# eloialonso/diamond

Measured on NVIDIA H100. Metric: imagined frames/sec (64x64, 3 denoise steps), higher is better.
Workload: dtype fp16 tensor-core operands (split-fp16 on the residual-stream 1x1/conv_in layers), fp32 accumulate, fp32 activations

## Files before the change

### diamond_b200/_lib.py

```python
import ctypes as C
import os
from typing import Optional

_HERE = os.path.dirname(os.path.abspath(__file__))
LIB_PATH = os.path.join(_HERE, "libdiamond_b200.so")
DMD_MAX_LEVELS = 8

_vp, _i, _f, _sz = C.c_void_p, C.c_int, C.c_float, C.c_size_t


class PrepDesc(C.Structure):
    _fields_ = [
        ("src0", _vp), ("src1", _vp), ("C0", _i), ("C1", _i), ("B", _i), ("Hs", _i), ("Ws", _i), ("upsample", _i),
        ("mode", _i), ("silu", _i), ("stats0", _vp), ("stats1", _vp), ("gs0", _i), ("gs1", _i),
        ("film", _vp), ("film_stride", _i), ("film_off", _i), ("gamma", _vp), ("beta", _vp), ("eps", _f),
        ("dst0", _vp), ("dst1", _vp), ("dst_raw0", _vp), ("dst_raw1", _vp),
        ("dst_lo0", _vp), ("dst_lo1", _vp), ("dst_raw_lo0", _vp), ("dst_raw_lo1", _vp),
    ]


class ConvDesc(C.Structure):
    _fields_ = [
        ("src0", _vp), ("src1", _vp), ("C0", _i), ("C1", _i), ("B", _i), ("H", _i), ("W", _i), ("taps", _i), ("stride", _i),
        ("wpk", _vp), ("bias", _vp), ("Cout", _i), ("CoutPad", _i),
        ("residual", _vp), ("out", _vp), ("out_stats", _vp), ("out_gs", _i), ("debug", _i), ("debug_buf", _vp),
        ("precise", _i), ("wpk_layout", _i), ("src0_lo", _vp), ("src1_lo", _vp),
        ("xsrc0", _vp), ("xsrc1", _vp), ("xsrc0_lo", _vp), ("xsrc1_lo", _vp), ("xC0", _i), ("xC1", _i), ("wpk_x", _vp), ("bias_x", _vp),
    ]


class DenoiserConfigC(C.Structure):
    _fields_ = [
        ("img_channels", _i), ("num_steps_conditioning", _i), ("cond_channels", _i), ("num_levels", _i),
        ("depths", _i * DMD_MAX_LEVELS), ("channels", _i * DMD_MAX_LEVELS), ("attn_depths", _i * DMD_MAX_LEVELS),
        ("num_actions", _i), ("sigma_data", _f), ("sigma_offset_noise", _f),
    ]


class ActorCriticConfigC(C.Structure):
    _fields_ = [
        ("lstm_dim", _i), ("img_channels", _i), ("img_size", _i), ("num_levels", _i),
        ("channels", _i * DMD_MAX_LEVELS), ("down", _i * DMD_MAX_LEVELS), ("num_actions", _i),
    ]


class RewEndConfigC(C.Structure):
    _fields_ = [
        ("lstm_dim", _i), ("img_channels", _i), ("img_size", _i), ("cond_channels", _i), ("num_levels", _i),
        ("depths", _i * DMD_MAX_LEVELS), ("channels", _i * DMD_MAX_LEVELS), ("attn_depths", _i * DMD_MAX_LEVELS), ("num_actions", _i),
    ]


class SamplerConfigC(C.Structure):
    _fields_ = [
        ("num_sigmas", _i), ("sigmas_host", C.POINTER(_f)), ("order", _i),
        ("s_churn", _f), ("s_tmin", _f), ("s_tmax", _f), ("s_noise", _f),
    ]


class WgradDesc(C.Structure):
    _fields_ = [("grad", _vp), ("act", _vp), ("Cg", _i), ("Ca", _i), ("B", _i), ("H", _i), ("W", _i), ("taps", _i),
                ("dW", _vp), ("Cout", _i), ("Cin", _i), ("CinTot", _i), ("ci_off", _i), ("inv_scale", _vp),
                ("accumulate", _i), ("partial", _vp), ("partial_bytes", _sz), ("debug", _i)]


class ConvPlanInfo(C.Structure):
    _fields_ = [("tiles", _i), ("kslabs", _i), ("stages", _i), ("acc_cols", _i),
                ("smem_bytes", C.c_ulonglong), ("weight_bytes", C.c_ulonglong)]


class NormBwdDesc(C.Structure):
    _fields_ = [("x", _vp), ("gy", _vp), ("stats", _vp), ("B", _i), ("HW", _i), ("C", _i), ("gs", _i), ("mode", _i), ("act", _i),
                ("film", _vp), ("film_stride", _i), ("film_off", _i), ("film_ctot", _i), ("c_off", _i),
                ("gamma", _vp), ("beta", _vp), ("eps", _f), ("sumA", _vp), ("sumB", _vp), ("sum_stride", _i),
                ("gx", _vp), ("addend", _vp), ("accumulate", _i)]


_ll = C.c_longlong


class U8Frames(C.Structure):
    _fields_ = [("levels", _vp), ("batch_stride", _ll), ("frame_stride", _ll),
                ("kinds", _vp), ("kind_batch_stride", _ll), ("kind_frame_stride", _ll), ("table", _vp)]


class OptimTensor(C.Structure):
    _fields_ = [("param", _vp), ("grad", _vp), ("exp_avg", _vp), ("exp_avg_sq", _vp), ("numel", _ll), ("weight_decay", C.c_double)]


SIGNATURES = {
    "dmd_version": (_i, []),
    "dmd_last_error": (C.c_char_p, []),
    "dmd_launch_count": (C.c_longlong, [_i]),
    "dmd_ktrace_begin": (_i, [_i]),
    "dmd_ktrace_end": (_i, [_vp, _i]),
    "dmd_ktrace_name": (C.c_char_p, [_i]),
    "dmd_pack_conv_weight": (_i, [_vp, _vp, _i, _i, _i, _i, _i, _i, _i, _i, _vp]),
    "dmd_plc16_bytes": (_sz, [_i, _i, _i, _i]),
    "dmd_prep_act": (_i, [C.POINTER(PrepDesc), _vp]),
    "dmd_prep_plan": (_i, [C.POINTER(PrepDesc), C.POINTER(C.c_int), C.POINTER(C.c_int), C.POINTER(C.c_int)]),
    "dmd_conv_plan": (_i, [C.POINTER(ConvDesc), C.POINTER(ConvPlanInfo)]),
    "dmd_conv2d_fprop": (_i, [C.POINTER(ConvDesc), _vp]),
    "dmd_pack_conv_weight_dgrad": (_i, [_vp, _vp, _i, _i, _i, _i, _i, _vp]),
    "dmd_wgrad_partial_bytes": (_sz, []),
    "dmd_conv2d_wgrad": (_i, [C.POINTER(WgradDesc), _vp]),
    "dmd_gn_stats": (_i, [_vp, _vp, _i, _i, _i, _i, _vp]),
    "dmd_attn_fwd": (_i, [_vp] * 10 + [_i, _i, _i, _i, _f, _vp]),
    "dmd_attn_scratch_bytes": (_sz, [_i, _i, _i]),
    "dmd_attn_fwd_scratch": (_i, [_vp] * 10 + [_i, _i, _i, _i, _f, _vp, _sz, _vp]),
    "dmd_nchw_to_nhwc": (_i, [_vp, _vp, _i, _i, _i, _i, _vp]),
    "dmd_nhwc_to_nchw": (_i, [_vp, _vp, _i, _i, _i, _i, _vp]),
    "dmd_linear": (_i, [_vp, _vp, _vp, _vp, _i, _i, _i, _i, _i, _i, _vp]),
    "dmd_maxpool2_stats": (_i, [_vp, _vp, _vp, _i, _i, _i, _i, _i, _vp]),
    "dmd_lstm_gates": (_i, [_vp, _vp, _vp, _vp, _i, _i, _vp]),
    "dmd_resize_nhwc": (_i, [_vp, _vp, _i, _i, _i, _i, _i, _i, _vp, _i, _vp]),
    "dmd_norm_bwd": (_i, [C.POINTER(NormBwdDesc), _i, _vp]),
    "dmd_norm_affine_grad": (_i, [C.POINTER(NormBwdDesc), _vp, _vp, _vp, _vp]),
    "dmd_attn_bwd": (_i, [_vp] * 16 + [_i, _i, _i, _i, _f, _vp]),
    "dmd_sgemm_partial_floats": (_ll, [_i, _i, _i, _i]),
    "dmd_sgemm": (_i, [_vp, _ll, _ll, _vp, _ll, _ll, _vp, _ll, _i, _i, _i, _vp, _i, _i, _vp, _vp]),
    "dmd_film_wgrad": (_i, [_vp, _vp, _vp, _vp, _vp, _i, _i, _i, _vp, _vp]),
    "dmd_embedding_bwd": (_i, [_vp, _vp, _vp, _i, _i, _i, _i, _vp, _vp]),
    "dmd_colsum": (_i, [_vp, _vp, _vp, _vp, _ll, _i, _i, _vp]),
    "dmd_sumpool2": (_i, [_vp, _vp, _i, _i, _i, _i, _i, _vp]),
    "dmd_dsilu_mul": (_i, [_vp, _vp, _vp, _ll, _vp]),
    "dmd_maxpool2_bwd": (_i, [_vp, _vp, _vp, _i, _i, _i, _i, _vp]),
    "dmd_lstm_cell_bwd": (_i, [_vp] * 6 + [_i, _i, _vp]),
    "dmd_heads_bwd": (_i, [_vp] * 10 + [_i, _i, _i, _vp]),
    "dmd_loss_scale": (_i, [_vp, _ll, _vp, _vp, _vp]),
    "dmd_denoiser_create": (_vp, [C.POINTER(DenoiserConfigC)]),
    "dmd_denoiser_destroy": (None, [_vp]),
    "dmd_denoiser_num_tensors": (_i, [_vp]),
    "dmd_denoiser_packed_bytes": (_sz, [_vp]),
    "dmd_denoiser_set_weights": (_i, [_vp, C.POINTER(_vp), _i, _vp, _vp]),
    "dmd_denoiser_workspace_bytes": (_sz, [_vp, _i, _i, _i]),
    "dmd_denoiser_forward": (_i, [_vp, _i, _i, _i, _vp, _vp, _i, _vp, _vp, _vp, _vp, _vp, _sz, _vp]),
    "dmd_inner_model_forward": (_i, [_vp, _i, _i, _i, _vp, _vp, _i, _vp, _vp, _vp, _vp, _sz, _vp]),
    "dmd_denoiser_train_workspace_bytes": (_sz, [_vp, _i, _i, _i]),
    "dmd_denoiser_grad_layout": (C.c_longlong, [_vp, C.POINTER(C.c_longlong), C.POINTER(C.c_longlong), _i]),
    "dmd_inner_model_forward_train": (_i, [_vp, _i, _i, _i, _vp, _vp, _i, _vp, _vp, _vp, _vp, _sz, _vp]),
    "dmd_denoiser_backward": (_i, [_vp, _i, _i, _i, _vp, _vp, C.c_longlong, _vp, _vp]),
    "dmd_inner_model_forward_u8": (_i, [_vp, _i, _i, _i, _vp, _vp, _i, C.POINTER(U8Frames), _vp, _vp, _vp, _sz, _vp]),
    "dmd_inner_model_forward_train_u8": (_i, [_vp, _i, _i, _i, _vp, _vp, _i, C.POINTER(U8Frames), _vp, _vp, _vp, _sz, _vp]),
    "dmd_sampler_sample": (_i, [_vp, C.POINTER(SamplerConfigC), _i, _i, _i, _vp, _vp, _i, _vp, _vp, _vp, _vp, _sz, _i, _vp]),
    "dmd_actor_critic_create": (_vp, [C.POINTER(ActorCriticConfigC)]),
    "dmd_actor_critic_destroy": (None, [_vp]),
    "dmd_actor_critic_num_tensors": (_i, [_vp]),
    "dmd_actor_critic_packed_bytes": (_sz, [_vp]),
    "dmd_actor_critic_set_weights": (_i, [_vp, C.POINTER(_vp), _i, _vp, _vp]),
    "dmd_actor_critic_workspace_bytes": (_sz, [_vp, _i]),
    "dmd_actor_critic_forward": (_i, [_vp, _i, _vp, _vp, _vp, _vp, _vp, _vp, _vp, _vp, _sz, _vp]),
    "dmd_actor_critic_backward_scratch_bytes": (_sz, [_vp, _i]),
    "dmd_actor_critic_grad_layout": (C.c_longlong, [_vp, C.POINTER(C.c_longlong), C.POINTER(C.c_longlong), _i]),
    "dmd_actor_critic_backward": (_i, [_vp, _i] + [_vp] * 8 + [C.c_longlong, _vp, _vp, _vp, _vp, _sz, _vp]),
    "dmd_actor_critic_backward_accumulate": (_i, [_vp, _i] + [_vp] * 8 + [C.c_longlong, _vp, _vp, _vp, _vp, _sz, _vp]),
    "dmd_rew_end_create": (_vp, [C.POINTER(RewEndConfigC)]),
    "dmd_rew_end_destroy": (None, [_vp]),
    "dmd_rew_end_num_tensors": (_i, [_vp]),
    "dmd_rew_end_packed_bytes": (_sz, [_vp]),
    "dmd_rew_end_set_weights": (_i, [_vp, C.POINTER(_vp), _i, _vp, _vp]),
    "dmd_rew_end_workspace_bytes": (_sz, [_vp, _i]),
    "dmd_rew_end_predict": (_i, [_vp, _i, _i] + [_vp] * 9 + [_vp, _sz, _vp]),
    "dmd_rew_end_train_workspace_bytes": (_sz, [_vp, _i, _i]),
    "dmd_rew_end_grad_layout": (C.c_longlong, [_vp, C.POINTER(C.c_longlong), C.POINTER(C.c_longlong), _i]),
    "dmd_rew_end_forward_train": (_i, [_vp, _i, _i] + [_vp] * 9 + [_vp, _sz, _vp]),
    "dmd_rew_end_backward": (_i, [_vp, _i, _i] + [_vp] * 5 + [C.c_longlong, _vp, _vp, _vp, _vp]),
    "dmd_rew_end_predict_u8": (_i, [_vp, _i, _i, C.POINTER(U8Frames), C.POINTER(U8Frames)] + [_vp] * 7 + [_vp, _sz, _vp]),
    "dmd_rew_end_forward_train_u8": (_i, [_vp, _i, _i, C.POINTER(U8Frames), C.POINTER(U8Frames)] + [_vp] * 7 + [_vp, _sz, _vp]),
    "dmd_lambda_returns": (_i, [_vp, _vp, _vp, _vp, _vp, _i, _i, C.c_double, C.c_double, _vp]),
    "dmd_grad_norm_partial_bytes": (_sz, [C.POINTER(OptimTensor), _i]),
    "dmd_grad_norm_clip": (_i, [C.POINTER(OptimTensor), _i, C.c_double, _i, _vp, _vp, _sz, _vp]),
    "dmd_adamw_step": (_i, [C.POINTER(OptimTensor), _i, C.c_double, C.c_double, C.c_double, C.c_double, C.c_double, _vp]),
}

_lib: Optional[C.CDLL] = None


class LibraryMissing(RuntimeError):
    pass


def lib() -> C.CDLL:
    global _lib
    if _lib is None:
        if not os.path.exists(LIB_PATH):
            raise LibraryMissing(
                f"{LIB_PATH} not found: build it with `python -c 'import __graft_entry__ as g; g.build()'` "
                "(diamond_b200 has no CPU / eager fallback)"
            )
        handle = C.CDLL(LIB_PATH)
        for name, (res, args) in SIGNATURES.items():
            fn = getattr(handle, name)
            fn.restype, fn.argtypes = res, args
        _lib = handle
    return _lib


def check(rc: int) -> None:
    if rc != 0:
        raise RuntimeError("diamond_b200: " + lib().dmd_last_error().decode("utf-8", "replace"))


def ptr(t) -> Optional[int]:
    return None if t is None else t.data_ptr()


def current_stream() -> int:
    import torch

    return torch.cuda.current_stream().cuda_stream
```

### diamond_b200/csrc/api.cu

```cuda
#include <cstdlib>
#include <memory>
#include <mutex>
#include <map>
#include <cuda_runtime.h>

#include <cmath>
#include <cstdarg>
#include <cstdio>
#include <cstring>
#include <functional>
#include <string>
#include <vector>

#include "../../include/diamond_b200.h"
#include "aux_kernels.cuh"
#include "conv_tc.cuh"
#include "wgrad_tc.cuh"
#include "bwd_kernels.cuh"
#include "optim_kernels.cuh"

using namespace dmd;

static thread_local std::string g_err;
static thread_local long long g_launches = 0;

static int fail(const char* fmt, ...) {
  char buf[1024];
  va_list ap;
  va_start(ap, fmt);
  vsnprintf(buf, sizeof(buf), fmt, ap);
  va_end(ap);
  g_err = buf;
  return 1;
}
#define DMD_CHECK(cond, ...) \
  do {                       \
    if (!(cond)) return fail(__VA_ARGS__); \
  } while (0)
#define DMD_CUDA(expr)                                                                   \
  do {                                                                                   \
    cudaError_t e__ = (expr);                                                            \
    if (e__ != cudaSuccess) { (void)cudaGetLastError(); return fail("%s failed: %s", #expr, cudaGetErrorString(e__)); } \
  } while (0)
#define DMD_LAUNCH_OK()                                                                 \
  do {                                                                                  \
    ++g_launches;                                                                       \
    cudaError_t e__ = cudaGetLastError();                                               \
    if (e__ != cudaSuccess) return fail("kernel launch failed: %s (%s:%d)", cudaGetErrorString(e__), __FILE__, __LINE__); \
  } while (0)

static int u8_frames_arg(const char* who, const char* name, const dmd_u8_frames* f, U8Frames* out) {
  DMD_CHECK(f, "%s: %s is NULL", who, name);
  DMD_CHECK(f->levels, "%s: %s->levels is NULL", who, name);
  DMD_CHECK(f->kinds, "%s: %s->kinds is NULL", who, name);
  DMD_CHECK(f->table, "%s: %s->table is NULL", who, name);
  DMD_CHECK(((uintptr_t)f->table & 3) == 0, "%s: %s->table is not 4-byte aligned", who, name);
  DMD_CHECK(f->batch_stride >= 0 && f->frame_stride >= 0, "%s: %s->batch_stride / frame_stride must be >= 0 (got %lld, %lld)", who,
            name, f->batch_stride, f->frame_stride);
  DMD_CHECK(f->kind_batch_stride >= 0 && f->kind_frame_stride >= 0,
            "%s: %s->kind_batch_stride / kind_frame_stride must be >= 0 (got %lld, %lld)", who, name, f->kind_batch_stride,
            f->kind_frame_stride);
  *out = U8Frames{f->levels, f->batch_stride, f->frame_stride, f->kinds, f->kind_batch_stride, f->kind_frame_stride, f->table};
  return 0;
}

extern "C" int dmd_version(void) { return DMD_VERSION; }
extern "C" const char* dmd_last_error(void) { return g_err.c_str(); }
extern "C" long long dmd_launch_count(int reset) {
  long long v = g_launches;
  if (reset) g_launches = 0;
  return v;
}

static long long* g_kt_buf = nullptr;
static int g_kt_cap = 0, g_kt_n = 0;
static bool g_kt_on = false;
static std::vector<std::string> g_kt_names;
static long long* kt_slot(const char* kind, int grid, int aux) {
  if (!g_kt_on || g_kt_n >= g_kt_cap) return nullptr;
  char buf[96];
  snprintf(buf, sizeof(buf), "%s grid=%d aux=%d", kind, grid, aux);
  g_kt_names.push_back(buf);
  return g_kt_buf + g_kt_n++;
}
extern "C" int dmd_ktrace_begin(int capacity) {
  if (g_kt_cap < capacity) {
    if (g_kt_buf) cudaFree(g_kt_buf);
    if (cudaMalloc(&g_kt_buf, (size_t)capacity * 8) != cudaSuccess) { g_kt_buf = nullptr; g_kt_cap = 0; g_err = "ktrace: cudaMalloc failed"; return 1; }
    g_kt_cap = capacity;
  }
  cudaMemset(g_kt_buf, 0, (size_t)g_kt_cap * 8);
  g_kt_n = 0; g_kt_names.clear(); g_kt_on = true;
  return 0;
}
extern "C" int dmd_ktrace_end(long long* stamps, int capacity) {
  g_kt_on = false;
  const int n = g_kt_n < capacity ? g_kt_n : capacity;
  if (n > 0 && stamps) cudaMemcpy(stamps, g_kt_buf, (size_t)n * 8, cudaMemcpyDeviceToHost);
  return n;
}
extern "C" const char* dmd_ktrace_name(int i) { return (i >= 0 && i < (int)g_kt_names.size()) ? g_kt_names[i].c_str() : ""; }

static inline int round_up(int x, int m) { return (x + m - 1) / m * m; }
constexpr int kPlanSms = 132;
static inline int gn_group_size(int C) {
  int G = C / 32 > 1 ? C / 32 : 1;
  return C / G;
}

static size_t plc16_bytes(int B, int H, int W, int C) {
  const Plc g = plc_geometry(B, H, W);
  return (size_t)(round_up(C, 16) / 8) * g.Qalloc * 16;
}
extern "C" size_t dmd_plc16_bytes(int B, int H, int W, int C) { return plc16_bytes(B, H, W, C); }

static int tune_int(const char* name, int dflt) {
  static std::mutex mu;
  static std::map<std::string, int> cache;
  std::lock_guard<std::mutex> lk(mu);
  auto it = cache.find(name);
  if (it != cache.end()) return it->second;
  const char* v = getenv(name);
  const int r = (v && *v) ? atoi(v) : dflt;
  cache[name] = r;
  return r;
}

static int conv_fill(const dmd_conv_desc* d, ConvParams* p, size_t* smem, int* acc_cols) {
  DMD_CHECK(d->src0 && d->out && d->wpk, "conv: null src0/out/wpk");
  DMD_CHECK(d->taps == 9 || d->taps == 1, "conv: taps must be 1 or 9 (got %d)", d->taps);
  DMD_CHECK(d->debug == 0 && d->debug_buf == nullptr, "conv: debug / debug_buf must be 0 / NULL (the kernel has no bring-up switches)");
  DMD_CHECK(d->stride == 1 || d->stride == 2, "conv: stride must be 1 or 2");
  DMD_CHECK(d->C0 > 0 && d->C0 % 16 == 0 && d->C1 % 16 == 0 && d->C0 + d->C1 <= kMaxCin, "conv: operand channels must be multiples of 16, total <= %d (C0=%d C1=%d)", kMaxCin, d->C0, d->C1);
  DMD_CHECK((d->C1 == 0) == (d->src1 == nullptr), "conv: src1/C1 mismatch");
  if (d->precise) DMD_CHECK(d->src0_lo && ((d->C1 == 0) == (d->src1_lo == nullptr)), "conv: precise mode needs the low operand parts");
  DMD_CHECK(d->CoutPad % 16 == 0 && d->CoutPad >= 16 && d->CoutPad <= 128 && d->Cout <= d->CoutPad && d->Cout > 0, "conv: bad Cout=%d CoutPad=%d", d->Cout, d->CoutPad);
  memset(p, 0, sizeof(*p));
  {
    const uint8_t* hi[2] = {(const uint8_t*)d->src0, (const uint8_t*)d->src1};
    const uint8_t* lo[2] = {(const uint8_t*)d->src0_lo, (const uint8_t*)d->src1_lo};
    const int cs[2] = {d->C0, d->C1};
    const int nsrc = d->C1 ? 2 : 1;
    int n = 0;
    for (int rep = 0; rep < (d->precise ? 3 : 1); ++rep)
      for (int k = 0; k < nsrc; ++k) { p->seg_base[n] = (rep == 1) ? lo[k] : hi[k]; p->seg_slabs[n] = cs[k] / 16; ++n; }
    p->Cin = (d->C0 + d->C1) * (d->precise ? 3 : 1);
    p->Cextra = 0;
    if (d->wpk_x) {
      DMD_CHECK(d->xsrc0 && d->xsrc0_lo && d->xC0 > 0 && d->xC0 % 16 == 0 && d->xC1 % 16 == 0 && d->xC0 + d->xC1 <= kMaxCin, "conv: bad fused projection operands");
      DMD_CHECK((d->xC1 == 0) == (d->xsrc1 == nullptr) && (d->xC1 == 0) == (d->xsrc1_lo == nullptr), "conv: fused projection src1 mismatch");
      const uint8_t* xh[2] = {(const uint8_t*)d->xsrc0, (const uint8_t*)d->xsrc1};
      const uint8_t* xl[2] = {(const uint8_t*)d->xsrc0_lo, (const uint8_t*)d->xsrc1_lo};
      const int xc[2] = {d->xC0, d->xC1};
      for (int rep = 0; rep < 2; ++rep)
        for (int k = 0; k < (d->xC1 ? 2 : 1); ++k) {
          DMD_CHECK(n < kMaxSegs, "conv: too many operand segments");
          p->seg_base[n] = (rep == 1) ? xl[k] : xh[k]; p->seg_slabs[n] = xc[k] / 16; ++n;
        }
      p->Cextra = 3 * (d->xC0 + d->xC1);
      p->xslabs = 2 * (d->xC0 + d->xC1) / 16;
      p->wpk_extra = reinterpret_cast<const __half*>(d->wpk_x);
      p->bias_extra = d->bias_x;
    }
    p->nseg = n;
  }
  p->B = d->B; p->H = d->H; p->W = d->W; p->taps = d->taps; p->stride = d->stride;
  if (d->stride == 2) DMD_CHECK(p->H % 2 == 0 && p->W % 2 == 0, "conv: stride 2 needs even H,W");
  p->wpk = reinterpret_cast<const __half*>(d->wpk); p->bias = d->bias; p->Cout = d->Cout; p->CoutPad = d->CoutPad;
  p->resid = d->residual; p->out = d->out; p->ostats = d->out_stats; p->ogs = d->out_gs > 0 ? d->out_gs : d->Cout;
  const Plc g = plc_geometry(d->B, d->H, d->W);
  p->PW = g.PW; p->PH = g.PH; p->Q = g.Q; p->G = g.G; p->plane_bytes = (unsigned long long)g.Qalloc * 16;
  DMD_CHECK((long long)g.Q * (g.PW > g.PH ? g.PW : g.PH) < (1ll << 32), "conv: problem too large for 32-bit position math");
  p->trs = d->wpk_layout == 1 ? 1 : 0;
  if (p->trs) DMD_CHECK(d->taps == 9 && !d->precise && 3 * d->CoutPad <= 256, "conv: row-stacked weights need a 3x3, non-split conv with CoutPad <= 80");
  const int halo = d->taps == 9 ? g.PW + 1 : 0;
  p->P = kTileM + 2 * halo; p->Palloc = p->P | 1;
  if (d->out_stats) {
    const int L4 = d->Cout / 4;
    DMD_CHECK(g.PH * g.PW >= 64, "conv: image too small for the statistics epilogue (a tile may touch at most %d images)", kStatSlots);
    DMD_CHECK(d->Cout % 4 == 0 && (L4 == 4 || L4 == 8 || L4 == 16 || L4 == 32), "conv: out_stats needs Cout in {16,32,64,128} (got %d)", d->Cout);
    DMD_CHECK(d->out_gs == 16 || d->out_gs == 32 || d->out_gs == 64 || d->out_gs == 128, "conv: out_gs must be 16/32/64/128");
    DMD_CHECK(d->Cout % d->out_gs == 0 && d->Cout / d->out_gs <= kMaxOutGroups, "conv: bad output groups");
  }
  p->dPW.init(g.PW); p->dPH.init(g.PH);
  p->num_tiles = (g.Q + kTileM - 1) / kTileM;
  const int kslabs = p->Cin / 16 + p->xslabs;
  const uint32_t w_bytes = conv_weight_bytes(p->taps, p->Cin, p->Cextra, p->CoutPad);
  const ConvSmemLayout L0 = conv_smem_layout(w_bytes, p->Palloc, 0);
  const long long budget = 227ll * 1024 - (long long)L0.total;
  int stages = budget > 0 ? (int)(budget / (long long)L0.slab_bytes) : 0;
  if (stages > 4 * kslabs) stages = 4 * kslabs;
  if (stages > kMaxStages) stages = kMaxStages;
  DMD_CHECK(stages >= 2, "conv: shared memory too small for W=%d Cin=%d CoutPad=%d", p->W, p->Cin, p->CoutPad);
  p->stages = stages;
  *smem = conv_smem_layout(w_bytes, p->Palloc, stages).total;
  *acc_cols = d->CoutPad <= 16 ? 16 : (d->CoutPad <= 32 ? 32 : (d->CoutPad <= 64 ? 64 : 128));
  return 0;
}

struct DevState { int num_sms = 0; void* zeros = nullptr; };
static thread_local int g_num_sms = 0;
static thread_local const uint8_t* g_zeros = nullptr;
static int init_kernels() {
  static std::mutex mu;
  static std::map<int, DevState> states;
  int dev = 0;
  DMD_CUDA(cudaGetDevice(&dev));
  std::lock_guard<std::mutex> lk(mu);
  auto it = states.find(dev);
  if (it == states.end()) {
    DevState st;
    DMD_CUDA(cudaDeviceGetAttribute(&st.num_sms, cudaDevAttrMultiProcessorCount, dev));
    DMD_CUDA(cudaFuncSetAttribute(conv_tc_kernel<16, 9>, cudaFuncAttributeMaxDynamicSharedMemorySize, 227 * 1024));
    DMD_CUDA(cudaFuncSetAttribute(conv_tc_kernel<32, 9>, cudaFuncAttributeMaxDynamicSharedMemorySize, 227 * 1024));
    DMD_CUDA(cudaFuncSetAttribute(conv_tc_kernel<64, 9>, cudaFuncAttributeMaxDynamicSharedMemorySize, 227 * 1024));
    DMD_CUDA(cudaFuncSetAttribute(conv_tc_kernel<128, 9>, cudaFuncAttributeMaxDynamicSharedMemorySize, 227 * 1024));
    DMD_CUDA(cudaFuncSetAttribute(conv_tc_kernel<16, 1>, cudaFuncAttributeMaxDynamicSharedMemorySize, 227 * 1024));
    DMD_CUDA(cudaFuncSetAttribute(conv_tc_kernel<32, 1>, cudaFuncAttributeMaxDynamicSharedMemorySize, 227 * 1024));
    DMD_CUDA(cudaFuncSetAttribute(conv_tc_kernel<64, 1>, cudaFuncAttributeMaxDynamicSharedMemorySize, 227 * 1024));
    DMD_CUDA(cudaFuncSetAttribute(conv_tc_kernel<128, 1>, cudaFuncAttributeMaxDynamicSharedMemorySize, 227 * 1024));
    DMD_CUDA(cudaFuncSetAttribute(wgrad_tc_kernel<16>, cudaFuncAttributeMaxDynamicSharedMemorySize, 227 * 1024));
    DMD_CUDA(cudaFuncSetAttribute(wgrad_tc_kernel<32>, cudaFuncAttributeMaxDynamicSharedMemorySize, 227 * 1024));
    DMD_CUDA(cudaFuncSetAttribute(wgrad_tc_kernel<64>, cudaFuncAttributeMaxDynamicSharedMemorySize, 227 * 1024));
    DMD_CUDA(cudaFuncSetAttribute(attn_cluster_kernel<64>, cudaFuncAttributeMaxDynamicSharedMemorySize, 128 * 1024));
    DMD_CUDA(cudaFuncSetAttribute(attn_cluster_kernel<32>, cudaFuncAttributeMaxDynamicSharedMemorySize, 128 * 1024));
    DMD_CUDA(cudaFuncSetAttribute(attn_kernel<64>, cudaFuncAttributeMaxDynamicSharedMemorySize, 128 * 1024));
    DMD_CUDA(cudaFuncSetAttribute(attn_kernel<32>, cudaFuncAttributeMaxDynamicSharedMemorySize, 128 * 1024));
    DMD_CUDA(cudaFuncSetAttribute(attn_bwd_kernel<64>, cudaFuncAttributeMaxDynamicSharedMemorySize, 200 * 1024));
    DMD_CUDA(cudaFuncSetAttribute(attn_bwd_kernel<32>, cudaFuncAttributeMaxDynamicSharedMemorySize, 200 * 1024));
    DMD_CUDA(cudaFuncSetAttribute(linear_kernel<4>, cudaFuncAttributeMaxDynamicSharedMemorySize, 64 * 1024));
    DMD_CUDA(cudaFuncSetAttribute(linear_kernel<2>, cudaFuncAttributeMaxDynamicSharedMemorySize, 64 * 1024));
    DMD_CUDA(cudaFuncSetAttribute(linear_kernel<1>, cudaFuncAttributeMaxDynamicSharedMemorySize, 64 * 1024));
    DMD_CUDA(cudaMalloc(&st.zeros, 4096));
    DMD_CUDA(cudaMemset(st.zeros, 0, 4096));
    it = states.emplace(dev, st).first;
  }
  g_num_sms = it->second.num_sms;
  g_zeros = (const uint8_t*)it->second.zeros;
  return 0;
}

template <typename Kernel, typename Params>
static int launch_pdl(Kernel kernel, dim3 grid, dim3 block, size_t smem, cudaStream_t st, const Params& p) {
  cudaLaunchConfig_t cfg;
  memset(&cfg, 0, sizeof(cfg));
  cfg.gridDim = grid; cfg.blockDim = block; cfg.dynamicSmemBytes = smem; cfg.stream = st;
  cudaLaunchAttribute attr[1];
  attr[0].id = cudaLaunchAttributeProgrammaticStreamSerialization;
  attr[0].val.programmaticStreamSerializationAllowed = 1;
  cfg.attrs = attr; cfg.numAttrs = tune_int("DMD_NO_PDL", 0) ? 0 : 1;
  DMD_CUDA(cudaLaunchKernelEx(&cfg, kernel, p));
  DMD_LAUNCH_OK();
  return 0;
}

template <int kCols>
static int conv_launch_t(const ConvParams& p0, size_t smem, cudaStream_t st) {
  if (init_kernels()) return 1;
  const int grid = p0.num_tiles < g_num_sms ? p0.num_tiles : g_num_sms;
  ConvParams p = p0;
  p.ktrace = kt_slot(p.taps == 9 ? "conv3x3" : "conv1x1", p.num_tiles, (p.Cin + p.Cextra) * 1000 + p.W);
  if (p.taps == 9) return launch_pdl(conv_tc_kernel<kCols, 9>, dim3(grid), dim3(kConvThreads), smem, st, p);
  return launch_pdl(conv_tc_kernel<kCols, 1>, dim3(grid), dim3(kConvThreads), smem, st, p);
}

static int prep_fill(const dmd_prep_desc* d, PrepParams* p, int* nsrc) {
  DMD_CHECK(d->src0 && d->dst0, "prep: null src0/dst0");
  DMD_CHECK(d->C0 % 8 == 0 && d->C1 % 8 == 0 && d->C0 > 0 && d->C0 <= kMaxCin && d->C1 <= kMaxCin, "prep: channels must be multiples of 8 (C0=%d C1=%d)", d->C0, d->C1);
  DMD_CHECK((d->C1 == 0) == (d->src1 == nullptr) && (d->C1 == 0) == (d->dst1 == nullptr), "prep: src1/dst1/C1 mismatch");
  DMD_CHECK(d->mode >= 0 && d->mode <= 2, "prep: bad mode");
  for (int c : {d->C0, d->C1 ? d->C1 : 16}) {
    const int cp = round_up(c, 16);
    DMD_CHECK(cp == 16 || cp == 32 || cp == 64 || cp == 128, "prep: a source must have <= 16/32/64/128 channels after padding (got %d)", c);
  }
  memset(p, 0, sizeof(*p));
  p->s[0].src = d->src0; p->s[0].C = d->C0; p->s[0].Cpad = round_up(d->C0, 16); p->s[0].stats = d->stats0; p->s[0].gs = d->gs0 > 0 ? d->gs0 : 8;
  p->s[0].c_offset = 0; p->s[0].dst = (uint8_t*)d->dst0; p->s[0].dst_raw = (uint8_t*)d->dst_raw0;
  p->s[0].dst_lo = (uint8_t*)d->dst_lo0; p->s[0].dst_raw_lo = (uint8_t*)d->dst_raw_lo0;
  p->s[1].dst_lo = (uint8_t*)d->dst_lo1; p->s[1].dst_raw_lo = (uint8_t*)d->dst_raw_lo1;
  DMD_CHECK(!(d->dst_raw_lo0 && !d->dst_raw0) && !(d->dst_raw_lo1 && !d->dst_raw1), "prep: raw low part needs the raw operand too");
  p->s[1].src = d->src1; p->s[1].C = d->C1; p->s[1].Cpad = round_up(d->C1 > 0 ? d->C1 : 16, 16); p->s[1].stats = d->stats1; p->s[1].gs = d->gs1 > 0 ? d->gs1 : 8;
  p->s[1].c_offset = d->C0; p->s[1].dst = (uint8_t*)d->dst1; p->s[1].dst_raw = (uint8_t*)d->dst_raw1;
  if (d->mode) {
    DMD_CHECK(d->stats0 && d->gs0 > 0 && d->C0 % d->gs0 == 0, "prep: norm mode needs stats0/gs0");
    if (d->C1) DMD_CHECK(d->stats1 && d->gs1 > 0 && d->C1 % d->gs1 == 0, "prep: norm mode needs stats1/gs1");
    if (d->mode == 1) DMD_CHECK(d->film != nullptr, "prep: AdaGroupNorm needs film");
    if (d->mode == 2) DMD_CHECK(d->gamma && d->beta, "prep: GroupNorm needs gamma/beta");
    DMD_CHECK(d->upsample == 0, "prep: norm + upsample unsupported");
  }
  p->B = d->B; p->Hs = d->Hs; p->Ws = d->Ws; p->ups = d->upsample;
  DMD_CHECK(d->upsample >= 0 && d->upsample <= 2, "prep: upsample must be 0, 1 (nearest 2x) or 2 (zero insertion)");
  DMD_CHECK(d->upsample != 2 || (d->mode == 0 && !d->silu && d->C1 == 0 && !d->dst_raw0 && !d->dst_lo0), "prep: zero insertion is a raw single-source operand");
  p->H = d->upsample ? 2 * d->Hs : d->Hs; p->W = d->upsample ? 2 * d->Ws : d->Ws;
  p->mode = d->mode; p->act = d->silu ? 1 : 0;
  p->film = d->film; p->film_stride = d->film_stride; p->film_off = d->film_off; p->film_ctot = d->C0 + d->C1;
  p->gamma = d->gamma; p->beta = d->beta; p->eps = d->eps;
  const Plc g = plc_geometry(d->B, p->H, p->W);
  DMD_CHECK(g.PH * g.PW >= 32, "prep: image too small");
  int ppb = g.PH * g.PW >= 256 ? 256 : (g.PH * g.PW / 32) * 32;
  while (ppb > 64 && (g.Qalloc + ppb - 1) / ppb < tune_int("DMD_PREP_MIN_BLOCKS", 2 * kPlanSms)) ppb >>= 1;
  ppb = (ppb / 32) * 32;
  p->pos_per_block = ppb;
  DMD_CHECK(d->mode == 0 || (d->C0 / (d->gs0 > 0 ? d->gs0 : 8) <= 4 && d->C1 / (d->gs1 > 0 ? d->gs1 : 8) <= 4),
            "prep: at most 4 groups per source (C0=%d gs0=%d, C1=%d gs1=%d)", d->C0, d->gs0, d->C1, d->gs1);
  DMD_CHECK((long long)g.Q * (g.PW > g.PH ? g.PW : g.PH) < (1ll << 32), "prep: problem too large for 32-bit position math");
  p->PW = g.PW; p->PH = g.PH; p->Q = g.Q; p->G = g.G; p->Qalloc = g.Qalloc; p->plane_bytes = (unsigned long long)g.Qalloc * 16;
  p->dPW.init(g.PW); p->dPH.init(g.PH);
  *nsrc = d->C1 ? 2 : 1;
  return 0;
}
static int prep_launch(const PrepParams& p0, int nsrc, cudaStream_t st) {
  PrepParams p = p0;
  p.ktrace = kt_slot("prep", (p.Qalloc + p.pos_per_block - 1) / p.pos_per_block * nsrc, p.mode * 1000 + p.W);
  if (p.ups == 2) {
    const long long total = (long long)p.Qalloc * (p.s[0].Cpad >> 3);
    return launch_pdl(zero_insert_prep_kernel, dim3((unsigned)((total + 255) / 256)), dim3(256), 0, st, p);
  }
  const dim3 grid((p.Qalloc + p.pos_per_block - 1) / p.pos_per_block, 1, nsrc);
  bool fast = tune_int("DMD_PREP_FAST", 1) != 0 && p.mode != 0 && p.act && p.ups == 0;
  const bool raw = p.s[0].dst_raw != nullptr;
  for (int k = 0; k < nsrc && fast; ++k) {
    const PrepSrc& S = p.s[k];
    if (S.dst_lo != nullptr || (S.dst_raw != nullptr) != raw || (S.dst_raw_lo != nullptr) != raw || S.Cpad != p.s[0].Cpad || S.C % 8 != 0) fast = false;
  }
  if (fast && (long long)p.B * p.Hs * p.Ws * (p.s[0].C > p.s[nsrc - 1].C ? p.s[0].C : p.s[nsrc - 1].C) >= (1ll << 31)) fast = false;
  if (fast) {
    const int nch = p.s[0].Cpad >> 3;
    if (nch == 8) return raw ? launch_pdl(prep_fast_kernel<8, true>, grid, dim3(kPrepThreads), 0, st, p) : launch_pdl(prep_fast_kernel<8, false>, grid, dim3(kPrepThreads), 0, st, p);
    if (nch == 4) return raw ? launch_pdl(prep_fast_kernel<4, true>, grid, dim3(kPrepThreads), 0, st, p) : launch_pdl(prep_fast_kernel<4, false>, grid, dim3(kPrepThreads), 0, st, p);
  }
  return launch_pdl(prep_act_kernel, grid, dim3(kPrepThreads), 0, st, p);
}
extern "C" int dmd_prep_plan(const dmd_prep_desc* d, int* blocks, int* pos_per_block, int* sources) {
  DMD_CHECK(d && blocks && pos_per_block && sources, "prep_plan: null argument");
  PrepParams p; int nsrc;
  if (prep_fill(d, &p, &nsrc)) return 1;
  *blocks = (p.Qalloc + p.pos_per_block - 1) / p.pos_per_block; *pos_per_block = p.pos_per_block; *sources = nsrc;
  return 0;
}
extern "C" int dmd_conv_plan(const dmd_conv_desc* d, dmd_conv_plan_info* out) {
  DMD_CHECK(d && out, "conv_plan: null argument");
  ConvParams p; size_t smem; int cols;
  if (conv_fill(d, &p, &smem, &cols)) return 1;
  out->tiles = p.num_tiles; out->kslabs = p.Cin / 16 + p.xslabs; out->stages = p.stages; out->acc_cols = cols;
  out->smem_bytes = smem; out->weight_bytes = conv_weight_bytes(p.taps, p.Cin, p.Cextra, p.CoutPad);
  return 0;
}
extern "C" int dmd_prep_act(const dmd_prep_desc* d, void* stream) {
  PrepParams p; int nsrc;
  if (prep_fill(d, &p, &nsrc)) return 1;
  return prep_launch(p, nsrc, (cudaStream_t)stream);
}

static int conv_launch(const ConvParams& p, size_t smem, int acc_cols, cudaStream_t st) {
  switch (acc_cols) {
    case 16: return conv_launch_t<16>(p, smem, st);
    case 32: return conv_launch_t<32>(p, smem, st);
    case 64: return conv_launch_t<64>(p, smem, st);
    default: return conv_launch_t<128>(p, smem, st);
  }
}

extern "C" int dmd_conv2d_fprop(const dmd_conv_desc* d, void* stream) {
  ConvParams p; size_t smem; int cols;
  if (conv_fill(d, &p, &smem, &cols)) return 1;
  return conv_launch(p, smem, cols, (cudaStream_t)stream);
}

struct WgradLaunch { WgradParams wp; WgradReduceParams rp; size_t smem; int grid; };
static size_t wgrad_partial_bytes(int num_sms) { return (size_t)num_sms * kWgTaps * 64 * 64 * sizeof(float); }

static int wgrad_fill(const void* grad, int Cg, const void* act, int Ca, int B, int H, int W, int taps, float* partial,
                      int Cout, int Cin, int CinTot, int ci_off, const float* inv_scale, int accumulate, int debug, WgradLaunch* L) {
  DMD_CHECK(grad && act && partial, "wgrad: null operand / partial buffer");
  DMD_CHECK(taps == 9 || taps == 1, "wgrad: taps must be 1 or 9");
  DMD_CHECK(Cg % 8 == 0 && Cg > 0 && Cg <= 64, "wgrad: gradient operand channels must be a multiple of 8, <= 64 (got %d)", Cg);
  DMD_CHECK(Ca == 16 || Ca == 32 || Ca == 64, "wgrad: activation operand channels must be 16, 32 or 64 (got %d)", Ca);
  DMD_CHECK(Cout > 0 && Cout <= Cg && Cin > 0 && Cin <= Ca && ci_off >= 0 && ci_off + Cin <= CinTot, "wgrad: bad channel counts");
  if (init_kernels()) return 1;
  memset(L, 0, sizeof(*L));
  const Plc g = plc_geometry(B, H, W);
  const size_t plane = (size_t)g.Qalloc * 16;
  WgradParams& wp = L->wp;
  const int ng = Cg / 8;
  for (int j = 0; j < 8; ++j) wp.a_plane[j] = j < ng ? (const uint8_t*)grad + (size_t)j * plane : nullptr;
  wp.zeros = g_zeros;
  wp.nB = Ca / 8;
  for (int j = 0; j < wp.nB; ++j) wp.b_plane[j] = (const uint8_t*)act + (size_t)j * plane;
  wp.taps = taps; wp.PW = g.PW; wp.halo = taps == 9 ? g.PW + 1 : 0;
  wp.G = g.G; wp.num_tiles = (g.Q + kTileM - 1) / kTileM; wp.Pb = kTileM + 2 * wp.halo;
  const WgradSmem one = wgrad_smem(wp.nB, wp.halo, 1);
  int stages = (int)((227ll * 1024 - 256) / (long long)(one.a_bytes + one.b_bytes));
  if (stages > kWgStagesMax) stages = kWgStagesMax;
  DMD_CHECK(stages >= 2, "wgrad: image too wide for the shared-memory stage (W=%d)", W);
  wp.stages = stages;
  wp.partial = partial; wp.dbg = debug;
  L->smem = wgrad_smem(wp.nB, wp.halo, stages).total;
  L->grid = wp.num_tiles < g_num_sms ? wp.num_tiles : g_num_sms;
  WgradReduceParams& rp = L->rp;
  rp.partial = partial; rp.nparts = L->grid; rp.N = Ca;
  rp.Cout = Cout; rp.Cin = Cin; rp.CinTot = CinTot; rp.ci_off = ci_off; rp.taps = taps;
  rp.inv_scale = inv_scale; rp.accumulate = accumulate;
  return 0;
}
static int wgrad_launch(const WgradLaunch& L, float* dW, cudaStream_t st) {
  const int N = L.wp.nB * 8;
  if (N == 16) { if (launch_pdl(wgrad_tc_kernel<16>, dim3(L.grid), dim3(kWgThreads), L.smem, st, L.wp)) return 1; }
  else if (N == 32) { if (launch_pdl(wgrad_tc_kernel<32>, dim3(L.grid), dim3(kWgThreads), L.smem, st, L.wp)) return 1; }
  else if (launch_pdl(wgrad_tc_kernel<64>, dim3(L.grid), dim3(kWgThreads), L.smem, st, L.wp)) return 1;
  WgradReduceParams rp = L.rp;
  rp.dW = dW;
  const int total = rp.taps * 64 * rp.N;
  wgrad_reduce_kernel<<<(total + 63) / 64, 256, 0, st>>>(rp);
  DMD_LAUNCH_OK();
  return 0;
}

extern "C" size_t dmd_wgrad_partial_bytes(void) {
  if (init_kernels()) return 0;
  return wgrad_partial_bytes(g_num_sms);
}
extern "C" int dmd_conv2d_wgrad(const dmd_wgrad_desc* d, void* stream) {
  DMD_CHECK(d && d->dW, "wgrad: null descriptor / dW");
  if (init_kernels()) return 1;
  DMD_CHECK(d->partial_bytes >= wgrad_partial_bytes(g_num_sms), "wgrad: partial buffer too small (%zu < %zu)", d->partial_bytes, wgrad_partial_bytes(g_num_sms));
  WgradLaunch L;
  if (wgrad_fill(d->grad, d->Cg, d->act, d->Ca, d->B, d->H, d->W, d->taps, (float*)d->partial, d->Cout, d->Cin, d->CinTot, d->ci_off,
                 d->inv_scale, d->accumulate, d->debug, &L)) return 1;
  return wgrad_launch(L, d->dW, (cudaStream_t)stream);
}
extern "C" int dmd_pack_conv_weight_dgrad(const float* w, void* wpk, int CoutF, int CinTotF, int ci_off, int CinK, int taps, void* stream) {
  DMD_CHECK(w && wpk, "pack_T: null pointer");
  const int CinP = round_up(CoutF, 16), CoutP = round_up(CinK, 16);
  const int total = taps * CinP * CoutP;
  pack_conv_weight_T_kernel<<<(total + 255) / 256, 256, 0, (cudaStream_t)stream>>>(w, (__half*)wpk, CoutF, CinTotF, ci_off, CinK, CinP, CoutP, taps);
  DMD_LAUNCH_OK();
  return 0;
}

extern "C" int dmd_pack_conv_weight(const float* w, void* wpk, int Cout, int CoutPad, int CinReal, int Cin, int taps,
                                    int c0_real, int c0_store, int precise, void* stream) {
  DMD_CHECK(w && wpk, "pack: null pointer");
  if (precise == 3) {
    DMD_CHECK(taps == 9, "pack: the row-stacked layout is for 3x3 kernels");
    const int total3 = 9 * Cin * CoutPad;
    pack_conv_weight_trs_kernel<<<(total3 + 255) / 256, 256, 0, (cudaStream_t)stream>>>(w, (__half*)wpk, Cout, CoutPad, CinReal, Cin, c0_real, c0_store);
    DMD_LAUNCH_OK();
    return 0;
  }
  DMD_CHECK(precise >= 0 && precise <= 2, "pack: precise must be 0, 1 (split [W_hi | W_hi | W_lo]), 2 (low parts only) or 3 (row-stacked)");
  const int total = taps * Cin * CoutPad * (precise == 1 ? 3 : 1);
  pack_conv_weight_kernel<<<(total + 255) / 256, 256, 0, (cudaStream_t)stream>>>(w, (__half*)wpk, Cout, CoutPad, CinReal, Cin, taps, c0_real, c0_store, precise);
  DMD_LAUNCH_OK();
  return 0;
}

extern "C" int dmd_gn_stats(const float* x, double* stats, int B, int HW, int C, int gs, void* stream) {
  DMD_CHECK(x && stats && gs > 0 && C % gs == 0, "gn_stats: bad arguments");
  long long per = (long long)HW * C;
  int chunks = (int)((per + 256 * 64 - 1) / (256 * 64));
  if (chunks < 1) chunks = 1;
  if (chunks > 64) chunks = 64;
  gn_stats_kernel<<<dim3(chunks, B), 256, 0, (cudaStream_t)stream>>>(x, stats, HW, C, gs);
  DMD_LAUNCH_OK();
  return 0;
}

static size_t attn_scratch_bytes(int B, int L, int C) { return L == kAttnL ? 0 : (size_t)B * L * 3 * C * sizeof(float); }

static int attn_launch(const AttnParams& p, int B, cudaStream_t st) {
  DMD_CHECK((p.C == 64 || p.C == 32) && p.L >= 1 && p.C % p.gs == 0 && p.gs % 8 == 0,
            "attn: unsupported shape L=%d C=%d gs=%d (C in {32, 64}, groups of a multiple of 8 channels)", p.L, p.C, p.gs);
  if (init_kernels()) return 1;
  if (p.L != kAttnL) {
    DMD_CHECK(p.scratch && ((uintptr_t)p.scratch & 15) == 0, "attn: L=%d needs 16-byte aligned scratch of dmd_attn_scratch_bytes", p.L);
    DMD_CHECK(B >= 1 && B <= 65535, "attn: B=%d out of range", B);
    const dim3 grid((p.L + kAttnTile - 1) / kAttnTile, B);
    AttnParams pa = p;
    pa.ktrace = kt_slot("attn qkv", (int)(grid.x * grid.y), p.L);
    if (p.C == 64) attn_qkv_kernel<64><<<grid, kAttnQkvThreads, 0, st>>>(pa);
    else attn_qkv_kernel<32><<<grid, kAttnQkvThreads, 0, st>>>(pa);
    DMD_LAUNCH_OK();
    pa.ktrace = kt_slot("attn softmax", (int)(grid.x * grid.y), p.L);
    if (p.C == 64) attn_stream_kernel<64><<<grid, kAttnSThreads, 0, st>>>(pa);
    else attn_stream_kernel<32><<<grid, kAttnSThreads, 0, st>>>(pa);
    DMD_LAUNCH_OK();
    return 0;
  }
  const size_t smem = sizeof(float) * ((size_t)p.L * (p.C + 1) * 2 + (size_t)p.L * (3 * p.C + 4));
  AttnParams pt = p;
  pt.ktrace = kt_slot("attn", B, p.C);
  if (tune_int("DMD_ATTN_CLUSTER", 1) != 0 && p.gs % (p.C / 4) == 0) {
    const int CH = p.C / 4;
    const size_t csmem = sizeof(float) * ((size_t)p.L * (p.C + 1) * 2 + (size_t)p.L * (3 * CH + 4) + (size_t)p.L * CH + (size_t)4 * CH * p.C);
    if (p.C == 64) attn_cluster_kernel<64><<<4 * B, kAttnCThreads, csmem, st>>>(pt);
    else attn_cluster_kernel<32><<<4 * B, kAttnCThreads, csmem, st>>>(pt);
    DMD_LAUNCH_OK();
    return 0;
  }
  if (p.C == 64) attn_kernel<64><<<B, kAttnThreads, smem, st>>>(pt);
  else attn_kernel<32><<<B, kAttnThreads, smem, st>>>(pt);
  DMD_LAUNCH_OK();
  return 0;
}

static int linear_launch(const float* in, const float* W, const float* bias, float* out, int B, int K, int F, int silu, cudaStream_t st,
                         int accumulate = 0, int hw_perm = 0) {
  DMD_CHECK(K % 4 == 0, "linear: K=%d must be a multiple of 4", K);
  DMD_CHECK(hw_perm == 0 || K % hw_perm == 0, "linear: bad hw_perm");
  if (init_kernels()) return 1;
  const int by = (B + 31) / 32;
  const int forceJ = tune_int("DMD_LINEAR_J", 0);
  if (forceJ == 4 || (forceJ == 0 && (long long)((F + 31) / 32) * by >= 2 * kPlanSms))
    linear_kernel<4><<<dim3((F + 31) / 32, by), 256, (size_t)(32 + 32) * kLinChunk * sizeof(float), st>>>(in, W, bias, out, B, K, F, silu, accumulate, hw_perm);
  else if (forceJ == 2 || (forceJ == 0 && (long long)((F + 15) / 16) * by >= kPlanSms))
    linear_kernel<2><<<dim3((F + 15) / 16, by), 256, (size_t)(16 + 32) * kLinChunk * sizeof(float), st>>>(in, W, bias, out, B, K, F, silu, accumulate, hw_perm);
  else
    linear_kernel<1><<<dim3((F + 7) / 8, by), 256, (size_t)(8 + 32) * kLinChunk * sizeof(float), st>>>(in, W, bias, out, B, K, F, silu, accumulate, hw_perm);
  DMD_LAUNCH_OK();
  return 0;
}

static int maxpool2_stats_launch(const float* x, float* y, double* stats, int B, int H, int W, int C, int gs, cudaStream_t st) {
  DMD_CHECK(H % 2 == 0 && W % 2 == 0, "maxpool2_stats: H=%d, W=%d must be even", H, W);
  DMD_CHECK((long long)(H / 2) * (W / 2) * C < (1ll << 31), "maxpool2_stats: image too large for 32-bit indices");
  if (stats) DMD_CHECK(gs > 0 && C % gs == 0 && (gs % 32 == 0 || (gs <= 32 && (gs & (gs - 1)) == 0)) && (C % 32 == 0 || 256 % C == 0),
                       "maxpool2_stats: statistics need gs a power of two <= 32 or a multiple of 32, and C %% 32 == 0 or 256 %% C == 0 (C=%d gs=%d)", C, gs);
  const int total = (H / 2) * (W / 2) * C;
  maxpool2_stats_kernel<<<dim3((total + 255) / 256, B), 256, 0, st>>>(x, y, stats, H, W, C, gs);
  DMD_LAUNCH_OK();
  return 0;
}

static int lstm_gates_launch(const float* gates, const float* c_in, float* h_out, float* c_out, int B, int Hd, cudaStream_t st) {
  lstm_gates_kernel<<<(B * Hd + 255) / 256, 256, 0, st>>>(gates, c_in, h_out, c_out, B, Hd);
  DMD_LAUNCH_OK();
  return 0;
}

extern "C" int dmd_linear(const float* in, const float* W, const float* bias, float* out, int B, int K, int F, int silu, int accumulate,
                          int hw_perm, void* stream) {
  DMD_CHECK(in && W && out && B > 0 && K > 0 && F > 0 && hw_perm >= 0, "linear: bad arguments");
  return linear_launch(in, W, bias, out, B, K, F, silu, (cudaStream_t)stream, accumulate, hw_perm);
}
extern "C" int dmd_maxpool2_stats(const float* x, float* y, double* stats, int B, int H, int W, int C, int gs, void* stream) {
  DMD_CHECK(x && y && B > 0 && H > 0 && W > 0 && C > 0, "maxpool2_stats: bad arguments");
  return maxpool2_stats_launch(x, y, stats, B, H, W, C, gs, (cudaStream_t)stream);
}
extern "C" int dmd_lstm_gates(const float* gates, const float* c_in, float* h_out, float* c_out, int B, int Hd, void* stream) {
  DMD_CHECK(gates && c_in && h_out && c_out && B > 0 && Hd > 0, "lstm_gates: bad arguments");
  DMD_CHECK((long long)B * Hd <= (1ll << 30), "lstm_gates: too many cells for 32-bit indices");
  return lstm_gates_launch(gates, c_in, h_out, c_out, B, Hd, (cudaStream_t)stream);
}

extern "C" int dmd_attn_fwd(const float* x, const double* stats_in, const float* gamma, const float* beta,
                            const float* wqkv, const float* bqkv, const float* wout, const float* bout, float* out,
                            double* out_stats, int B, int L, int C, int gs, float eps, void* stream) {
  AttnParams p{x, stats_in, gamma, beta, wqkv, bqkv, wout, bout, out, out_stats, L, C, gs, eps};
  return attn_launch(p, B, (cudaStream_t)stream);
}
extern "C" size_t dmd_attn_scratch_bytes(int B, int L, int C) { return B > 0 && L > 0 && C > 0 ? attn_scratch_bytes(B, L, C) : 0; }
extern "C" int dmd_attn_fwd_scratch(const float* x, const double* stats_in, const float* gamma, const float* beta,
                                    const float* wqkv, const float* bqkv, const float* wout, const float* bout, float* out,
                                    double* out_stats, int B, int L, int C, int gs, float eps, void* scratch, size_t scratch_bytes,
                                    void* stream) {
  DMD_CHECK(x && stats_in && gamma && beta && wqkv && bqkv && wout && bout && out && B > 0 && L > 0 && C > 0 && gs > 0,
            "attn_fwd_scratch: bad arguments");
  DMD_CHECK(scratch_bytes >= attn_scratch_bytes(B, L, C), "attn_fwd_scratch: scratch too small (%zu < %zu)", scratch_bytes,
            attn_scratch_bytes(B, L, C));
  AttnParams p{x, stats_in, gamma, beta, wqkv, bqkv, wout, bout, out, out_stats, L, C, gs, eps};
  p.scratch = (float*)scratch;
  return attn_launch(p, B, (cudaStream_t)stream);
}

extern "C" int dmd_nchw_to_nhwc(const float* in, float* out, int B, int C, int CP, int HW, void* stream) {
  nchw_to_nhwc_kernel<<<dim3((HW + 255) / 256, B), 256, 0, (cudaStream_t)stream>>>(in, out, C, CP, HW);
  DMD_LAUNCH_OK();
  return 0;
}
extern "C" int dmd_nhwc_to_nchw(const float* in, float* out, int B, int C, int CP, int HW, void* stream) {
  nhwc_to_nchw_kernel<<<dim3((HW + 255) / 256, B), 256, 0, (cudaStream_t)stream>>>(in, out, C, CP, HW);
  DMD_LAUNCH_OK();
  return 0;
}


static int loss_scale_launch(const float* g, long long n, unsigned int* amax_bits, float* scale, cudaStream_t st) {
  absmax_kernel<<<(int)std::min<long long>(std::max<long long>((n + 255) / 256, 1), 1184), 256, 0, st>>>(g, amax_bits, n);
  DMD_LAUNCH_OK();
  loss_scale_kernel<<<1, 1, 0, st>>>(amax_bits, scale);
  DMD_LAUNCH_OK();
  return 0;
}

static int colsum_launch(const float* x, float* out, float* out2, const float* inv, long long rows, int C, int Creal, cudaStream_t st) {
  const int L4 = (C < 256 ? C : 256) >> 2, lanes = 256 / L4;
  long long blocks = (rows + (long long)lanes * 8 - 1) / ((long long)lanes * 8);
  blocks = blocks > 592 ? 592 : (blocks < 1 ? 1 : blocks);
  colsum_kernel<<<dim3((unsigned)blocks, (C + 255) / 256), 256, 0, st>>>(x, out, out2, inv, rows, C, Creal);
  DMD_LAUNCH_OK();
  return 0;
}

static int norm_bwd_ppb(int B, int HW) {
  int ppb = HW;
  while (ppb > 32 && (long long)B * ((HW + ppb - 1) / ppb) < 2 * kPlanSms) ppb >>= 1;
  return ppb;
}
static int norm_bwd_launch(const NormBwdParams& nb, int pass, cudaStream_t st) {
  const int ppb = norm_bwd_ppb(nb.B, nb.HW);
  const dim3 grid((nb.HW + ppb - 1) / ppb, nb.B);
  if (pass == 1) norm_bwd_pass1_kernel<<<grid, kNormThreads, 0, st>>>(nb, ppb);
  else norm_bwd_pass2_kernel<<<grid, kNormThreads, 0, st>>>(nb, ppb);
  DMD_LAUNCH_OK();
  return 0;
}
// ... 217 lines not shown
  FilmW n1, n2; ConvW c1, c2;
  int has_attn; int an_w, an_b, qkv_w, qkv_b, op_w, op_b;
};

struct Tens { float* data; double* stats; int C, H, W, gs; float* grad = nullptr; int gid = -1; };

enum OpKind { OP_CONV = 0, OP_ATTN = 1, OP_PREP = 2, OP_RESIZE = 4 };
struct Op { int kind; ConvParams conv; size_t smem; int cols; AttnParams attn; PrepParams prep; int prep_nsrc; ResizeParams rs; };
constexpr int kScratchSlots = 10;

struct Operand {
  uint8_t *n0 = nullptr, *n1 = nullptr, *r0 = nullptr, *r1 = nullptr, *nl0 = nullptr, *rl0 = nullptr, *rl1 = nullptr; int C0 = 0, C1 = 0, H = 0, W = 0, op = -1;
  Tens a{}, b{}; bool has_b = false;
  int upsample = 0, mode = 0; const FilmW* film = nullptr; int gamma_idx = 0, beta_idx = 0; bool silu = false, also_raw = false, split = false;
};

enum BKind { B_PREP = 0, B_CONV, B_WGRAD, B_COLSUM, B_NORM1, B_NORM2, B_AFFINE, B_POOL, B_ATTN, B_MEMSET, B_SGEMM, B_FILMW,
             B_LINEAR, B_DSILU, B_EMB };
struct BOp {
  int kind = 0;
  PrepParams prep; int prep_nsrc = 1;
  ConvParams conv; size_t smem = 0; int cols = 0;
  WgradLaunch wg;
  long long goff = -1, goff2 = -1;
  NormBwdParams nb;
  int chunks = 0;
  const float* src = nullptr; float* dst = nullptr; long long rows = 0; int C = 0, Creal = 0, H = 0, W = 0, acc = 0;
  AttnBwdParams ab; long long goffs[6] = {-1, -1, -1, -1, -1, -1};
  void* ms_ptr = nullptr; size_t ms_bytes = 0;
  const float *ga = nullptr, *gb = nullptr; float* gc = nullptr; long long sam = 0, sak = 0, sbk = 0, sbn = 0, ldc = 0, c_goff = -1;
  int M = 0, N = 0, K = 0, use_inv = 0;
  const float *lin_in = nullptr, *lin_w = nullptr, *lin_b = nullptr; float* lin_out = nullptr; int lin_K = 0, lin_F = 0;
  int emb_T = 0, emb_actions = 0;
};

enum RecKind { R_CONVIN = 0, R_DOWN, R_UP, R_RES, R_OUT };
struct Rec {
  int kind = 0;
  const ConvW* cw = nullptr; const ResBlockW* rb = nullptr;
  Tens x, skip, t, o, a; bool has_skip = false;
  Operand in1, in2;
};

struct Plan {
  int B = 0, H = 0, W = 0;
  int T = 1;
  long long tmp_floats = 0;
  uint8_t* base = nullptr;
  size_t bytes = 0;
  float *xin = nullptr, *cs = nullptr, *cemb = nullptr, *chid = nullptr, *cond = nullptr, *film = nullptr, *fout = nullptr;
  double* stats = nullptr; size_t stats_bytes = 0;
  int CP_in = 0, CF = 0;
  std::vector<Op> ops;
  uint8_t* scratch[kScratchSlots] = {nullptr};
  int scratch_next = 0;
  bool train = false;
  int n_grad_tensors = 0;
  std::vector<BOp> bops;
  std::vector<Rec> tape;
  const int64_t* t_act = nullptr;
  float *tA = nullptr, *tB = nullptr, *tC = nullptr;
  uint8_t *gyA = nullptr, *gyB = nullptr;
  float *gF = nullptr;
  float *dfilm = nullptr, *nsum = nullptr, *partial = nullptr, *scale = nullptr;
  float *dcond = nullptr, *dh = nullptr, *cpre = nullptr, *dpre = nullptr, *de = nullptr;
  unsigned int* amax = nullptr;
  long long *film_woff = nullptr, *film_boff = nullptr;
  std::vector<long long> film_woff_h, film_boff_h;
  uint8_t* zero_begin = nullptr; size_t zero_bytes = 0;
  Tens feat{};
  float *gates = nullptr;
  float *cseq = nullptr, *hseq = nullptr;
  float *hid = nullptr, *logits_tm = nullptr;
  int64_t* act_tm = nullptr;
  float *g_tm = nullptr, *g_hid = nullptr, *hpre = nullptr, *g_pre = nullptr, *g_y = nullptr, *dgates = nullptr, *gcs = nullptr;
  float *s_xc = nullptr, *s_x2 = nullptr, *s_d = nullptr;
  float *sig_all = nullptr, *cemb_all = nullptr, *chid_all = nullptr, *cond_all = nullptr, *film_all = nullptr;
};

constexpr int kMaxSamplerEvals = 24;
struct SamplerGraph {
  bool valid = false;
  int B = 0, H = 0, W = 0; void* ws = nullptr; int order = 0; bool has_eps = false;
  const void *obs = nullptr, *act = nullptr, *traj = nullptr, *eps = nullptr, *out = nullptr; StackView sv{};
  unsigned long long stamp = 0;
  std::vector<float> sigmas; float churn[4] = {0, 0, 0, 0};
  long long kernels = 0;
  cudaGraphExec_t exec = nullptr;
};

struct ModelCore {
  int n_tensors = 0;
  std::vector<long long> numel, goff;
  long long grad_total = 0;
  std::vector<const float*> ptrs;
  uint8_t* packed = nullptr;
  size_t packed_bytes = 0;
  int cond_channels = 0, film_rows = 0;
  size_t film_w_off = 0, film_b_off = 0;
  std::vector<std::unique_ptr<Plan>> tplans;

  const float* P(int idx) const { return ptrs.empty() ? nullptr : ptrs[idx]; }
  void finish(size_t pk) {
    n_tensors = (int)numel.size();
    goff.assign(n_tensors, 0);
    grad_total = 0;
    for (int i = 0; i < n_tensors; ++i) { goff[i] = grad_total; grad_total += (numel[i] + 3) & ~3ll; }
    film_w_off = pk; pk += (size_t)film_rows * cond_channels * 4; pk = (pk + 255) & ~(size_t)255;
    film_b_off = pk; pk += (size_t)film_rows * 4; pk = (pk + 255) & ~(size_t)255;
    packed_bytes = pk;
  }
  int set_weights(const char* module, const float* const* ptrs_host, int n_ptrs, void* packed_buf, bool* moved) {
    DMD_CHECK(ptrs_host && packed_buf, "set_weights: null argument");
    DMD_CHECK(n_ptrs == n_tensors, "set_weights: expected %d tensors (%s.state_dict order), got %d", n_tensors, module, n_ptrs);
    *moved = packed != (uint8_t*)packed_buf || ptrs.empty() || memcmp(ptrs.data(), ptrs_host, sizeof(float*) * n_ptrs) != 0;
    ptrs.assign(ptrs_host, ptrs_host + n_ptrs);
    packed = (uint8_t*)packed_buf;
    return 0;
  }
  bool ready() const { return !ptrs.empty() && packed; }
};

long long grad_layout(const ModelCore* m, long long* offsets, long long* numels, int n) {
  if (!m || n != m->n_tensors) { fail("grad_layout: expected %d entries", m ? m->n_tensors : 0); return -1; }
  for (int i = 0; i < n; ++i) { if (offsets) offsets[i] = m->goff[i]; if (numels) numels[i] = m->numel[i]; }
  return m->grad_total;
}

struct RewEndLayout {
  Plan plan;
  Tens feat{};
  float *x_gates = nullptr, *y = nullptr, *hid = nullptr, *logits_tm = nullptr, *hc[2] = {nullptr, nullptr};
};

}

struct dmd_denoiser {
  dmd_denoiser_config cfg;
  ModelCore core;
  int i_fourier = 0, i_actemb = 0, i_cp0w = 0, i_cp0b = 0, i_cp2w = 0, i_cp2b = 0, i_normout_w = 0, i_normout_b = 0;
  ConvW conv_in, conv_out;
  std::vector<std::vector<ResBlockW>> d_blocks, u_blocks;
  std::vector<ResBlockW> mid;
  std::vector<ConvW> downs, ups;
  Plan plan;
  std::vector<SamplerGraph> graphs;
  unsigned long long graph_clock = 0;
  cudaStream_t cap_stream = nullptr;
  int need_B = 0, need_H = 0, need_W = 0; size_t need_bytes = 0;
};

struct dmd_rew_end {
  dmd_rew_end_config cfg;
  ModelCore core;
  ConvW conv_in;
  std::vector<std::vector<ResBlockW>> blocks;
  std::vector<ConvW> downs;
  int i_actemb = 0, i_wih = 0, i_whh = 0, i_bih = 0, i_bhh = 0, i_h0w = 0, i_h0b = 0, i_h2w = 0;
  int feat_c = 0, feat_hw = 0;
  RewEndLayout lay;
};

namespace {

struct Walker {
  ModelCore* m; size_t pk = 0;
  int next(long long n) { m->numel.push_back(n); return (int)m->numel.size() - 1; }
  size_t take(size_t bytes) { const size_t off = pk; pk = (pk + bytes + 255) & ~(size_t)255; return off; }
  ConvW conv(int cout, int cin_real, int taps, int c0_real, int c0_store, int c1, bool split = false, bool dgrad = true) {
    ConvW c; c.w_idx = next((long long)cout * cin_real * taps); c.b_idx = next(cout);
    c.Cout = cout; c.CoutPad = round_up(cout, 16); c.CinReal = cin_real; c.taps = taps;
    c.c0_real = c0_real; c.c0_store = c0_store; c.Cin = round_up(c0_store + c1, 16);
    const size_t w1 = (size_t)taps * c.Cin * c.CoutPad * 2;
    c.precise = split && 3 * w1 <= 120 * 1024;
    c.three_pass = split && !c.precise;
    c.trs = (taps == 9 && !split && 3 * c.CoutPad <= 256 && tune_int("DMD_CONV_TRS", 0) != 0) ? 1 : 0;
    c.pk_off = take(w1 * (c.precise ? 3 : 1));
    if (c.three_pass) c.pk_lo_off = take(w1);
    if (dgrad) {
      c.nsrcT = c1 ? 2 : 1;
      c.srcC[0] = c0_real; c.srcC[1] = c1; c.srcOff[0] = 0; c.srcOff[1] = c0_real;
      for (int k = 0; k < c.nsrcT; ++k) c.pkT_off[k] = take((size_t)taps * round_up(cout, 16) * round_up(c.srcC[k], 16) * 2);
    }
    return c;
  }
  FilmW film(int C) {
    FilmW f; f.w_idx = next((long long)2 * C * m->cond_channels); f.b_idx = next(2 * C);
    f.C = C; f.off = m->film_rows; m->film_rows += 2 * C; return f;
  }
  ResBlockW resblock(int c0, int c1, int cout, bool attn) {
    ResBlockW r; r.cin = c0 + c1; r.cout = cout;
    r.has_proj = (r.cin != cout);
    if (r.has_proj) r.proj = conv(cout, r.cin, 1, c0, c0, c1, true);
    r.n1 = film(r.cin);
    r.c1 = conv(cout, r.cin, 9, c0, c0, c1);
    r.n2 = film(cout);
    r.c2 = conv(cout, cout, 9, cout, cout, 0);
    r.has_attn = attn;
    if (attn) {
      r.an_w = next(cout); r.an_b = next(cout); r.qkv_w = next((long long)3 * cout * cout); r.qkv_b = next(3 * cout);
      r.op_w = next((long long)cout * cout); r.op_b = next(cout);
    }
    return r;
  }
};

int build_structure(dmd_denoiser* h) {
  const dmd_denoiser_config& c = h->cfg;
  const int L = c.num_levels;
  h->core.cond_channels = c.cond_channels;
  Walker w{&h->core};
  const long long CC = c.cond_channels;
  h->i_fourier = w.next(CC / 2); h->i_actemb = w.next((long long)c.num_actions * (CC / c.num_steps_conditioning));
  h->i_cp0w = w.next(CC * CC); h->i_cp0b = w.next(CC); h->i_cp2w = w.next(CC * CC); h->i_cp2b = w.next(CC);
  const int cin_real = (c.num_steps_conditioning + 1) * c.img_channels;
  const int cin_store = round_up(cin_real, 16);
  h->conv_in = w.conv(c.channels[0], cin_real, 9, cin_real, cin_store, 0, true, false);
  h->d_blocks.resize(L);
  for (int i = 0; i < L; ++i) {
    const int c1 = c.channels[i > 0 ? i - 1 : 0], c2 = c.channels[i];
    for (int k = 0; k < c.depths[i]; ++k) h->d_blocks[i].push_back(w.resblock(k == 0 ? c1 : c2, 0, c2, c.attn_depths[i] != 0));
  }
  h->u_blocks.resize(L);
  for (int m = 0; m < L; ++m) {
    const int i = L - 1 - m;
    const int c1 = c.channels[i > 0 ? i - 1 : 0], c2 = c.channels[i];
    const int n = c.depths[i];
    for (int k = 0; k <= n; ++k) h->u_blocks[m].push_back(w.resblock(c2, k < n ? c2 : c1, k < n ? c2 : c1, c.attn_depths[i] != 0));
  }
  for (int k = 0; k < 2; ++k) h->mid.push_back(w.resblock(c.channels[L - 1], 0, c.channels[L - 1], true));
  h->downs.resize(L); h->ups.resize(L);
  for (int i = 1; i < L; ++i) h->downs[i] = w.conv(c.channels[i - 1], c.channels[i - 1], 9, c.channels[i - 1], c.channels[i - 1], 0);
  for (int m = 1; m < L; ++m) { const int ch = c.channels[L - 1 - m]; h->ups[m] = w.conv(ch, ch, 9, ch, ch, 0); }
  h->i_normout_w = w.next(c.channels[0]); h->i_normout_b = w.next(c.channels[0]);
  h->conv_out = w.conv(c.img_channels, c.channels[0], 9, c.channels[0], c.channels[0], 0);
  h->core.finish(w.pk);
  return 0;
}

dmd_prep_desc prep_desc(const float* src, int C, int B, int Hs, int Ws, int ups, int mode, const double* stats, const float* gamma,
                        const float* beta, void* dst, void* dst_lo = nullptr) {
  dmd_prep_desc d; memset(&d, 0, sizeof(d));
  d.src0 = src; d.C0 = C; d.B = B; d.Hs = Hs; d.Ws = Ws; d.upsample = ups; d.mode = mode; d.silu = mode ? 1 : 0;
  if (mode) { d.stats0 = stats; d.gs0 = gn_group_size(C); d.gamma = gamma; d.beta = beta; }
  d.eps = kGnEps; d.dst0 = dst; d.dst_lo0 = dst_lo;
  return d;
}
dmd_conv_desc dgrad_desc(const ConvW& cw, int k, const void* wpk, const void* gy, int B, int H, int W, float* out, bool accumulate) {
  dmd_conv_desc d; memset(&d, 0, sizeof(d));
  d.src0 = gy; d.C0 = round_up(cw.Cout, 16); d.B = B; d.H = H; d.W = W; d.taps = cw.taps; d.stride = 1;
  d.wpk = wpk; d.Cout = cw.srcC[k]; d.CoutPad = round_up(cw.srcC[k], 16);
  d.out = out; d.residual = accumulate ? out : nullptr;
  return d;
}
dmd_conv_desc conv_pass(dmd_conv_desc d, int pass, const void* wpk_lo) {
  const void *lo0 = d.src0_lo, *lo1 = d.src1_lo;
  d.precise = 0; d.src0_lo = d.src1_lo = nullptr;
  if (pass == 1) { d.src0 = lo0; d.src1 = lo1; }
  if (pass == 2) d.wpk = wpk_lo;
  if (pass > 0) { d.bias = nullptr; d.residual = d.out; }
  if (pass < 2) d.out_stats = nullptr;
  return d;
}
NormBwdParams gn_bwd_params(const float* x, const float* gy, const double* stats, int B, int HW, int C, int gs, const float* gamma,
                            const float* beta, float* nsum, float* gx, const float* addend, bool accumulate) {
  NormBwdParams nb; memset(&nb, 0, sizeof(nb));
  nb.x = x; nb.gy = gy; nb.stats = stats; nb.B = B; nb.HW = HW; nb.C = C; nb.gs = gs; nb.mode = 2; nb.act = 1; nb.eps = kGnEps;
  nb.gamma = gamma; nb.beta = beta;
  nb.sumA = nsum; nb.sumB = nsum ? nsum + (size_t)B * kMaxCin : nullptr; nb.sum_stride = kMaxCin;
  nb.gx = gx; nb.addend = addend; nb.accumulate = accumulate ? 1 : 0;
  return nb;
}

struct Bump {
  uint8_t* base; size_t off = 0;
  void* take(size_t bytes) { off = (off + 255) & ~(size_t)255; void* p = base ? base + off : nullptr; off += bytes; return p; }
};

struct PlanBuilder {
  const ModelCore* core; Plan* pl; Bump* bump; Bump* sbump; int err = 0;

  Tens tensor(int C, int H, int W, bool with_stats, bool with_grad = true) {
    Tens t; t.C = C; t.H = H; t.W = W; t.gs = gn_group_size(C);
    t.data = (float*)bump->take((size_t)pl->B * H * W * C * 4);
    t.stats = with_stats ? (double*)sbump->take((size_t)pl->B * (C / t.gs) * 2 * 8) : nullptr;
    if (pl->train && with_grad) { t.grad = (float*)bump->take((size_t)pl->B * H * W * C * 4); t.gid = pl->n_grad_tensors++; }
    return t;
  }
  void record(const Rec& r) { if (pl->train) pl->tape.push_back(r); }
  const float* P(int idx) const { return core->P(idx); }
  const void* pk(size_t off) const { return core->packed ? core->packed + off : (const void*)1; }

  uint8_t* scratch() {
    uint8_t* p = pl->scratch[pl->scratch_next];
    pl->scratch_next = (pl->scratch_next + 1) % kScratchSlots;
    return p ? p : (uint8_t*)1;
  }

  Operand prep(const Tens& a, const Tens* b, int upsample, int mode, const FilmW* film, int gamma_idx, int beta_idx, bool silu, bool also_raw, bool split = false) {
    Operand o;
    o.a = a; o.has_b = b != nullptr; if (b) o.b = *b;
    o.upsample = upsample; o.mode = mode; o.film = film; o.gamma_idx = gamma_idx; o.beta_idx = beta_idx; o.silu = silu; o.also_raw = also_raw; o.split = split;
    o.C0 = round_up(a.C, 16); o.C1 = b ? round_up(b->C, 16) : 0;
    o.H = upsample ? 2 * a.H : a.H; o.W = upsample ? 2 * a.W : a.W;
    materialize(o);
    return o;
  }
  void materialize(Operand& o) {
    if (o.n0) return;
    const Tens& a = o.a; const Tens* b = o.has_b ? &o.b : nullptr;
    dmd_prep_desc d; memset(&d, 0, sizeof(d));
    d.src0 = a.data ? a.data : (const float*)1; d.C0 = a.C; d.src1 = b ? (b->data ? b->data : (const float*)1) : nullptr; d.C1 = b ? b->C : 0;
    d.B = pl->B; d.Hs = a.H; d.Ws = a.W; d.upsample = o.upsample; d.mode = o.mode; d.silu = o.silu;
    if (o.mode) {
      d.stats0 = a.stats ? a.stats : (const double*)1; d.gs0 = a.gs;
      if (b) { d.stats1 = b->stats ? b->stats : (const double*)1; d.gs1 = b->gs; }
    }
    if (o.mode == 1) { d.film = pl->film ? pl->film : (const float*)1; d.film_stride = core->film_rows; d.film_off = o.film->off; }
    if (o.mode == 2) { d.gamma = P(o.gamma_idx) ? P(o.gamma_idx) : (const float*)1; d.beta = P(o.beta_idx) ? P(o.beta_idx) : (const float*)1; }
    d.eps = kGnEps;
    o.n0 = scratch(); d.dst0 = o.n0;
    if (b) { o.n1 = scratch(); d.dst1 = o.n1; }
    if (o.also_raw) { o.r0 = scratch(); d.dst_raw0 = o.r0; if (b) { o.r1 = scratch(); d.dst_raw1 = o.r1; } }
    if (o.split && o.also_raw) { o.rl0 = scratch(); d.dst_raw_lo0 = o.rl0; if (b) { o.rl1 = scratch(); d.dst_raw_lo1 = o.rl1; } }
    if (o.split && !o.also_raw) { o.nl0 = scratch(); d.dst_lo0 = o.nl0; }
    Op op; op.kind = OP_PREP;
    if (prep_fill(&d, &op.prep, &op.prep_nsrc)) { err = 1; return; }
    o.op = (int)pl->ops.size();
    pl->ops.push_back(op);
  }

  void conv(const ConvW& cw, Operand& in, bool raw, int stride, const Tens* resid, Tens& out, bool out_stats,
            const ConvW* xproj = nullptr, Operand* xin = nullptr) {
    materialize(in);
    if (xin) materialize(*xin);
    if (err) return;
    dmd_conv_desc d; memset(&d, 0, sizeof(d));
    if (xproj) {
      d.xsrc0 = xin->r0; d.xsrc0_lo = xin->rl0; d.xC0 = xin->C0;
      if (xin->C1) { d.xsrc1 = xin->r1; d.xsrc1_lo = xin->rl1; d.xC1 = xin->C1; }
      d.wpk_x = pk(xproj->pk_off); d.bias_x = P(xproj->b_idx);
      if (!xproj->precise) { fail("plan: a fused projection needs its split-fp16 weights in one pack"); err = 1; return; }
    }
    const bool split = cw.precise || cw.three_pass;
    d.src0 = raw ? in.r0 : in.n0; d.src1 = in.C1 ? (raw ? in.r1 : in.n1) : nullptr;
    d.precise = cw.precise; d.wpk_layout = cw.trs;
    if (split) { d.src0_lo = raw ? in.rl0 : in.nl0; d.src1_lo = in.C1 ? in.rl1 : nullptr; }
    d.C0 = in.C0; d.C1 = in.C1; d.B = pl->B; d.H = in.H; d.W = in.W; d.taps = cw.taps; d.stride = stride;
    d.wpk = pk(cw.pk_off); d.bias = P(cw.b_idx);
    d.Cout = cw.Cout; d.CoutPad = cw.CoutPad;
    d.residual = resid ? (resid->data ? resid->data : (const float*)1) : nullptr; d.out = out.data ? out.data : (float*)1;
    d.out_stats = out_stats ? (out.stats ? out.stats : (double*)1) : nullptr; d.out_gs = out.gs;
    if (split && (!d.src0_lo || (in.C1 && !d.src1_lo))) { fail("plan: precise conv without low operand parts"); err = 1; return; }
    if (in.C0 + in.C1 != cw.Cin) { fail("plan: operand channels %d+%d do not match the packed weights (%d)", in.C0, in.C1, cw.Cin); err = 1; return; }
    for (int pass = 0; pass < (cw.three_pass ? 3 : 1); ++pass) {
      const dmd_conv_desc dp = cw.three_pass ? conv_pass(d, pass, pk(cw.pk_lo_off)) : d;
      Op op; op.kind = OP_CONV;
      if (conv_fill(&dp, &op.conv, &op.smem, &op.cols)) { err = 1; return; }
      pl->ops.push_back(op);
    }
  }

  Tens resblock(const ResBlockW& rb, const Tens& x, const Tens* skip) {
    const int H = x.H, W = x.W;
    Operand in1 = prep(x, skip, 0, 1, &rb.n1, 0, 0, true, rb.has_proj != 0, rb.has_proj != 0);
    Tens t = tensor(rb.cout, H, W, true, false);
    conv(rb.c1, in1, false, 1, nullptr, t, true);
    Operand in2 = prep(t, nullptr, 0, 1, &rb.n2, 0, 0, true, false);
    Tens o = tensor(rb.cout, H, W, true);
    if (rb.has_proj) conv(rb.c2, in2, false, 1, nullptr, o, true, &rb.proj, &in1);
    else conv(rb.c2, in2, false, 1, &x, o, true);
    Rec rec; rec.kind = R_RES; rec.rb = &rb; rec.x = x; rec.has_skip = skip != nullptr; if (skip) rec.skip = *skip;
    rec.t = t; rec.o = o; rec.in1 = in1; rec.in2 = in2;
    if (!rb.has_attn) { record(rec); return o; }
    if (pl->train && H * W != kAttnL) {
      fail("training: the attention backward (attn_bwd_kernel) is built for 8x8 = 64 tokens only; this plan has an attention block "
           "over %dx%d = %d tokens (inference runs at any token count)", H, W, H * W);
      err = 1;
      return o;
    }
    Tens a = tensor(rb.cout, H, W, true);
    Op op; op.kind = OP_ATTN;
    op.attn = AttnParams{o.data, o.stats, P(rb.an_w), P(rb.an_b), P(rb.qkv_w), P(rb.qkv_b), P(rb.op_w), P(rb.op_b), a.data, a.stats, H * W, rb.cout, o.gs, kGnEps};
    if (H * W != kAttnL) op.attn.scratch = (float*)bump->take(attn_scratch_bytes(pl->B, H * W, rb.cout));
    pl->ops.push_back(op);
    rec.a = a;
    record(rec);
    return a;
  }

  int build_rew_end(const dmd_rew_end* h, Tens* feat) {
    const dmd_rew_end_config& c = h->cfg;
    const int L = c.num_levels, B = pl->B, H = pl->H, W = pl->W;
    if (H % (1 << (L - 1)) || W % (1 << (L - 1))) return fail("rew_end: H=%d W=%d must be multiples of %d", H, W, 1 << (L - 1));
    int cmax = 16;
    for (int i = 0; i < L; ++i) cmax = c.channels[i] > cmax ? c.channels[i] : cmax;
    const size_t slot_bytes = (plc16_bytes(B, H, W, cmax) + 255) & ~(size_t)255;
    for (int i = 0; i < kScratchSlots; ++i) pl->scratch[i] = (uint8_t*)bump->take(slot_bytes);
    pl->scratch_next = 0;
    pl->CP_in = h->conv_in.c0_store;
    pl->xin = (float*)bump->take((size_t)B * H * W * pl->CP_in * 4);
    pl->cond = (float*)bump->take((size_t)B * c.cond_channels * 4);
    pl->film = (float*)bump->take((size_t)B * core->film_rows * 4);
    Tens xin{pl->xin, nullptr, pl->CP_in, H, W, 8};
    Tens x = tensor(c.channels[0], H, W, true);
    {
      Operand in0 = prep(xin, nullptr, 0, 0, nullptr, 0, 0, false, false, true);
      conv(h->conv_in, in0, false, 1, nullptr, x, true);
      Rec rec; rec.kind = R_CONVIN; rec.cw = &h->conv_in; rec.x = xin; rec.o = x; rec.in1 = in0; record(rec);
    }
    for (int i = 0; i <= L; ++i) {
      if (i > 0 && i < L) {
        Tens xd = tensor(c.channels[i - 1], x.H / 2, x.W / 2, true);
        Operand ind = prep(x, nullptr, 0, 0, nullptr, 0, 0, false, false);
        conv(h->downs[i], ind, false, 2, nullptr, xd, true);
        Rec rec; rec.kind = R_DOWN; rec.cw = &h->downs[i]; rec.x = x; rec.o = xd; rec.in1 = ind; record(rec);
        x = xd;
      }
      for (auto& rb : h->blocks[i]) x = resblock(rb, x, nullptr);
    }
    *feat = x;
    return err;
  }

  void resize(const Tens& src, const Tens& dst) {
    Op op; op.kind = OP_RESIZE;
    op.rs = ResizeParams{src.data ? src.data : (const float*)1, dst.data ? dst.data : (float*)1, pl->B, src.H, src.W, dst.H, dst.W, src.C,
                         dst.stats ? dst.stats : (double*)1, dst.gs};
    pl->ops.push_back(op);
  }

  int build(const dmd_denoiser* h) {
    const dmd_denoiser_config& c = h->cfg;
    const int L = c.num_levels, B = pl->B, H = pl->H, W = pl->W;
    const int div = 1 << (L - 1);
    const int Hp = (H + div - 1) / div * div, Wp = (W + div - 1) / div * div;
    const bool padded = Hp != H || Wp != W;
    if (padded && pl->train) return fail("denoiser: training at H=%d W=%d (not multiples of %d) needs the pad / crop adjoints, which are not built", H, W, div);
    int cmax = 16;
    for (int i = 0; i < L; ++i) cmax = c.channels[i] > cmax ? c.channels[i] : cmax;
    const size_t slot_bytes = (plc16_bytes(B, Hp, Wp, cmax) + 255) & ~(size_t)255;
    for (int i = 0; i < kScratchSlots; ++i) pl->scratch[i] = (uint8_t*)bump->take(slot_bytes);
    pl->scratch_next = 0;
    pl->CP_in = h->conv_in.c0_store;
    pl->xin = (float*)bump->take((size_t)B * H * W * pl->CP_in * 4);
    pl->cs = (float*)bump->take((size_t)(B + 1) * 4 * 4);
    pl->cemb = (float*)bump->take((size_t)B * c.cond_channels * 4);
    pl->chid = (float*)bump->take((size_t)B * c.cond_channels * 4);
    pl->cond = (float*)bump->take((size_t)B * c.cond_channels * 4);
    pl->film = (float*)bump->take((size_t)B * core->film_rows * 4);
    Tens xin{pl->xin, nullptr, pl->CP_in, H, W, 8};
    Tens x = tensor(c.channels[0], H, W, !padded);
    {
      Operand in = prep(xin, nullptr, 0, 0, nullptr, 0, 0, false, false, true);
      conv(h->conv_in, in, false, 1, nullptr, x, !padded);
      Rec rec; rec.kind = R_CONVIN; rec.cw = &h->conv_in; rec.x = xin; rec.o = x; rec.in1 = in; record(rec);
    }
    if (padded) {
      Tens xp = tensor(c.channels[0], Hp, Wp, true);
      resize(x, xp);
      x = xp;
    }
    std::vector<std::vector<Tens>> d_outputs;
    for (int i = 0; i < L; ++i) {
      Tens xd = x;
      if (i > 0) {
        xd = tensor(c.channels[i - 1], x.H / 2, x.W / 2, true);
        Operand in = prep(x, nullptr, 0, 0, nullptr, 0, 0, false, false);
        conv(h->downs[i], in, false, 2, nullptr, xd, true);
        Rec rec; rec.kind = R_DOWN; rec.cw = &h->downs[i]; rec.x = x; rec.o = xd; rec.in1 = in; record(rec);
      }
      std::vector<Tens> outs{xd};
      x = xd;
      for (auto& rb : h->d_blocks[i]) { x = resblock(rb, x, nullptr); outs.push_back(x); }
      d_outputs.push_back(outs);
    }
    for (auto& rb : h->mid) x = resblock(rb, x, nullptr);
    for (int m = 0; m < L; ++m) {
      Tens xu = x;
      if (m > 0) {
        xu = tensor(x.C, x.H * 2, x.W * 2, true);
        Operand in = prep(x, nullptr, 1, 0, nullptr, 0, 0, false, false);
        conv(h->ups[m], in, false, 1, nullptr, xu, true);
        Rec rec; rec.kind = R_UP; rec.cw = &h->ups[m]; rec.x = x; rec.o = xu; rec.in1 = in; record(rec);
      }
      x = xu;
      const std::vector<Tens>& skip = d_outputs[L - 1 - m];
      const int ns = (int)skip.size();
      for (size_t k = 0; k < h->u_blocks[m].size(); ++k) x = resblock(h->u_blocks[m][k], x, &skip[ns - 1 - (int)k]);
    }
    if (padded) {
      Tens xc = tensor(x.C, H, W, true);
      resize(x, xc);
      x = xc;
    }
    pl->CF = c.img_channels;
    pl->fout = (float*)bump->take((size_t)B * H * W * pl->CF * 4);
    Tens f{pl->fout, nullptr, pl->CF, H, W, pl->CF};
    {
      Operand in = prep(x, nullptr, 0, 2, nullptr, h->i_normout_w, h->i_normout_b, true, false, false);
      conv(h->conv_out, in, false, 1, nullptr, f, false);
      Rec rec; rec.kind = R_OUT; rec.cw = &h->conv_out; rec.x = x; rec.in1 = in; record(rec);
    }
    const size_t img = (size_t)B * c.img_channels * H * W * 4;
    pl->s_xc = (float*)bump->take(img); pl->s_x2 = (float*)bump->take(img); pl->s_d = (float*)bump->take(img);
    if (!pl->train) {
      const size_t K = kMaxSamplerEvals;
      pl->sig_all = (float*)bump->take(K * 4);
      pl->cemb_all = (float*)bump->take(K * B * c.cond_channels * 4); pl->chid_all = (float*)bump->take(K * B * c.cond_channels * 4);
      pl->cond_all = (float*)bump->take(K * B * c.cond_channels * 4); pl->film_all = (float*)bump->take(K * B * core->film_rows * 4);
    }
    return err;
  }
};

int make_plan(const dmd_denoiser* h, Plan* pl, int B, int H, int W, uint8_t* base, size_t* total) {
  pl->B = B; pl->H = H; pl->W = W; pl->ops.clear();
  Bump b0{nullptr}, s0{nullptr};
  { Plan tmp; tmp.B = B; tmp.H = H; tmp.W = W; PlanBuilder pb{&h->core, &tmp, &b0, &s0}; if (pb.build(h)) return 1; }
  const size_t stats_bytes = (s0.off + 255) & ~(size_t)255;
  if (total) *total = stats_bytes + b0.off + 256;
  if (!base) return 0;
  Bump sb{base}, bb{base + stats_bytes};
  pl->base = base; pl->stats = (double*)base; pl->stats_bytes = stats_bytes;
  PlanBuilder pb{&h->core, pl, &bb, &sb};
  if (pb.build(h)) return 1;
  pl->bytes = stats_bytes + bb.off;
  return 0;
}

struct BwdBuilder {
  const ModelCore* core; Plan* pl; int err = 0;
  std::vector<char> ginit;

  const float* P(int idx) const { return core->P(idx); }
  long long G(int idx) const { return core->goff[idx]; }
  bool was_init(const Tens& t) { const bool w = ginit[t.gid] != 0; ginit[t.gid] = 1; return w; }
  void push(const BOp& b) { pl->bops.push_back(b); }
  void begin() { ginit.assign(pl->n_grad_tensors, 0); pl->bops.clear(); }

  void replay(const Operand& o) { BOp b; b.kind = B_PREP; b.prep = pl->ops[o.op].prep; b.prep_nsrc = pl->ops[o.op].prep_nsrc; push(b); }
  void gprep(const float* g, int C, int Hs, int Ws, int ups, uint8_t* dst) {
    const dmd_prep_desc d = prep_desc(g, C, pl->B, Hs, Ws, ups, 0, nullptr, nullptr, nullptr, dst);
    BOp b; b.kind = B_PREP;
    if (prep_fill(&d, &b.prep, &b.prep_nsrc)) { err = 1; return; }
    push(b);
  }
  void colsum(const float* g, long long rows, int C, int Creal, int idx, int idx2 = -1) {
    BOp b; b.kind = B_COLSUM; b.src = g; b.rows = rows; b.C = C; b.Creal = Creal; b.goff = G(idx); b.goff2 = idx2 >= 0 ? G(idx2) : -1;
    push(b);
  }
  void dgrad(const ConvW& cw, int k, const uint8_t* gy, int H, int W, float* out, bool accumulate) {
    const dmd_conv_desc d = dgrad_desc(cw, k, core->packed + cw.pkT_off[k], gy, pl->B, H, W, out, accumulate);
    BOp b; b.kind = B_CONV;
    if (conv_fill(&d, &b.conv, &b.smem, &b.cols)) { err = 1; return; }
    push(b);
  }
  void wgrad(const ConvW& cw, const uint8_t* gy, const uint8_t* act, int Ca, int Cin, int ci_off, int H, int W) {
    BOp b; b.kind = B_WGRAD; b.goff = G(cw.w_idx);
    if (wgrad_fill(gy ? gy : (const void*)1, round_up(cw.Cout, 16), act ? act : (const void*)1, Ca, pl->B, H, W, cw.taps,
                   pl->partial ? pl->partial : (float*)1, cw.Cout, Cin, cw.CinReal, ci_off, pl->scale ? pl->scale + 1 : (const float*)1, 1, 0, &b.wg)) { err = 1; return; }
    push(b);
  }
  void norm_bwd(const Tens& x, const float* gy, int mode, const FilmW* film, int c_off, int ctot, int gamma_idx, int beta_idx,
                float* gx, const float* addend, bool accumulate) {
    const int R = core->film_rows;
    NormBwdParams nb = gn_bwd_params(x.data, gy, x.stats, pl->B, x.H * x.W, x.C, x.gs, P(gamma_idx), P(beta_idx), pl->nsum, gx, addend, accumulate);
    if (mode == 1) {
      nb.mode = 1; nb.gamma = nb.beta = nullptr; nb.c_off = c_off;
      nb.film = pl->film; nb.film_stride = R; nb.film_off = film->off; nb.film_ctot = ctot;
      nb.sumB = pl->dfilm ? pl->dfilm + film->off + c_off : nullptr;
      nb.sumA = pl->dfilm ? pl->dfilm + film->off + ctot + c_off : nullptr;
      nb.sum_stride = R;
    } else {
      BOp m; m.kind = B_MEMSET; m.ms_ptr = pl->nsum; m.ms_bytes = (size_t)2 * pl->B * kMaxCin * 4; push(m);
    }
    BOp b1; b1.kind = B_NORM1; b1.nb = nb;
    push(b1);
    if (mode == 2) {
      BOp a; a.kind = B_AFFINE; a.nb = nb; a.goff = G(gamma_idx); a.goff2 = G(beta_idx); push(a);
    }
    BOp b2 = b1; b2.kind = B_NORM2; push(b2);
  }

  void resblock(const Rec& r) {
    const ResBlockW& rb = *r.rb;
    const int H = r.o.H, W = r.o.W, B = pl->B;
    const long long pix = (long long)B * H * W;
    Tens o = r.o;
    if (rb.has_attn) {
      BOp b; b.kind = B_ATTN;
      b.ab = AttnBwdParams{o.data, o.stats, P(rb.an_w), P(rb.an_b), P(rb.qkv_w), P(rb.qkv_b), P(rb.op_w), r.a.grad, o.grad,
                           nullptr, nullptr, nullptr, nullptr, nullptr, nullptr, pl->scale ? pl->scale + 1 : nullptr, H * W, rb.cout, o.gs, kGnEps};
      const int ids[6] = {rb.an_w, rb.an_b, rb.qkv_w, rb.qkv_b, rb.op_w, rb.op_b};
      for (int i = 0; i < 6; ++i) b.goffs[i] = G(ids[i]);
      push(b);
      ginit[o.gid] = 1;
    }
    const Tens* src[2] = {&r.x, r.has_skip ? &r.skip : nullptr};
    const int nsrc = r.has_skip ? 2 : 1;
    gprep(o.grad, rb.cout, H, W, 0, pl->gyA);
    colsum(o.grad, pix, rb.cout, rb.cout, rb.c2.b_idx, rb.has_proj ? rb.proj.b_idx : -1);
    replay(r.in2);
    wgrad(rb.c2, pl->gyA, r.in2.n0, round_up(rb.cout, 16), rb.cout, 0, H, W);
    dgrad(rb.c2, 0, pl->gyA, H, W, pl->tA, false);
    norm_bwd(r.t, pl->tA, 1, &rb.n2, 0, rb.cout, 0, 0, pl->tB, nullptr, false);
    gprep(pl->tB, rb.cout, H, W, 0, pl->gyB);
    colsum(pl->tB, pix, rb.cout, rb.cout, rb.c1.b_idx);
    replay(r.in1);
    for (int k = 0; k < nsrc; ++k) {
      const uint8_t* act = k == 0 ? r.in1.n0 : r.in1.n1;
      wgrad(rb.c1, pl->gyB, act, round_up(src[k]->C, 16), src[k]->C, rb.c1.srcOff[k], H, W);
      float* ga = k == 0 ? pl->tA : pl->tC;
      dgrad(rb.c1, k, pl->gyB, H, W, ga, false);
      const float* addend = (!rb.has_proj && k == 0) ? o.grad : nullptr;
      const bool acc = was_init(*src[k]);
      norm_bwd(*src[k], ga, 1, &rb.n1, rb.c1.srcOff[k], rb.cin, 0, 0, src[k]->grad, addend, acc);
    }
    if (rb.has_proj) {
      for (int k = 0; k < nsrc; ++k) {
        const uint8_t* raw = k == 0 ? r.in1.r0 : r.in1.r1;
        wgrad(rb.proj, pl->gyA, raw, round_up(src[k]->C, 16), src[k]->C, rb.proj.srcOff[k], H, W);
        dgrad(rb.proj, k, pl->gyA, H, W, src[k]->grad, true);
      }
    }
  }

  int walk(int end) {
    const int B = pl->B;
    for (int i = end - 1; i >= 0; --i) {
      const Rec& r = pl->tape[i];
      if (r.kind == R_RES) {
        resblock(r);
      } else if (r.kind == R_UP) {
        const ConvW& cw = *r.cw;
        const int H = r.o.H, W = r.o.W;
        gprep(r.o.grad, cw.Cout, H, W, 0, pl->gyA);
        colsum(r.o.grad, (long long)B * H * W, cw.Cout, cw.Cout, cw.b_idx);
        replay(r.in1);
        wgrad(cw, pl->gyA, r.in1.n0, round_up(r.x.C, 16), r.x.C, 0, H, W);
        dgrad(cw, 0, pl->gyA, H, W, pl->tA, false);
        BOp b; b.kind = B_POOL; b.src = pl->tA; b.dst = r.x.grad; b.H = r.x.H; b.W = r.x.W; b.C = r.x.C; b.acc = was_init(r.x) ? 1 : 0;
        push(b);
      } else if (r.kind == R_DOWN) {
        const ConvW& cw = *r.cw;
        const int H = r.x.H, W = r.x.W;
        gprep(r.o.grad, cw.Cout, r.o.H, r.o.W, 2, pl->gyA);
        colsum(r.o.grad, (long long)B * r.o.H * r.o.W, cw.Cout, cw.Cout, cw.b_idx);
        replay(r.in1);
        wgrad(cw, pl->gyA, r.in1.n0, round_up(r.x.C, 16), r.x.C, 0, H, W);
        dgrad(cw, 0, pl->gyA, H, W, r.x.grad, was_init(r.x));
      } else if (r.kind == R_CONVIN) {
        const ConvW& cw = *r.cw;
        const int H = r.o.H, W = r.o.W;
        gprep(r.o.grad, cw.Cout, H, W, 0, pl->gyA);
        colsum(r.o.grad, (long long)B * H * W, cw.Cout, cw.Cout, cw.b_idx);
        replay(r.in1);
        wgrad(cw, pl->gyA, r.in1.n0, cw.c0_store, cw.c0_real, 0, H, W);
      } else {
        return fail("backward plan: record %d of kind %d belongs to a model's own head", i, r.kind);
      }
      if (err) return 1;
    }
    return 0;
  }

  void sgemm(const float* A, long long sam, long long sak, const float* Bm, long long sbk, long long sbn, float* C, long long c_goff,
             long long ldc, int M, int N, int K, int use_inv, int acc) {
    BOp b; b.kind = B_SGEMM; b.ga = A; b.sam = sam; b.sak = sak; b.gb = Bm; b.sbk = sbk; b.sbn = sbn; b.gc = C; b.c_goff = c_goff; b.ldc = ldc;
    b.M = M; b.N = N; b.K = K; b.use_inv = use_inv; b.acc = acc; push(b);
  }
  void film_tail() {
    const int B = pl->B, CC = core->cond_channels, R = core->film_rows;
    { BOp b; b.kind = B_FILMW; push(b); }
    const float* Wf = core->packed ? (const float*)(core->packed + core->film_w_off) : nullptr;
    sgemm(pl->dfilm, R, 1, Wf, CC, 1, pl->dcond, -1, CC, B, CC, R, 0, 0);
    {
      const long long fit = pl->tmp_floats / ((long long)B * CC);
      int splits = R / 256; if (splits > 32) splits = 32; if (splits > fit) splits = (int)fit;
      if (splits > 1) pl->bops.back().chunks = splits;
    }
  }
  void embedding(const float* de, int idx, int T, int num_actions) {
    BOp b; b.kind = B_EMB; b.src = de; b.goff = G(idx); b.C = core->cond_channels; b.emb_T = T; b.emb_actions = num_actions; push(b);
  }
};

int build_denoiser_bwd(const dmd_denoiser* h, BwdBuilder& bw) {
  Plan* pl = bw.pl;
  const int B = pl->B;
  bw.begin();
  {
    const Rec& r = pl->tape.back();
    if (r.kind != R_OUT) return fail("denoiser backward plan: the tape does not end with the output head");
    const ConvW& cw = *r.cw;
    const int H = r.x.H, W = r.x.W;
    bw.gprep(pl->gF, 8, H, W, 0, pl->gyA);
    bw.colsum(pl->gF, (long long)B * H * W, 8, cw.Cout, cw.b_idx);
    bw.replay(r.in1);
    bw.wgrad(cw, pl->gyA, r.in1.n0, round_up(r.x.C, 16), r.x.C, 0, H, W);
    bw.dgrad(cw, 0, pl->gyA, H, W, pl->tA, false);
    bw.norm_bwd(r.x, pl->tA, 2, nullptr, 0, r.x.C, h->i_normout_w, h->i_normout_b, r.x.grad, nullptr, bw.was_init(r.x));
    if (bw.err) return 1;
  }
  if (bw.walk((int)pl->tape.size() - 1)) return 1;
  bw.film_tail();
  const int CC = h->cfg.cond_channels;
  const long long* goff = h->core.goff.data();
  bw.sgemm(pl->dcond, 1, CC, pl->chid, CC, 1, nullptr, goff[h->i_cp2w], CC, CC, CC, B, 1, 1);
  bw.colsum(pl->dcond, B, CC, CC, h->i_cp2b);
  bw.sgemm(pl->dcond, CC, 1, bw.P(h->i_cp2w), CC, 1, pl->dh, -1, CC, B, CC, CC, 0, 0);
  { BOp b; b.kind = B_LINEAR; b.lin_in = pl->cemb; b.lin_w = bw.P(h->i_cp0w); b.lin_b = bw.P(h->i_cp0b); b.lin_out = pl->cpre; b.lin_K = CC; b.lin_F = CC; bw.push(b); }
  { BOp b; b.kind = B_DSILU; b.src = pl->cpre; b.ga = pl->dh; b.dst = pl->dpre; b.rows = (long long)B * CC; bw.push(b); }
  bw.sgemm(pl->dpre, 1, CC, pl->cemb, CC, 1, nullptr, goff[h->i_cp0w], CC, CC, CC, B, 1, 1);
  bw.colsum(pl->dpre, B, CC, CC, h->i_cp0b);
  bw.sgemm(pl->dpre, CC, 1, bw.P(h->i_cp0w), CC, 1, pl->de, -1, CC, B, CC, CC, 0, 0);
  bw.embedding(pl->de, h->i_actemb, h->cfg.num_steps_conditioning, h->cfg.num_actions);
  return bw.err;
}

using FwdPlanFn = std::function<int(PlanBuilder&)>;
using BwdPlanFn = std::function<int(BwdBuilder&)>;
int make_train_plan(const ModelCore& core, int cmax, int gF_ch, Plan* pl, int B, int H, int W, int T, uint8_t* base, size_t* total,
                    const FwdPlanFn& fwd, const BwdPlanFn& bwd) {
  pl->train = true; pl->n_grad_tensors = 0; pl->tape.clear();
  pl->B = B; pl->H = H; pl->W = W; pl->T = T; pl->ops.clear(); pl->bops.clear();
  Bump b0{nullptr}, s0{nullptr};
  { Plan tmp; tmp.train = true; tmp.B = B; tmp.H = H; tmp.W = W; tmp.T = T; PlanBuilder pb{&core, &tmp, &b0, &s0}; if (fwd(pb)) return 1; }
  const size_t stats_bytes = (s0.off + 255) & ~(size_t)255;
  Bump sb{base}, bb{base ? base + stats_bytes : nullptr};
  if (base) { pl->base = base; pl->stats = (double*)base; pl->stats_bytes = stats_bytes; }
  if (base) { PlanBuilder pb{&core, pl, &bb, &sb}; if (fwd(pb)) return 1; } else bb.off = b0.off;
  pl->tmp_floats = (long long)B * H * W * cmax;
  const size_t act_bytes = (size_t)pl->tmp_floats * 4;
  pl->tA = (float*)bb.take(act_bytes); pl->tB = (float*)bb.take(act_bytes); pl->tC = (float*)bb.take(act_bytes);
  const size_t op_bytes = plc16_bytes(B, H, W, cmax);
  pl->gyA = (uint8_t*)bb.take(op_bytes); pl->gyB = (uint8_t*)bb.take(op_bytes);
  pl->gF = (float*)bb.take((size_t)B * H * W * gF_ch * 4);
  if (init_kernels()) return 1;
  pl->partial = (float*)bb.take(wgrad_partial_bytes(g_num_sms));
  const int CC = core.cond_channels;
  pl->dcond = (float*)bb.take((size_t)B * CC * 4); pl->dh = (float*)bb.take((size_t)B * CC * 4); pl->cpre = (float*)bb.take((size_t)B * CC * 4);
  pl->dpre = (float*)bb.take((size_t)B * CC * 4); pl->de = (float*)bb.take((size_t)B * CC * 4);
  pl->film_woff = (long long*)bb.take((size_t)core.film_rows * 8); pl->film_boff = (long long*)bb.take((size_t)core.film_rows * 8);
  pl->scale = (float*)bb.take(256);
  uint8_t* z0 = (uint8_t*)bb.take(0);
  pl->dfilm = (float*)bb.take((size_t)B * core.film_rows * 4);
  pl->nsum = (float*)bb.take((size_t)2 * B * kMaxCin * 4);
  pl->amax = (unsigned int*)bb.take(256);
  pl->zero_begin = z0; pl->zero_bytes = base ? (size_t)((uint8_t*)pl->amax + 256 - z0) : 0;
  if (total) *total = stats_bytes + bb.off + 512;
  if (!base) return 0;
  pl->bytes = stats_bytes + bb.off;
  BwdBuilder bw{&core, pl};
  if (bwd(bw)) return 1;
  pl->film_woff_h.assign(core.film_rows, 0); pl->film_boff_h.assign(core.film_rows, 0);
  auto fill_film = [&](const FilmW& f) {
    for (int r = 0; r < 2 * f.C; ++r) { pl->film_woff_h[f.off + r] = core.goff[f.w_idx] + (long long)r * CC; pl->film_boff_h[f.off + r] = core.goff[f.b_idx] + r; }
  };
  for (const Rec& r : pl->tape) if (r.kind == R_RES) { fill_film(r.rb->n1); fill_film(r.rb->n2); }
  return 0;
}

template <class Cfg> int widest_channels(const Cfg& c) {
  int cmax = 16;
  for (int i = 0; i < c.num_levels; ++i) cmax = c.channels[i] > cmax ? c.channels[i] : cmax;
  return cmax;
}
int make_denoiser_train_plan(const dmd_denoiser* h, Plan* pl, int B, int H, int W, uint8_t* base, size_t* total) {
  return make_train_plan(h->core, widest_channels(h->cfg), 8, pl, B, H, W, 1, base, total,
                         [h](PlanBuilder& pb) { return pb.build(h); }, [h](BwdBuilder& bw) { return build_denoiser_bwd(h, bw); });
// ... 1241 lines not shown
```

### diamond_b200/csrc/conv_tc.cuh

```cuda
#pragma once
#include "ptx.cuh"

namespace dmd {

constexpr int kConvThreads = 384;
constexpr int kConvConsumerWarps = 8;
constexpr int kTileM = 128;
constexpr int kMaxCin = 128;
constexpr int kMaxSegs = 8;
constexpr int kMaxStages = 24;
constexpr int kStatSlots = 3;
constexpr int kMaxOutGroups = 4;

struct FastDiv {
  uint32_t d, m;
  __host__ void init(uint32_t dd) {
    d = dd;
    m = (uint32_t)((0x100000000ull / dd) + 1);
  }
  __device__ __forceinline__ uint32_t div(uint32_t n) const { return d == 1 ? n : __umulhi(n, m); }
};

struct Plc {
  int PW, PH, Q, G, Qalloc;
};
__host__ __device__ inline Plc plc_geometry(int B, int H, int W) {
  Plc g;
  g.PW = W + 1; g.PH = H + 1; g.Q = B * g.PH * g.PW; g.G = g.PW + 1;
  g.Qalloc = g.G + ((g.Q + kTileM - 1) / kTileM) * kTileM + kTileM + g.PW + 1;
  return g;
}

struct ConvParams {
  const uint8_t* seg_base[kMaxSegs];
  int seg_slabs[kMaxSegs];
  int nseg;
  int Cin;
  int Cextra;
  const __half* wpk_extra;
  const float* bias_extra;
  int xslabs;
  int B, H, W;
  int taps;
  int stride;
  const __half* wpk;
  const float* bias;
  int Cout, CoutPad;
  const float* resid;
  float* out;
  double* ostats;
  int ogs;
  int PW, PH, Q, G;
  unsigned long long plane_bytes;
  int P, Palloc;
  int num_tiles, stages;
  int trs;
  FastDiv dPW, dPH;
  long long* ktrace;
};

struct ConvSmemLayout {
  uint32_t bias_off, w_off, a_off, slab_bytes, total;
};

__host__ __device__ inline uint32_t conv_weight_bytes(int taps, int Cin, int Cextra, int CoutPad) {
  return (((uint32_t)taps * Cin * CoutPad * 2 + 127u) & ~127u) + (uint32_t)Cextra * CoutPad * 2;
}
__host__ __device__ inline ConvSmemLayout conv_smem_layout(uint32_t w_bytes, int Palloc, int stages) {
  ConvSmemLayout L;
  L.bias_off = 512;
  L.w_off = L.bias_off + 128 * 4;
  L.a_off = (L.w_off + w_bytes + 127u) & ~127u;
  L.slab_bytes = 2u * Palloc * 16;
  L.total = L.a_off + (uint32_t)stages * L.slab_bytes + 16;
  return L;
}

template <int N>
struct RegEpilogue {
  int lane, r0, G;
  float s[kStatSlots][kMaxOutGroups], ss[kStatSlots][kMaxOutGroups];
  int n_cur;

  __device__ __forceinline__ void init(const ConvParams& p, int row0, int lane_) {
    lane = lane_;
    r0 = row0;
    G = p.ostats ? p.Cout / p.ogs : 1;
#pragma unroll
    for (int k = 0; k < kStatSlots; ++k)
#pragma unroll
      for (int g = 0; g < kMaxOutGroups; ++g) s[k][g] = ss[k][g] = 0.f;
    n_cur = -1;
  }

  template <int kG = kMaxOutGroups>
  __device__ __forceinline__ void flush_stats(const ConvParams& p, int img0, int nslots) {
#pragma unroll
    for (int k = 0; k < kStatSlots; ++k) {
      if (k < nslots) {
        float a[kG], b[kG];
#pragma unroll
        for (int g = 0; g < kG; ++g) { a[g] = s[k][g]; b[g] = ss[k][g]; }
#pragma unroll
        for (int m = 16; m > 0; m >>= 1)
#pragma unroll
          for (int g = 0; g < kG; ++g) {
            a[g] += __shfl_xor_sync(0xffffffffu, a[g], m);
            b[g] += __shfl_xor_sync(0xffffffffu, b[g], m);
          }
        if (lane == 0 && img0 + k < p.B) {
#pragma unroll
          for (int g = 0; g < kG; ++g)
            if (g < G && (a[g] != 0.f || b[g] != 0.f)) {
              double* dst = p.ostats + ((size_t)(img0 + k) * G + g) * 2;
              atomicAdd(dst, (double)a[g]);
              atomicAdd(dst + 1, (double)b[g]);
            }
        }
      }
#pragma unroll
      for (int g = 0; g < kMaxOutGroups; ++g) s[k][g] = ss[k][g] = 0.f;
    }
  }

  template <int kLgs, bool kFull>
  __device__ __forceinline__ void tile(const ConvParams& p, const float* sbias, const float (&acc)[N / 2], int q0) {
    constexpr bool kStats = kLgs > 0;
    constexpr int kGroups = (N / 8) >> kLgs > 0 ? ((N / 8) >> kLgs < kMaxOutGroups ? (N / 8) >> kLgs : kMaxOutGroups) : 1;
    const int n_lo = (int)p.dPH.div(p.dPW.div((uint32_t)q0));
    const int q_last = min(q0 + kTileM, p.Q) - 1;
    const bool single_image = (int)p.dPH.div(p.dPW.div((uint32_t)q_last)) == n_lo;
    if (kStats && n_cur >= 0 && (!single_image || n_lo != n_cur)) { flush_stats<kGroups>(p, n_cur, 1); n_cur = -1; }
    const int c0 = 2 * (lane & 3);
    const bool vec = kFull || (p.Cout & 1) == 0;
    const bool resid = p.resid != nullptr;
    constexpr int kBatch = N / 8 < 8 ? N / 8 : 8;
    constexpr int kRows = N / 8 <= 8 ? 2 : 1;
#pragma unroll
    for (int h0 = 0; h0 < 2; h0 += kRows) {
      int opix[kRows], slot[kRows];
#pragma unroll
      for (int r = 0; r < kRows; ++r) {
        const int q = q0 + r0 + 8 * (h0 + r);
        opix[r] = -1; slot[r] = 0;
        if (q < p.Q) {
          const uint32_t R = p.dPW.div((uint32_t)q);
          const int x = q - (int)R * p.PW;
          const int n = (int)p.dPH.div(R);
          const int y = (int)R - n * p.PH;
          bool valid = (x < p.W) && (y < p.H);
          int yo = y, xo = x, Ho = p.H, Wo = p.W;
          if (!kFull && p.stride == 2) {
            valid = valid && ((x & 1) == 0) && ((y & 1) == 0);
            yo = y >> 1; xo = x >> 1; Ho = p.H >> 1; Wo = p.W >> 1;
          }
          if (valid) { opix[r] = (n * Ho + yo) * Wo + xo; slot[r] = n - n_lo; }
        }
      }
      if (kRows == 1 && opix[0] < 0) continue;
      float gs[kRows][kMaxOutGroups], gss[kRows][kMaxOutGroups];
#pragma unroll
      for (int r = 0; r < kRows; ++r)
#pragma unroll
        for (int g = 0; g < kMaxOutGroups; ++g) gs[r][g] = gss[r][g] = 0.f;
#pragma unroll
      for (int jb = 0; jb < N / 8; jb += kBatch) {
        float2 bv[kBatch], rv[kRows][kBatch];
#pragma unroll
        for (int u = 0; u < kBatch; ++u) {
          const int col = 8 * (jb + u) + c0;
          bv[u] = (kFull || col < p.Cout) ? *reinterpret_cast<const float2*>(sbias + col) : make_float2(0.f, 0.f);
#pragma unroll
          for (int r = 0; r < kRows; ++r) {
            const int h = h0 + r;
            rv[r][u] = make_float2(0.f, 0.f);
            if (resid && opix[r] >= 0 && (kFull || col < p.Cout)) {
              const float* rp = p.resid + (size_t)opix[r] * p.Cout;
              if (vec) rv[r][u] = __ldg(reinterpret_cast<const float2*>(rp + col));
              else {
                rv[r][u].x = __ldg(rp + col);
                if (col + 1 < p.Cout) rv[r][u].y = __ldg(rp + col + 1);
              }
            }
          }
        }
#pragma unroll
        for (int r = 0; r < kRows; ++r) {
          const int h = h0 + r;
          if (opix[r] < 0) continue;
          float* op = p.out + (size_t)opix[r] * p.Cout;
#pragma unroll
          for (int u = 0; u < kBatch; ++u) {
            const int j = jb + u;
            const int col = 8 * j + c0;
            if (kFull || col < p.Cout) {
              float2 o = make_float2(acc[4 * j + 2 * h] + bv[u].x, acc[4 * j + 2 * h + 1] + bv[u].y);
              if (vec) {
                if (resid) { o.x += rv[r][u].x; o.y += rv[r][u].y; }
                *reinterpret_cast<float2*>(op + col) = o;
              } else {
                if (resid) o.x += rv[r][u].x;
                op[col] = o.x;
                if (col + 1 < p.Cout) { if (resid) o.y += rv[r][u].y; op[col + 1] = o.y; } else o.y = 0.f;
              }
              if (kStats) {
                gs[r][j >> kLgs] += o.x + o.y;
                gss[r][j >> kLgs] += fmaf(o.x, o.x, o.y * o.y);
              }
            }
          }
        }
      }
      if (kStats) {
#pragma unroll
        for (int r = 0; r < kRows; ++r) {
          const int h = h0 + r;
          if (opix[r] < 0) continue;
          if (single_image) {
#pragma unroll
            for (int g = 0; g < kGroups; ++g) { s[0][g] += gs[r][g]; ss[0][g] += gss[r][g]; }
          } else {
#pragma unroll
            for (int k = 0; k < kStatSlots; ++k)
#pragma unroll
              for (int g = 0; g < kGroups; ++g) {
                s[k][g] += (slot[r] == k) ? gs[r][g] : 0.f;
                ss[k][g] += (slot[r] == k) ? gss[r][g] : 0.f;
              }
          }
        }
      }
    }
    if (kStats) {
      if (single_image) n_cur = n_lo;
      else { flush_stats<kGroups>(p, n_lo, kStatSlots); n_cur = -1; }
    }
  }

  template <bool kFull>
  __device__ __forceinline__ void tile_any(const ConvParams& p, int lgs, const float* sbias, const float (&acc)[N / 2], int q0) {
    if (lgs == 0) tile<0, kFull>(p, sbias, acc, q0);
    else if (lgs == 1 || N == 16) tile<1, kFull>(p, sbias, acc, q0);
    else if (lgs == 2 || N == 32) tile<2, kFull>(p, sbias, acc, q0);
    else if (lgs == 3 || N == 64) tile<3, kFull>(p, sbias, acc, q0);
    else tile<4, kFull>(p, sbias, acc, q0);
  }

  __device__ __forceinline__ void finish(const ConvParams& p) {
    if (p.ostats != nullptr && n_cur >= 0) flush_stats(p, n_cur, 1);
  }
};

template <int N, int kTaps>
__global__ void __launch_bounds__(kConvThreads, 1) conv_tc_kernel(const ConvParams p) {
  extern __shared__ __align__(128) uint8_t smem[];
  uint64_t* wbar = reinterpret_cast<uint64_t*>(smem);
  uint64_t* full = wbar + 1;
  uint64_t* empty = full + kMaxStages;
  const ConvSmemLayout L = conv_smem_layout(conv_weight_bytes(p.taps, p.Cin, p.Cextra, p.CoutPad), p.Palloc, p.stages);
  float* sbias = reinterpret_cast<float*>(smem + L.bias_off);
  uint8_t* sW = smem + L.w_off;
  uint8_t* sA = smem + L.a_off;

  const int tid = threadIdx.x;
  const int warp = tid >> 5, lane = tid & 31;
  const int halo = (kTaps == 9) ? (p.PW + 1) : 0;
  const int S = p.stages;
  const int main_slabs = p.Cin >> 4;
  const int kslabs = main_slabs + p.xslabs;
  const uint32_t w_main_bytes = ((uint32_t)p.taps * p.Cin * p.CoutPad * 2 + 127u) & ~127u;
  const int tiles_lo = p.num_tiles / (int)gridDim.x, tiles_rem = p.num_tiles % (int)gridDim.x;
  const int tile_begin = (int)blockIdx.x * tiles_lo + min((int)blockIdx.x, tiles_rem);
  const int my_tiles = tiles_lo + ((int)blockIdx.x < tiles_rem ? 1 : 0);

  pdl_launch_dependents();
  if (tid == 0) {
    mbar_init(wbar, 1);
    for (int s = 0; s < S; ++s) { mbar_init(full + s, 1); mbar_init(empty + s, kConvConsumerWarps); }
    fence_mbar_init();
    const uint32_t tap_bytes = (uint32_t)p.Cin * p.CoutPad * 2;
    const uint32_t extra_bytes = (uint32_t)p.Cextra * p.CoutPad * 2;
    mbar_expect_tx(wbar, tap_bytes * p.taps + extra_bytes);
    for (int t = 0; t < p.taps; ++t)
      bulk_g2s(sW + (size_t)t * tap_bytes, reinterpret_cast<const uint8_t*>(p.wpk) + (size_t)t * tap_bytes, tap_bytes, wbar);
    if (extra_bytes) bulk_g2s(sW + w_main_bytes, p.wpk_extra, extra_bytes, wbar);
  }
  for (int i = tid; i < 128; i += blockDim.x)
    sbias[i] = ((p.bias != nullptr && i < p.Cout) ? __ldg(p.bias + i) : 0.f) + ((p.bias_extra != nullptr && i < p.Cout) ? __ldg(p.bias_extra + i) : 0.f);
  __syncthreads();
  pdl_wait();
  if (blockIdx.x == 0 && tid == 128) ktrace_stamp(p.ktrace);

  if (warp < 2) {
    const uint32_t pid = (uint32_t)warp;
    const uint32_t chunk_bytes = (uint32_t)p.P * 16;
    uint32_t stage = 0, phase = 0, nslab = 0;
    for (int it = 0; it < my_tiles; ++it) {
      const size_t pos0 = (size_t)((tile_begin + it) * kTileM - halo + p.G) * 16;
      int seg = 0, seg_ks = 0;
      for (int ks = 0; ks < kslabs; ++ks, ++nslab) {
        if ((nslab & 1u) == pid) {
          mbar_wait(empty + stage, phase ^ 1u);
          if (elect_one_sync()) {
            uint8_t* slab = sA + (size_t)stage * L.slab_bytes;
            const bool xs = ks >= main_slabs;
            const uint32_t bytes = xs ? (uint32_t)kTileM * 16 : chunk_bytes;
            mbar_expect_tx(full + stage, 2 * bytes);
            const uint8_t* plane = p.seg_base[seg] + (size_t)(2 * seg_ks) * p.plane_bytes + pos0 + (xs ? (size_t)halo * 16 : 0);
            bulk_g2s(slab, plane, bytes, full + stage);
            bulk_g2s(slab + (size_t)p.Palloc * 16, plane + p.plane_bytes, bytes, full + stage);
          }
          __syncwarp();
        }
        if (++seg_ks == p.seg_slabs[seg]) { seg_ks = 0; ++seg; }
        if (++stage == (uint32_t)S) { stage = 0; phase ^= 1u; }
      }
    }
  } else if (warp >= 4) {
    const int m0 = ((warp >> 2) - 1) * 64;
    RegEpilogue<N> epi;
    epi.init(p, m0 + 16 * (warp & 3) + (lane >> 2), lane);
    const int lgs = p.ostats ? 31 - __clz(p.ogs >> 3) : 0;
    const bool full_cols = p.Cout == N && p.stride == 1;
    if (my_tiles > 0) mbar_wait(wbar, 0);
    const uint64_t hi = gmma_desc_hi(128);
    const uint32_t a_lbo = (uint32_t)p.Palloc * 16;
    const uint32_t b_lbo = (uint32_t)(p.trs ? 3 * p.CoutPad : p.CoutPad) * 16;
    const uint32_t x_lbo = (uint32_t)p.CoutPad * 16;
    const uint32_t a_lo0 = (((smem_u32(sA) + (uint32_t)m0 * 16) >> 4) & 0x3FFFu) | (((a_lbo >> 4) & 0x3FFFu) << 16);
    const uint32_t b_lo0 = ((smem_u32(sW) >> 4) & 0x3FFFu) | (((b_lbo >> 4) & 0x3FFFu) << 16);
    const uint32_t b_x0 = (((smem_u32(sW) + w_main_bytes) >> 4) & 0x3FFFu) | (((x_lbo >> 4) & 0x3FFFu) << 16);
    const uint32_t slab16 = L.slab_bytes >> 4;
    const uint32_t kstep16 = (2u * b_lbo) >> 4;
    const uint32_t xstep16 = (2u * x_lbo) >> 4;
    uint32_t shift[kTaps], b_tap[kTaps];
#pragma unroll
    for (int t = 0; t < kTaps; ++t) {
      shift[t] = (uint32_t)(halo + (kTaps == 9 ? (t / 3 - 1) * p.PW + (t % 3 - 1) : 0));
      b_tap[t] = p.trs ? ((uint32_t)(t / 3) * p.Cin * 3u * p.CoutPad * 2 + (uint32_t)(t % 3) * p.CoutPad * 16) >> 4
                       : ((uint32_t)t * p.Cin * p.CoutPad * 2) >> 4;
    }
    const int ng = p.xslabs >> 1;
    float acc[N / 2];
    uint32_t stage = 0, phase = 0, prev = 0;
    int done = 0;
    auto slab = [&](auto issue) {
      mbar_wait(full + stage, phase);
      wgmma_fence();
      issue(a_lo0 + stage * slab16);
      wgmma_commit();
      wgmma_wait<1>();
      if (done > 0 && lane == 0) mbar_arrive(empty + prev);
      prev = stage;
      ++done;
      if (++stage == (uint32_t)S) { stage = 0; phase ^= 1u; }
    };
    for (int it = 0; it < my_tiles; ++it) {
#pragma unroll
      for (int i = 0; i < N / 2; ++i) acc[i] = 0.f;
      done = 0;
      for (int ks = 0; ks < main_slabs; ++ks) {
        const uint32_t b_lo = b_lo0 + (uint32_t)ks * kstep16;
        slab([&](uint32_t a_lo) {
#pragma unroll
          for (int t = 0; t < kTaps; ++t) Wgmma<N>::template mma<0, 0>(acc, hi | (a_lo + shift[t]), hi | (b_lo + b_tap[t]), 1u);
        });
      }
      for (int g = 0; g < ng; ++g)
        slab([&](uint32_t a_lo) {
          Wgmma<N>::template mma<0, 0>(acc, hi | a_lo, hi | (b_x0 + (uint32_t)g * xstep16), 1u);
          Wgmma<N>::template mma<0, 0>(acc, hi | a_lo, hi | (b_x0 + (uint32_t)(2 * ng + g) * xstep16), 1u);
        });
      for (int g = 0; g < ng; ++g)
        slab([&](uint32_t a_lo) { Wgmma<N>::template mma<0, 0>(acc, hi | a_lo, hi | (b_x0 + (uint32_t)(ng + g) * xstep16), 1u); });
      wgmma_wait<0>();
      wgmma_fence_operands(acc);
      if (done > 0 && lane == 0) mbar_arrive(empty + prev);
      const int q0 = (tile_begin + it) * kTileM;
      if (full_cols) epi.template tile_any<true>(p, lgs, sbias, acc, q0);
      else epi.template tile_any<false>(p, lgs, sbias, acc, q0);
    }
    epi.finish(p);
  }
}

struct PrepSrc {
  const float* src;
  int C;
  int Cpad;
  const double* stats;
  int gs;
  int c_offset;
  uint8_t* dst;
  uint8_t* dst_lo;
  uint8_t* dst_raw;
  uint8_t* dst_raw_lo;
};
struct PrepParams {
  PrepSrc s[2];
  int B, Hs, Ws, ups, H, W;
  int mode;
  int act;
  const float* film;
  int film_stride, film_off, film_ctot;
  const float* gamma;
  const float* beta;
  float eps;
  int PW, PH, Q, G, Qalloc;
  unsigned long long plane_bytes;
  int pos_per_block;
  FastDiv dPW, dPH;
  long long* ktrace;
};

constexpr int kPrepThreads = 256;
constexpr int kPrepBatch = 2;

__device__ __forceinline__ uint4 pack_lo8(const float (&v)[8], const uint4& hi) {
  const __half2* h = reinterpret_cast<const __half2*>(&hi);
  uint4 lo;
  uint32_t* l = reinterpret_cast<uint32_t*>(&lo);
#pragma unroll
  for (int k = 0; k < 4; ++k) {
    const float2 f = __half22float2(h[k]);
    l[k] = pack_h2(v[2 * k] - f.x, v[2 * k + 1] - f.y);
  }
  return lo;
}

__global__ void __launch_bounds__(kPrepThreads, 4) prep_act_kernel(const PrepParams p) {
  __shared__ float sa[2][kMaxCin], sb[2][kMaxCin];
  __shared__ float smr[2][4][2];
  pdl_launch_dependents();
  pdl_wait();
  if (blockIdx.x == 0 && blockIdx.z == 0 && threadIdx.x == 0) ktrace_stamp(p.ktrace);
  const PrepSrc& S = p.s[blockIdx.z];
  const int nch = S.Cpad >> 3;
  const int pa0 = blockIdx.x * p.pos_per_block;
  const int q_first = pa0 - p.G;
  const int n0 = q_first > 0 ? (int)p.dPH.div(p.dPW.div((uint32_t)min(q_first, p.Q - 1))) : 0;
  const int pstep = kPrepThreads / nch;
  const int j = threadIdx.x % nch;
  int pl = threadIdx.x / nch;
  int x, y, n;
  {
    const int q = pa0 + pl - p.G;
    const int qq = q < 0 ? 0 : q;
    const uint32_t R = p.dPW.div((uint32_t)qq);
    x = qq - (int)R * p.PW; n = (int)p.dPH.div(R); y = (int)R - n * p.PH;
    if (q < 0) x += q;
  }
  const bool has_data = j * 8 < S.C;
  float4 v0[kPrepBatch], v1[kPrepBatch];
  int meta[kPrepBatch];
  size_t off[kPrepBatch];
  auto load_batch = [&]() {
#pragma unroll
    for (int u = 0; u < kPrepBatch; ++u) {
      const int pa = pa0 + pl + u * pstep;
      meta[u] = -2;
      if (pl + u * pstep < p.pos_per_block && pa < p.Qalloc) {
        meta[u] = -1;
        off[u] = (size_t)j * p.plane_bytes + (size_t)pa * 16;
        if (has_data && x >= 0 && x < p.W && y < p.H && n < p.B) {
          const int ys = p.ups ? (y >> 1) : y, xs = p.ups ? (x >> 1) : x;
          const float4* gp = reinterpret_cast<const float4*>(S.src + (((size_t)n * p.Hs + ys) * p.Ws + xs) * S.C + j * 8);
          v0[u] = __ldg(gp); v1[u] = __ldg(gp + 1);
          meta[u] = (n - n0) | (j << 8);
        }
      }
      x += pstep;
      while (x >= p.PW) { x -= p.PW; if (++y == p.PH) { y = 0; ++n; } }
    }
  };
  load_batch();
  if (p.mode != 0) {
    const int G = S.C / S.gs;
    if (threadIdx.x < 2 * G) {
      const int slot = threadIdx.x / G, g = threadIdx.x - slot * G;
      const int n = n0 + slot;
      float mean_f = 0.f, rstd_f = 0.f;
      if (n < p.B) {
        const double* st = S.stats + ((size_t)n * G + g) * 2;
        const double cnt = (double)p.Hs * p.Ws * S.gs;
        const double mean = st[0] / cnt;
        double var = st[1] / cnt - mean * mean;
        var = var > 0.0 ? var : 0.0;
        mean_f = (float)mean;
        rstd_f = (float)(1.0 / sqrt(var + (double)p.eps));
      }
      smr[slot][g][0] = mean_f;
      smr[slot][g][1] = rstd_f;
    }
    float sc[2] = {0.f, 0.f}, sh[2] = {0.f, 0.f};
#pragma unroll
    for (int k = 0; k < 2; ++k) {
      const int e = threadIdx.x + k * kPrepThreads;
      if (e < 2 * S.C) {
        const int slot = e / S.C, c = e - slot * S.C;
        const int n = n0 + slot, cg = S.c_offset + c;
        if (n < p.B) {
          if (p.mode == 1) {
            const float* f = p.film + (size_t)n * p.film_stride + p.film_off;
            sc[k] = 1.f + __ldg(f + cg);
            sh[k] = __ldg(f + p.film_ctot + cg);
          } else {
            sc[k] = __ldg(p.gamma + cg);
            sh[k] = __ldg(p.beta + cg);
          }
        }
      }
    }
    __syncthreads();
#pragma unroll
    for (int k = 0; k < 2; ++k) {
      const int e = threadIdx.x + k * kPrepThreads;
      if (e < 2 * S.C) {
        const int slot = e / S.C, c = e - slot * S.C;
        const float mean = smr[slot][c / S.gs][0], rstd = smr[slot][c / S.gs][1];
        const float a = rstd * sc[k];
        sa[slot][c] = a;
        sb[slot][c] = sh[k] - mean * a;
      }
    }
    __syncthreads();
  }
  for (;;) {
#pragma unroll
    for (int u = 0; u < kPrepBatch; ++u) {
      if (meta[u] == -2) continue;
      uint4 packed = make_uint4(0u, 0u, 0u, 0u), raw = packed, packed_lo = packed, raw_lo = packed;
      if (meta[u] >= 0) {
        const int slot = meta[u] & 0xff, j = meta[u] >> 8;
        float v[8] = {v0[u].x, v0[u].y, v0[u].z, v0[u].w, v1[u].x, v1[u].y, v1[u].z, v1[u].w};
        if (S.dst_raw != nullptr) {
          raw.x = pack_h2(v[0], v[1]); raw.y = pack_h2(v[2], v[3]); raw.z = pack_h2(v[4], v[5]); raw.w = pack_h2(v[6], v[7]);
          if (S.dst_raw_lo != nullptr) raw_lo = pack_lo8(v, raw);
        }
        if (p.mode != 0) {
          const float4* ca = reinterpret_cast<const float4*>(&sa[slot][j * 8]);
          const float4* cb = reinterpret_cast<const float4*>(&sb[slot][j * 8]);
          const float4 a0 = ca[0], a1 = ca[1], b0 = cb[0], b1 = cb[1];
          v[0] = fmaf(a0.x, v[0], b0.x); v[1] = fmaf(a0.y, v[1], b0.y); v[2] = fmaf(a0.z, v[2], b0.z); v[3] = fmaf(a0.w, v[3], b0.w);
          v[4] = fmaf(a1.x, v[4], b1.x); v[5] = fmaf(a1.y, v[5], b1.y); v[6] = fmaf(a1.z, v[6], b1.z); v[7] = fmaf(a1.w, v[7], b1.w);
        }
        if (p.act) {
#pragma unroll
          for (int k = 0; k < 8; ++k) v[k] = silu_f(v[k]);
        }
        packed.x = pack_h2(v[0], v[1]); packed.y = pack_h2(v[2], v[3]); packed.z = pack_h2(v[4], v[5]); packed.w = pack_h2(v[6], v[7]);
        if (S.dst_lo != nullptr) packed_lo = pack_lo8(v, packed);
      }
      *reinterpret_cast<uint4*>(S.dst + off[u]) = packed;
      if (S.dst_lo != nullptr) *reinterpret_cast<uint4*>(S.dst_lo + off[u]) = packed_lo;
      if (S.dst_raw != nullptr) *reinterpret_cast<uint4*>(S.dst_raw + off[u]) = raw;
      if (S.dst_raw_lo != nullptr) *reinterpret_cast<uint4*>(S.dst_raw_lo + off[u]) = raw_lo;
    }
    pl += kPrepBatch * pstep;
    if (pl >= p.pos_per_block) break;
    load_batch();
  }
}

template <int NCH, bool RAW>
__global__ void __launch_bounds__(kPrepThreads, 4) prep_fast_kernel(const PrepParams p) {
  __shared__ float sa[2][kMaxCin], sb[2][kMaxCin];
  __shared__ float smr[2][4][2];
  constexpr int PSTEP = kPrepThreads / NCH;
  constexpr int kBatch = 4;
  pdl_launch_dependents();
  pdl_wait();
  if (blockIdx.x == 0 && blockIdx.z == 0 && threadIdx.x == 0) ktrace_stamp(p.ktrace);
  const PrepSrc& S = p.s[blockIdx.z];
  const int pa0 = blockIdx.x * p.pos_per_block;
  const int q_first = pa0 - p.G;
  const int n0 = q_first > 0 ? (int)p.dPH.div(p.dPW.div((uint32_t)min(q_first, p.Q - 1))) : 0;
  const int j = threadIdx.x & (NCH - 1);
  int pl = threadIdx.x / NCH;
  int x, y, n;
  {
    const int q = pa0 + pl - p.G;
    const int qq = q < 0 ? 0 : q;
    const uint32_t R = p.dPW.div((uint32_t)qq);
    x = qq - (int)R * p.PW; n = (int)p.dPH.div(R); y = (int)R - n * p.PH;
    if (q < 0) x += q;
  }
  const bool has_data = j * 8 < S.C;
  {
    const int G = S.C / S.gs;
    if (threadIdx.x < 2 * G) {
      const int slot = threadIdx.x / G, g = threadIdx.x - slot * G;
      const int ni = n0 + slot;
      float mean_f = 0.f, rstd_f = 0.f;
      if (ni < p.B) {
        const double* st = S.stats + ((size_t)ni * G + g) * 2;
        const double cnt = (double)p.Hs * p.Ws * S.gs;
        const double mean = st[0] / cnt;
        double var = st[1] / cnt - mean * mean;
        var = var > 0.0 ? var : 0.0;
        mean_f = (float)mean;
        rstd_f = (float)(1.0 / sqrt(var + (double)p.eps));
      }
      smr[slot][g][0] = mean_f;
      smr[slot][g][1] = rstd_f;
    }
    float sc[2] = {0.f, 0.f}, sh[2] = {0.f, 0.f};
#pragma unroll
    for (int k = 0; k < 2; ++k) {
      const int e = threadIdx.x + k * kPrepThreads;
      if (e < 2 * S.C) {
        const int slot = e / S.C, c = e - slot * S.C;
        const int ni = n0 + slot, cg = S.c_offset + c;
        if (ni < p.B) {
          if (p.mode == 1) {
            const float* f = p.film + (size_t)ni * p.film_stride + p.film_off;
            sc[k] = 1.f + __ldg(f + cg);
            sh[k] = __ldg(f + p.film_ctot + cg);
          } else {
            sc[k] = __ldg(p.gamma + cg);
            sh[k] = __ldg(p.beta + cg);
          }
        }
      }
    }
    __syncthreads();
#pragma unroll
    for (int k = 0; k < 2; ++k) {
      const int e = threadIdx.x + k * kPrepThreads;
      if (e < 2 * S.C) {
        const int slot = e / S.C, c = e - slot * S.C;
        const float mean = smr[slot][c / S.gs][0], rstd = smr[slot][c / S.gs][1];
        const float a = rstd * sc[k];
        sa[slot][c] = a;
        sb[slot][c] = sh[k] - mean * a;
      }
    }
    __syncthreads();
  }
  uint8_t* const d_n = S.dst + (size_t)j * p.plane_bytes + (size_t)pa0 * 16;
  uint8_t* const d_r = RAW ? S.dst_raw + (size_t)j * p.plane_bytes + (size_t)pa0 * 16 : nullptr;
  uint8_t* const d_rl = RAW ? S.dst_raw_lo + (size_t)j * p.plane_bytes + (size_t)pa0 * 16 : nullptr;
  const int limit = min(p.pos_per_block, p.Qalloc - pa0);
  const uint4 zero4 = make_uint4(0u, 0u, 0u, 0u);
  for (; pl < limit; pl += kBatch * PSTEP) {
    float4 v0[kBatch], v1[kBatch];
    int slot[kBatch];
#pragma unroll
    for (int u = 0; u < kBatch; ++u) {
      slot[u] = -1;
      if (pl + u * PSTEP < limit && has_data && x >= 0 && x < p.W && y < p.H && n < p.B) {
        const uint32_t idx = (uint32_t)((n * p.Hs + y) * p.Ws + x) * (uint32_t)S.C + (uint32_t)(j * 8);
        const float4* gp = reinterpret_cast<const float4*>(S.src + idx);
        v0[u] = __ldg(gp); v1[u] = __ldg(gp + 1);
        slot[u] = n - n0;
      }
      x += PSTEP;
      while (x >= p.PW) { x -= p.PW; if (++y == p.PH) { y = 0; ++n; } }
    }
#pragma unroll
    for (int u = 0; u < kBatch; ++u) {
      const int pp = pl + u * PSTEP;
      if (pp >= limit) break;
      uint4 packed = zero4, raw = zero4, raw_lo = zero4;
      if (slot[u] >= 0) {
        const float4* pa4 = reinterpret_cast<const float4*>(&sa[slot[u]][j * 8]);
        const float4* pb4 = reinterpret_cast<const float4*>(&sb[slot[u]][j * 8]);
        const float4 a0 = pa4[0], a1 = pa4[1], b0 = pb4[0], b1 = pb4[1];
        const float ca[8] = {a0.x, a0.y, a0.z, a0.w, a1.x, a1.y, a1.z, a1.w};
        const float cb[8] = {b0.x, b0.y, b0.z, b0.w, b1.x, b1.y, b1.z, b1.w};
        float v[8] = {v0[u].x, v0[u].y, v0[u].z, v0[u].w, v1[u].x, v1[u].y, v1[u].z, v1[u].w};
        if (RAW) {
          raw.x = pack_h2(v[0], v[1]); raw.y = pack_h2(v[2], v[3]); raw.z = pack_h2(v[4], v[5]); raw.w = pack_h2(v[6], v[7]);
          raw_lo = pack_lo8(v, raw);
        }
#pragma unroll
        for (int k = 0; k < 8; ++k) v[k] = silu_f(fmaf(ca[k], v[k], cb[k]));
        packed.x = pack_h2(v[0], v[1]); packed.y = pack_h2(v[2], v[3]); packed.z = pack_h2(v[4], v[5]); packed.w = pack_h2(v[6], v[7]);
      }
      *reinterpret_cast<uint4*>(d_n + (size_t)pp * 16) = packed;
      if (RAW) {
        *reinterpret_cast<uint4*>(d_r + (size_t)pp * 16) = raw;
        *reinterpret_cast<uint4*>(d_rl + (size_t)pp * 16) = raw_lo;
      }
    }
  }
}

__global__ void __launch_bounds__(256) zero_insert_prep_kernel(const PrepParams p) {
  pdl_launch_dependents();
  pdl_wait();
  const PrepSrc& S = p.s[0];
  const int nch = S.Cpad >> 3;
  const long long idx = (long long)blockIdx.x * blockDim.x + threadIdx.x;
  const long long total = (long long)p.Qalloc * nch;
  if (idx >= total) return;
  const int j = (int)(idx % nch);
  const int pa = (int)(idx / nch);
  uint4 packed = make_uint4(0u, 0u, 0u, 0u);
  const int q = pa - p.G;
  if (q >= 0 && q < p.Q && j * 8 < S.C) {
    const uint32_t R = p.dPW.div((uint32_t)q);
    const int x = q - (int)R * p.PW;
    const int n = (int)p.dPH.div(R);
    const int y = (int)R - n * p.PH;
    if (x < p.W && y < p.H && ((x | y) & 1) == 0) {
      const float4* gp = reinterpret_cast<const float4*>(S.src + (((size_t)n * p.Hs + (y >> 1)) * p.Ws + (x >> 1)) * S.C + j * 8);
      const float4 a = __ldg(gp), b = __ldg(gp + 1);
      packed.x = pack_h2(a.x, a.y); packed.y = pack_h2(a.z, a.w); packed.z = pack_h2(b.x, b.y); packed.w = pack_h2(b.z, b.w);
    }
  }
  *reinterpret_cast<uint4*>(S.dst + (size_t)j * p.plane_bytes + (size_t)pa * 16) = packed;
}

}
```

### diamond_b200/ops.py

```python
import ctypes as C
from typing import Optional, Tuple

import torch
from torch import Tensor

from . import _lib


def _cuda(*ts):
    for t in ts:
        if t is not None and not (t.is_cuda and t.is_contiguous()):
            raise RuntimeError("diamond_b200 ops need contiguous CUDA tensors (no CPU fallback)")


def round_up(x: int, m: int) -> int:
    return (x + m - 1) // m * m


def nchw_to_nhwc(x: Tensor, cpad: Optional[int] = None) -> Tensor:
    _cuda(x)
    b, c, h, w = x.shape
    cp = cpad or c
    out = torch.empty(b, h, w, cp, device=x.device, dtype=torch.float32)
    _lib.check(_lib.lib().dmd_nchw_to_nhwc(x.data_ptr(), out.data_ptr(), b, c, cp, h * w, _lib.current_stream()))
    return out


def nhwc_to_nchw(x: Tensor, c: Optional[int] = None) -> Tensor:
    _cuda(x)
    b, h, w, cp = x.shape
    c = c or cp
    out = torch.empty(b, c, h, w, device=x.device, dtype=torch.float32)
    _lib.check(_lib.lib().dmd_nhwc_to_nchw(x.data_ptr(), out.data_ptr(), b, c, cp, h * w, _lib.current_stream()))
    return out


def pack_conv_weight(w: Tensor, cin_pad: int, c0_real: Optional[int] = None, c0_store: Optional[int] = None,
                     precise: bool = False, trs: bool = False) -> Tuple[Tensor, int]:
    _cuda(w)
    cout, cin, kh, kw = w.shape
    taps = kh * kw
    cout_pad = round_up(cout, 16)
    c0_real = cin if c0_real is None else c0_real
    c0_store = c0_real if c0_store is None else c0_store
    out = torch.empty(taps * cin_pad * cout_pad * (3 if precise else 1), device=w.device, dtype=torch.float16)
    _lib.check(_lib.lib().dmd_pack_conv_weight(w.data_ptr(), out.data_ptr(), cout, cout_pad, cin, cin_pad, taps,
                                              c0_real, c0_store, 3 if trs else int(precise), _lib.current_stream()))
    return out, cout_pad


def gn_stats(x: Tensor, gs: int) -> Tensor:
    _cuda(x)
    b, h, w, c = x.shape
    st = torch.zeros(b, c // gs, 2, device=x.device, dtype=torch.float64)
    _lib.check(_lib.lib().dmd_gn_stats(x.data_ptr(), st.data_ptr(), b, h * w, c, gs, _lib.current_stream()))
    return st


def prep_act(src0: Tensor, *, src1: Optional[Tensor] = None, upsample: bool = False, mode: int = 0, silu: bool = False,
             stats0: Optional[Tensor] = None, stats1: Optional[Tensor] = None, gs0: int = 0, gs1: int = 0,
             film: Optional[Tensor] = None, film_off: int = 0, gamma: Optional[Tensor] = None, beta: Optional[Tensor] = None,
             eps: float = 1e-5, also_raw: bool = False, split: bool = False, raw_split: bool = False):
    _cuda(src0, src1, stats0, stats1, film, gamma, beta)
    if raw_split and not also_raw:
        raise ValueError("raw_split needs also_raw")
    lib = _lib.lib()
    b, hs, ws, c0 = src0.shape
    h, w = (2 * hs, 2 * ws) if upsample else (hs, ws)
    c1 = src1.shape[3] if src1 is not None else 0

    def buf(c):
        return torch.empty(lib.dmd_plc16_bytes(b, h, w, c), dtype=torch.uint8, device=src0.device)

    n0, n1 = buf(c0), (buf(c1) if c1 else None)
    r0, r1 = (buf(c0) if also_raw else None), (buf(c1) if (also_raw and c1) else None)
    d = _lib.PrepDesc()
    d.src0, d.src1, d.C0, d.C1 = src0.data_ptr(), _lib.ptr(src1), c0, c1
    d.B, d.Hs, d.Ws, d.upsample, d.mode, d.silu = b, hs, ws, int(upsample), mode, int(silu)
    d.stats0, d.stats1, d.gs0, d.gs1 = _lib.ptr(stats0), _lib.ptr(stats1), gs0, gs1
    d.film, d.film_stride, d.film_off = _lib.ptr(film), (film.shape[1] if film is not None else 0), film_off
    d.gamma, d.beta, d.eps = _lib.ptr(gamma), _lib.ptr(beta), eps
    d.dst0, d.dst1, d.dst_raw0, d.dst_raw1 = n0.data_ptr(), _lib.ptr(n1), _lib.ptr(r0), _lib.ptr(r1)
    l0, l1 = (buf(c0) if split else None), (buf(c1) if (split and c1) else None)
    d.dst_lo0, d.dst_lo1 = _lib.ptr(l0), _lib.ptr(l1)
    rl0, rl1 = (buf(c0) if raw_split else None), (buf(c1) if (raw_split and c1) else None)
    d.dst_raw_lo0, d.dst_raw_lo1 = _lib.ptr(rl0), _lib.ptr(rl1)
    _lib.check(lib.dmd_prep_act(C.byref(d), _lib.current_stream()))
    if raw_split:
        return n0, n1, r0, r1, h, w, l0, l1, rl0, rl1
    if split:
        return n0, n1, r0, r1, h, w, l0, l1
    return n0, n1, r0, r1, h, w


def conv2d_operand(n0: Tensor, n1: Optional[Tensor], c0: int, c1: int, b: int, h: int, w: int, wpk: Tensor, cout: int,
                   cout_pad: int, taps: int = 9, *, bias: Optional[Tensor] = None, stride: int = 1,
                   residual: Optional[Tensor] = None, out_gs: int = 0, out: Optional[Tensor] = None,
                   ostats: Optional[Tensor] = None, debug: int = 0, debug_buf: Optional[Tensor] = None,
                   lo0: Optional[Tensor] = None, lo1: Optional[Tensor] = None, xproj=None, trs: bool = False):
    _cuda(n0, n1, wpk, bias, residual)
    ho, wo = h // stride, w // stride
    if out is None:
        out = torch.empty(b, ho, wo, cout, device=n0.device, dtype=torch.float32)
    if ostats is None and out_gs:
        ostats = torch.zeros(b, cout // out_gs, 2, device=n0.device, dtype=torch.float64)
    d = _lib.ConvDesc()
    d.src0, d.src1, d.C0, d.C1 = n0.data_ptr(), _lib.ptr(n1), c0, c1
    d.B, d.H, d.W, d.taps, d.stride = b, h, w, taps, stride
    d.wpk, d.bias, d.Cout, d.CoutPad = wpk.data_ptr(), _lib.ptr(bias), cout, cout_pad
    d.residual, d.out, d.out_stats, d.out_gs, d.debug = _lib.ptr(residual), out.data_ptr(), _lib.ptr(ostats), out_gs, debug
    d.debug_buf = _lib.ptr(debug_buf)
    d.precise, d.src0_lo, d.src1_lo = int(lo0 is not None), _lib.ptr(lo0), _lib.ptr(lo1)
    d.wpk_layout = int(trs)
    if xproj is not None:
        xh0, xh1, xl0, xl1, xc0, xc1, wpk_x, bias_x = xproj
        d.xsrc0, d.xsrc1, d.xsrc0_lo, d.xsrc1_lo = xh0.data_ptr(), _lib.ptr(xh1), xl0.data_ptr(), _lib.ptr(xl1)
        d.xC0, d.xC1, d.wpk_x, d.bias_x = xc0, xc1, wpk_x.data_ptr(), _lib.ptr(bias_x)
    _lib.check(_lib.lib().dmd_conv2d_fprop(C.byref(d), _lib.current_stream()))
    return out, ostats


def conv2d_fprop(src0: Tensor, wpk: Tensor, cout: int, cout_pad: int, cin_pad: int, taps: int = 9, *,
                 src1: Optional[Tensor] = None, bias: Optional[Tensor] = None, upsample: bool = False, stride: int = 1,
                 prologue: int = 0, silu: bool = False, stats0: Optional[Tensor] = None, stats1: Optional[Tensor] = None,
                 gs0: int = 0, gs1: int = 0, film: Optional[Tensor] = None, film_off: int = 0,
                 gamma: Optional[Tensor] = None, beta: Optional[Tensor] = None, eps: float = 1e-5,
                 residual: Optional[Tensor] = None, out_gs: int = 0, debug: int = 0, debug_buf: Optional[Tensor] = None,
                 precise: bool = False, trs: bool = False) -> Tuple[Tensor, Optional[Tensor]]:
    res = prep_act(src0, src1=src1, upsample=upsample, mode=prologue, silu=silu, stats0=stats0, stats1=stats1,
                   gs0=gs0, gs1=gs1, film=film, film_off=film_off, gamma=gamma, beta=beta, eps=eps, split=precise)
    n0, n1, _, _, h, w = res[:6]
    lo0, lo1 = (res[6], res[7]) if precise else (None, None)
    c0, c1 = round_up(src0.shape[3], 16), (round_up(src1.shape[3], 16) if src1 is not None else 0)
    if c0 + c1 != cin_pad:
        raise ValueError(f"operand channels {c0}+{c1} do not match the packed weights ({cin_pad})")
    return conv2d_operand(n0, n1, c0, c1, src0.shape[0], h, w, wpk, cout, cout_pad, taps, bias=bias, stride=stride,
                          residual=residual, out_gs=out_gs, debug=debug, debug_buf=debug_buf, lo0=lo0, lo1=lo1, trs=trs)


def attn_fwd(x: Tensor, stats_in: Tensor, gamma: Tensor, beta: Tensor, wqkv: Tensor, bqkv: Tensor, wout: Tensor,
             bout: Tensor, gs: int, eps: float = 1e-5, want_stats: bool = True) -> Tuple[Tensor, Optional[Tensor]]:
    _cuda(x, stats_in, gamma, beta, wqkv, bqkv, wout, bout)
    b, h, w, c = x.shape
    out = torch.empty_like(x)
    ostats = torch.zeros(b, c // gs, 2, device=x.device, dtype=torch.float64) if want_stats else None
    _lib.check(_lib.lib().dmd_attn_fwd(x.data_ptr(), stats_in.data_ptr(), gamma.data_ptr(), beta.data_ptr(),
                                       wqkv.data_ptr(), bqkv.data_ptr(), wout.data_ptr(), bout.data_ptr(), out.data_ptr(),
                                       _lib.ptr(ostats), b, h * w, c, gs, eps, _lib.current_stream()))
    return out, ostats



def linear(x: Tensor, w: Tensor, bias: Optional[Tensor] = None, *, out: Optional[Tensor] = None, silu: bool = False,
           accumulate: bool = False, hw_perm: int = 0) -> Tensor:
    _cuda(x, w, bias, out)
    b, k, f = x.shape[0], x[0].numel(), w.shape[0]
    if out is None:
        if accumulate:
            raise ValueError("accumulate needs out")
        out = torch.empty(b, f, device=x.device, dtype=torch.float32)
    _lib.check(_lib.lib().dmd_linear(x.data_ptr(), w.data_ptr(), _lib.ptr(bias), out.data_ptr(), b, k, f, int(silu), int(accumulate),
                                     hw_perm, _lib.current_stream()))
    return out


def maxpool2_stats(x: Tensor, y: Tensor, stats: Optional[Tensor] = None, gs: int = 0) -> Tensor:
    _cuda(x, y, stats)
    b, h, w, c = x.shape
    _lib.check(_lib.lib().dmd_maxpool2_stats(x.data_ptr(), y.data_ptr(), _lib.ptr(stats), b, h, w, c, gs, _lib.current_stream()))
    return y


def lstm_gates(gates: Tensor, c_in: Tensor, h_out: Tensor, c_out: Tensor) -> Tuple[Tensor, Tensor]:
    _cuda(gates, c_in, h_out, c_out)
    b, hd = c_in.shape
    _lib.check(_lib.lib().dmd_lstm_gates(gates.data_ptr(), c_in.data_ptr(), h_out.data_ptr(), c_out.data_ptr(), b, hd, _lib.current_stream()))
    return h_out, c_out


def resize_nhwc(x: Tensor, out: Tensor, stats: Optional[Tensor] = None, gs: int = 0) -> Tensor:
    _cuda(x, out, stats)
    b, h, w, c = x.shape
    _lib.check(_lib.lib().dmd_resize_nhwc(x.data_ptr(), out.data_ptr(), b, h, w, out.shape[1], out.shape[2], c, _lib.ptr(stats), gs,
                                          _lib.current_stream()))
    return out


def pack_conv_weight_T(w: Tensor, ci_off: int = 0, cin_k: Optional[int] = None) -> Tuple[Tensor, int, int]:
    _cuda(w)
    cout, cin, kh, kw = w.shape
    cin_k = cin - ci_off if cin_k is None else cin_k
    cin_p, cout_p = round_up(cout, 16), round_up(cin_k, 16)
    out = torch.empty(kh * kw * cin_p * cout_p, device=w.device, dtype=torch.float16)
    _lib.check(_lib.lib().dmd_pack_conv_weight_dgrad(w.data_ptr(), out.data_ptr(), cout, cin, ci_off, cin_k, kh * kw, _lib.current_stream()))
    return out, cin_p, cout_p


_partial = {}


def conv2d_wgrad(grad_op: Tensor, cg: int, act_op: Tensor, ca: int, b: int, h: int, w: int, cout: int, cin: int, taps: int = 9, *,
                 dw: Optional[Tensor] = None, cin_tot: Optional[int] = None, ci_off: int = 0, inv_scale: Optional[Tensor] = None,
                 accumulate: bool = False, debug: int = 0) -> Tensor:
    _cuda(grad_op, act_op)
    lib = _lib.lib()
    cin_tot = cin if cin_tot is None else cin_tot
    if dw is None:
        dw = torch.zeros(cout, cin_tot, taps, device=grad_op.device, dtype=torch.float32)
    key = grad_op.device.index
    if key not in _partial:
        _partial[key] = torch.empty(lib.dmd_wgrad_partial_bytes(), dtype=torch.uint8, device=grad_op.device)
    part = _partial[key]
    d = _lib.WgradDesc()
    d.grad, d.act, d.Cg, d.Ca, d.B, d.H, d.W, d.taps = grad_op.data_ptr(), act_op.data_ptr(), cg, ca, b, h, w, taps
    d.dW, d.Cout, d.Cin, d.CinTot, d.ci_off = dw.data_ptr(), cout, cin, cin_tot, ci_off
    d.inv_scale, d.accumulate, d.partial, d.partial_bytes, d.debug = _lib.ptr(inv_scale), int(accumulate), part.data_ptr(), part.numel(), debug
    _lib.check(lib.dmd_conv2d_wgrad(C.byref(d), _lib.current_stream()))
    return dw



def _inv(inv_scale):
    return _lib.ptr(inv_scale)


def norm_bwd(x: Tensor, gy: Tensor, stats: Tensor, gs: int, gx: Tensor, sum_a: Tensor, sum_b: Tensor, sum_stride: int, *, mode: int,
             act: bool = True, film: Optional[Tensor] = None, film_off: int = 0, film_ctot: int = 0, c_off: int = 0,
             gamma: Optional[Tensor] = None, beta: Optional[Tensor] = None, eps: float = 1e-5, addend: Optional[Tensor] = None,
             accumulate: bool = False, dgamma: Optional[Tensor] = None, dbeta: Optional[Tensor] = None,
             inv_scale: Optional[Tensor] = None) -> None:
    _cuda(x, gy, stats, gx, film, gamma, beta, addend)
    lib = _lib.lib()
    b, c = x.shape[0], x.shape[-1]
    d = _lib.NormBwdDesc()
    d.x, d.gy, d.stats, d.B, d.HW, d.C, d.gs = x.data_ptr(), gy.data_ptr(), stats.data_ptr(), b, x.numel() // (b * c), c, gs
    d.mode, d.act = mode, int(act)
    d.film, d.film_stride, d.film_off, d.film_ctot, d.c_off = _lib.ptr(film), (film.shape[1] if film is not None else 0), film_off, film_ctot, c_off
    d.gamma, d.beta, d.eps = _lib.ptr(gamma), _lib.ptr(beta), eps
    d.sumA, d.sumB, d.sum_stride = sum_a.data_ptr(), sum_b.data_ptr(), sum_stride
    d.gx, d.addend, d.accumulate = gx.data_ptr(), _lib.ptr(addend), int(accumulate)
    st = _lib.current_stream()
    _lib.check(lib.dmd_norm_bwd(C.byref(d), 1, st))
    if dgamma is not None:
        _lib.check(lib.dmd_norm_affine_grad(C.byref(d), dgamma.data_ptr(), dbeta.data_ptr(), _inv(inv_scale), st))
    _lib.check(lib.dmd_norm_bwd(C.byref(d), 2, st))


def attn_bwd(x: Tensor, stats_in: Tensor, gamma: Tensor, beta: Tensor, wqkv: Tensor, bqkv: Tensor, wout: Tensor, gout: Tensor, gs: int,
             pgrads: Tuple[Tensor, ...], inv_scale: Optional[Tensor] = None, eps: float = 1e-5) -> Tensor:
    _cuda(x, stats_in, gamma, beta, wqkv, bqkv, wout, gout, *pgrads)
    b, h, w, c = x.shape
    gx = torch.empty_like(x)
    _lib.check(_lib.lib().dmd_attn_bwd(x.data_ptr(), stats_in.data_ptr(), gamma.data_ptr(), beta.data_ptr(), wqkv.data_ptr(),
                                       bqkv.data_ptr(), wout.data_ptr(), gout.data_ptr(), gx.data_ptr(), *[t.data_ptr() for t in pgrads],
                                       _inv(inv_scale), b, h * w, c, gs, eps, _lib.current_stream()))
    return gx


def sgemm(a: Tensor, sam: int, sak: int, bm: Tensor, sbk: int, sbn: int, c: Tensor, ldc: int, m: int, n: int, k: int, *,
          alpha: Optional[Tensor] = None, accumulate: bool = False, chunks: int = 0) -> Tensor:
    _cuda(a, bm, c, alpha)
    lib = _lib.lib()
    nf = lib.dmd_sgemm_partial_floats(m, n, k, chunks)
    part = torch.empty(max(nf, 1), device=c.device, dtype=torch.float32) if nf else None
    _lib.check(lib.dmd_sgemm(a.data_ptr(), sam, sak, bm.data_ptr(), sbk, sbn, c.data_ptr(), ldc, m, n, k, _lib.ptr(alpha),
                             int(accumulate), chunks, _lib.ptr(part), _lib.current_stream()))
    return c


def film_wgrad(dfilm: Tensor, cond: Tensor, grads: Tensor, woff: Tensor, boff: Tensor, inv_scale: Optional[Tensor] = None) -> Tensor:
    _cuda(dfilm, cond, grads, woff, boff)
    b, rows = dfilm.shape
    _lib.check(_lib.lib().dmd_film_wgrad(dfilm.data_ptr(), cond.data_ptr(), grads.data_ptr(), woff.data_ptr(), boff.data_ptr(), b, rows,
                                         cond.shape[1], _inv(inv_scale), _lib.current_stream()))
    return grads


def embedding_bwd(de: Tensor, act: Tensor, de_table: Tensor, inv_scale: Optional[Tensor] = None) -> Tensor:
    _cuda(de, act, de_table)
    b, t = act.shape
    _lib.check(_lib.lib().dmd_embedding_bwd(de.data_ptr(), act.data_ptr(), de_table.data_ptr(), b, de.shape[1], t, de_table.shape[0],
                                            _inv(inv_scale), _lib.current_stream()))
    return de_table


def colsum(x: Tensor, out: Tensor, out2: Optional[Tensor] = None, inv_scale: Optional[Tensor] = None, creal: Optional[int] = None) -> Tensor:
    _cuda(x, out, out2)
    rows, c = x.shape
    _lib.check(_lib.lib().dmd_colsum(x.data_ptr(), out.data_ptr(), _lib.ptr(out2), _inv(inv_scale), rows, c,
                                     c if creal is None else creal, _lib.current_stream()))
    return out


def sumpool2(inp: Tensor, out: Tensor, accumulate: bool = False) -> Tensor:
    _cuda(inp, out)
    b, h, w, c = out.shape
    _lib.check(_lib.lib().dmd_sumpool2(inp.data_ptr(), out.data_ptr(), b, h, w, c, int(accumulate), _lib.current_stream()))
    return out


def dsilu_mul(pre: Tensor, dh: Tensor) -> Tensor:
    _cuda(pre, dh)
    out = torch.empty_like(pre)
    _lib.check(_lib.lib().dmd_dsilu_mul(pre.data_ptr(), dh.data_ptr(), out.data_ptr(), pre.numel(), _lib.current_stream()))
    return out


def maxpool2_bwd(y: Tensor, gp: Tensor) -> Tensor:
    _cuda(y, gp)
    b, h, w, c = y.shape
    gy = torch.empty_like(y)
    _lib.check(_lib.lib().dmd_maxpool2_bwd(y.data_ptr(), gp.data_ptr(), gy.data_ptr(), b, h, w, c, _lib.current_stream()))
    return gy


def lstm_cell_bwd(gates: Tensor, c_in: Tensor, g_h: Optional[Tensor], g_c: Optional[Tensor]) -> Tuple[Tensor, Tensor]:
    _cuda(gates, c_in, g_h, g_c)
    b, hd = c_in.shape
    dgates, gc = torch.empty_like(gates), torch.empty_like(c_in)
    _lib.check(_lib.lib().dmd_lstm_cell_bwd(gates.data_ptr(), c_in.data_ptr(), _lib.ptr(g_h), _lib.ptr(g_c), dgates.data_ptr(),
                                            gc.data_ptr(), b, hd, _lib.current_stream()))
    return dgates, gc


def heads_bwd(g_hx: Optional[Tensor], g_logits: Optional[Tensor], g_val: Optional[Tensor], hx_out: Tensor, wa: Tensor, wc: Tensor,
              dba: Tensor, dwc: Tensor, dbc: Tensor) -> Tensor:
    _cuda(g_hx, g_logits, g_val, hx_out, wa, wc, dba, dwc, dbc)
    b, hd = hx_out.shape
    g_h = torch.empty_like(hx_out)
    _lib.check(_lib.lib().dmd_heads_bwd(_lib.ptr(g_hx), _lib.ptr(g_logits), _lib.ptr(g_val), hx_out.data_ptr(), wa.data_ptr(),
                                        wc.data_ptr(), g_h.data_ptr(), dba.data_ptr(), dwc.data_ptr(), dbc.data_ptr(), b, hd,
                                        wa.shape[0], _lib.current_stream()))
    return g_h


def loss_scale(g: Tensor) -> Tensor:
    _cuda(g)
    amax = torch.zeros(1, device=g.device, dtype=torch.int32)
    scale = torch.empty(2, device=g.device, dtype=torch.float32)
    _lib.check(_lib.lib().dmd_loss_scale(g.data_ptr(), g.numel(), amax.data_ptr(), scale.data_ptr(), _lib.current_stream()))
    return scale
```

### include/diamond_b200.h

```cpp
#ifndef DIAMOND_B200_H_
#define DIAMOND_B200_H_

#include <stddef.h>
#include <stdint.h>

#ifdef __cplusplus
extern "C" {
#endif

#define DMD_VERSION 100
#define DMD_LOSS_SCALE_EXP 8

int dmd_version(void);
const char* dmd_last_error(void);
long long dmd_launch_count(int reset);
int dmd_ktrace_begin(int capacity);
int dmd_ktrace_end(long long* stamps, int capacity);
const char* dmd_ktrace_name(int i);


int dmd_pack_conv_weight(const float* w, void* wpk, int Cout, int CoutPad, int CinReal, int Cin, int taps,
                         int c0_real, int c0_store, int precise, void* stream);

size_t dmd_plc16_bytes(int B, int H, int W, int C);

typedef struct dmd_prep_desc {
  const float* src0;
  const float* src1;
  int C0, C1;
  int B, Hs, Ws;
  int upsample;
  int mode;
  int silu;
  const double* stats0;
  const double* stats1;
  int gs0, gs1;
  const float* film;
  int film_stride, film_off;
  const float* gamma;
  const float* beta;
  float eps;
  void* dst0;
  void* dst1;
  void* dst_raw0;
  void* dst_raw1;
  void* dst_lo0;
  void* dst_lo1;
  void* dst_raw_lo0;
  void* dst_raw_lo1;
} dmd_prep_desc;

int dmd_prep_act(const dmd_prep_desc* d, void* stream);

typedef struct dmd_conv_desc {
  const void* src0;
  const void* src1;
  int C0, C1;
  int B, H, W;
  int taps;
  int stride;
  const void* wpk;
  const float* bias;
  int Cout, CoutPad;
  const float* residual;
  float* out;
  double* out_stats;
  int out_gs;
  int debug;
  void* debug_buf;
  int precise;
  int wpk_layout;
  const void* src0_lo;
  const void* src1_lo;
  const void* xsrc0; const void* xsrc1; const void* xsrc0_lo; const void* xsrc1_lo;
  int xC0, xC1;
  const void* wpk_x;
  const float* bias_x;
} dmd_conv_desc;

int dmd_conv2d_fprop(const dmd_conv_desc* d, void* stream);

int dmd_pack_conv_weight_dgrad(const float* w, void* wpk, int CoutF, int CinTotF, int ci_off, int CinK, int taps, void* stream);

typedef struct dmd_wgrad_desc {
  const void* grad;
  const void* act;
  int Cg, Ca;
  int B, H, W;
  int taps;
  float* dW;
  int Cout, Cin, CinTot, ci_off;
  const float* inv_scale;
  int accumulate;
  void* partial;
  size_t partial_bytes;
  int debug;
} dmd_wgrad_desc;
size_t dmd_wgrad_partial_bytes(void);
int dmd_conv2d_wgrad(const dmd_wgrad_desc* d, void* stream);

typedef struct dmd_conv_plan_info {
  int tiles;
  int kslabs;
  int stages;
  int acc_cols;
  unsigned long long smem_bytes;
  unsigned long long weight_bytes;
} dmd_conv_plan_info;
int dmd_conv_plan(const dmd_conv_desc* d, dmd_conv_plan_info* out);
int dmd_prep_plan(const dmd_prep_desc* d, int* blocks, int* pos_per_block, int* sources);

int dmd_gn_stats(const float* x, double* stats, int B, int HW, int C, int gs, void* stream);

int dmd_attn_fwd(const float* x, const double* stats_in, const float* gamma, const float* beta, const float* wqkv,
                 const float* bqkv, const float* wout, const float* bout, float* out, double* out_stats, int B, int L,
                 int C, int gs, float eps, void* stream);
size_t dmd_attn_scratch_bytes(int B, int L, int C);
int dmd_attn_fwd_scratch(const float* x, const double* stats_in, const float* gamma, const float* beta, const float* wqkv,
                         const float* bqkv, const float* wout, const float* bout, float* out, double* out_stats, int B, int L,
                         int C, int gs, float eps, void* scratch, size_t scratch_bytes, void* stream);

int dmd_nchw_to_nhwc(const float* in, float* out, int B, int C, int CP, int HW, void* stream);
int dmd_nhwc_to_nchw(const float* in, float* out, int B, int C, int CP, int HW, void* stream);

int dmd_linear(const float* in, const float* W, const float* bias, float* out, int B, int K, int F, int silu, int accumulate,
               int hw_perm, void* stream);
int dmd_maxpool2_stats(const float* x, float* y, double* stats, int B, int H, int W, int C, int gs, void* stream);
int dmd_lstm_gates(const float* gates, const float* c_in, float* h_out, float* c_out, int B, int Hd, void* stream);
int dmd_resize_nhwc(const float* src, float* dst, int B, int Hs, int Ws, int Hd, int Wd, int C, double* stats, int gs, void* stream);


typedef struct dmd_norm_bwd_desc {
  const float* x;
  const float* gy;
  const double* stats;
  int B, HW, C, gs;
  int mode;
  int act;
  const float* film;
  int film_stride, film_off, film_ctot, c_off;
  const float* gamma;
  const float* beta;
  float eps;
  float* sumA;
  float* sumB;
  int sum_stride;
  float* gx;
  const float* addend;
  int accumulate;
} dmd_norm_bwd_desc;
int dmd_norm_bwd(const dmd_norm_bwd_desc* d, int pass, void* stream);
int dmd_norm_affine_grad(const dmd_norm_bwd_desc* d, float* dgamma, float* dbeta, const float* inv_scale, void* stream);

int dmd_attn_bwd(const float* x, const double* stats_in, const float* gamma, const float* beta, const float* wqkv, const float* bqkv,
                 const float* wout, const float* gout, float* gx, float* dgamma, float* dbeta, float* dwqkv, float* dbqkv,
                 float* dwout, float* dbout, const float* inv_scale, int B, int L, int C, int gs, float eps, void* stream);

long long dmd_sgemm_partial_floats(int M, int N, int K, int chunks);
int dmd_sgemm(const float* A, long long sam, long long sak, const float* B, long long sbk, long long sbn, float* C, long long ldc,
              int M, int N, int K, const float* alpha, int accumulate, int chunks, float* partial, void* stream);

int dmd_film_wgrad(const float* dfilm, const float* cond, float* grads, const long long* woff, const long long* boff, int B, int rows,
                   int CC, const float* inv_scale, void* stream);
int dmd_embedding_bwd(const float* de, const int64_t* act, float* dE, int B, int CC, int T, int num_actions, const float* inv_scale,
                      void* stream);
int dmd_colsum(const float* x, float* out, float* out2, const float* inv_scale, long long rows, int C, int Creal, void* stream);
int dmd_sumpool2(const float* in, float* out, int B, int H, int W, int C, int accumulate, void* stream);
int dmd_dsilu_mul(const float* pre, const float* dh, float* out, long long n, void* stream);
int dmd_maxpool2_bwd(const float* y, const float* gp, float* gy, int B, int H, int W, int C, void* stream);
int dmd_lstm_cell_bwd(const float* gates, const float* c_in, const float* g_h, const float* g_c, float* dgates, float* g_c_in,
                      int B, int Hd, void* stream);
int dmd_heads_bwd(const float* g_hx, const float* g_logits, const float* g_val, const float* hx_out, const float* Wa, const float* Wc,
                  float* g_h, float* dba, float* dWc, float* dbc, int B, int Hd, int A, void* stream);
int dmd_loss_scale(const float* g, long long n, unsigned int* amax, float* scale, void* stream);

#define DMD_MAX_LEVELS 8

typedef struct dmd_denoiser_config {
  int img_channels;
  int num_steps_conditioning;
  int cond_channels;
  int num_levels;
  int depths[DMD_MAX_LEVELS];
  int channels[DMD_MAX_LEVELS];
  int attn_depths[DMD_MAX_LEVELS];
  int num_actions;
  float sigma_data;
  float sigma_offset_noise;
} dmd_denoiser_config;

typedef struct dmd_denoiser dmd_denoiser;

#define DMD_FRAME_KINDS 3
typedef struct dmd_u8_frames {
  const uint8_t* levels;
  long long batch_stride;
  long long frame_stride;
  const uint8_t* kinds;
  long long kind_batch_stride;
  long long kind_frame_stride;
  const float* table;
} dmd_u8_frames;

dmd_denoiser* dmd_denoiser_create(const dmd_denoiser_config* cfg);
void dmd_denoiser_destroy(dmd_denoiser* h);

int dmd_denoiser_num_tensors(const dmd_denoiser* h);
size_t dmd_denoiser_packed_bytes(const dmd_denoiser* h);
int dmd_denoiser_set_weights(dmd_denoiser* h, const float* const* ptrs_host, int n_ptrs, void* packed, void* stream);

size_t dmd_denoiser_workspace_bytes(const dmd_denoiser* h, int B, int H, int W);

int dmd_denoiser_forward(dmd_denoiser* h, int B, int H, int W, const float* noisy, const float* sigma,
                         int sigma_is_scalar, const float* obs, const int64_t* act, float* out_model,
                         float* out_denoised, void* workspace, size_t workspace_bytes, void* stream);

int dmd_inner_model_forward(dmd_denoiser* h, int B, int H, int W, const float* noisy_rescaled, const float* c_noise,
                            int c_noise_is_scalar, const float* obs_rescaled, const int64_t* act, float* out,
                            void* workspace, size_t workspace_bytes, void* stream);

size_t dmd_denoiser_train_workspace_bytes(const dmd_denoiser* h, int B, int H, int W);
long long dmd_denoiser_grad_layout(const dmd_denoiser* h, long long* offsets, long long* numels, int n);
int dmd_inner_model_forward_train(dmd_denoiser* h, int B, int H, int W, const float* noisy_rescaled, const float* c_noise,
                                  int c_noise_is_scalar, const float* obs_rescaled, const int64_t* act, float* out,
                                  void* workspace, size_t workspace_bytes, void* stream);
int dmd_denoiser_backward(dmd_denoiser* h, int B, int H, int W, const float* grad_out, float* grads, long long grads_numel,
                          void* workspace, void* stream);

int dmd_inner_model_forward_u8(dmd_denoiser* h, int B, int H, int W, const float* noisy_rescaled, const float* c_noise,
                               int c_noise_is_scalar, const dmd_u8_frames* obs, const int64_t* act, float* out,
                               void* workspace, size_t workspace_bytes, void* stream);
int dmd_inner_model_forward_train_u8(dmd_denoiser* h, int B, int H, int W, const float* noisy_rescaled, const float* c_noise,
                                     int c_noise_is_scalar, const dmd_u8_frames* obs, const int64_t* act, float* out,
                                     void* workspace, size_t workspace_bytes, void* stream);

typedef struct dmd_sampler_config {
  int num_sigmas;
  const float* sigmas_host;
  int order;
  float s_churn, s_tmin, s_tmax, s_noise;
} dmd_sampler_config;

int dmd_sampler_sample(dmd_denoiser* h, const dmd_sampler_config* sc, int B, int H, int W, const float* prev_obs,
                       const int64_t* prev_act, int ring_head, float* traj, const float* eps, float* out_x, void* workspace,
                       size_t workspace_bytes, int use_graph, void* stream);

typedef struct dmd_actor_critic_config {
  int lstm_dim;
  int img_channels;
  int img_size;
  int num_levels;
  int channels[DMD_MAX_LEVELS];
  int down[DMD_MAX_LEVELS];
  int num_actions;
} dmd_actor_critic_config;

typedef struct dmd_actor_critic dmd_actor_critic;

dmd_actor_critic* dmd_actor_critic_create(const dmd_actor_critic_config* cfg);
void dmd_actor_critic_destroy(dmd_actor_critic* h);
int dmd_actor_critic_num_tensors(const dmd_actor_critic* h);
size_t dmd_actor_critic_packed_bytes(const dmd_actor_critic* h);
int dmd_actor_critic_set_weights(dmd_actor_critic* h, const float* const* ptrs_host, int n_ptrs, void* packed, void* stream);
size_t dmd_actor_critic_workspace_bytes(const dmd_actor_critic* h, int B);
int dmd_actor_critic_forward(dmd_actor_critic* h, int B, const float* obs, const float* hx_in, const float* cx_in,
                             float* logits, float* val, float* hx_out, float* cx_out, void* workspace,
                             size_t workspace_bytes, void* stream);

size_t dmd_actor_critic_backward_scratch_bytes(const dmd_actor_critic* h, int B);
long long dmd_actor_critic_grad_layout(const dmd_actor_critic* h, long long* offsets, long long* numels, int n);
int dmd_actor_critic_backward(dmd_actor_critic* h, int B, const float* hx_in, const float* cx_in, const float* hx_out,
                              const float* g_logits, const float* g_val, const float* g_hx, const float* g_cx, float* grads,
                              long long grads_numel, float* g_hx_in, float* g_cx_in, void* workspace, void* scratch,
                              size_t scratch_bytes, void* stream);
int dmd_actor_critic_backward_accumulate(dmd_actor_critic* h, int B, const float* hx_in, const float* cx_in, const float* hx_out,
                                         const float* g_logits, const float* g_val, const float* g_hx, const float* g_cx,
                                         float* grads, long long grads_numel, float* g_hx_in, float* g_cx_in, void* workspace,
                                         void* scratch, size_t scratch_bytes, void* stream);

int dmd_lambda_returns(const float* rew, const int64_t* end, const int64_t* trunc, const float* val_bootstrap, float* out, int B,
                       int T, double gamma, double lambda_, void* stream);

typedef struct dmd_rew_end_config {
  int lstm_dim;
  int img_channels;
  int img_size;
  int cond_channels;
  int num_levels;
  int depths[DMD_MAX_LEVELS];
  int channels[DMD_MAX_LEVELS];
  int attn_depths[DMD_MAX_LEVELS];
  int num_actions;
} dmd_rew_end_config;
typedef struct dmd_rew_end dmd_rew_end;
dmd_rew_end* dmd_rew_end_create(const dmd_rew_end_config* cfg);
void dmd_rew_end_destroy(dmd_rew_end* h);
int dmd_rew_end_num_tensors(const dmd_rew_end* h);
size_t dmd_rew_end_packed_bytes(const dmd_rew_end* h);
int dmd_rew_end_set_weights(dmd_rew_end* h, const float* const* ptrs_host, int n_ptrs, void* packed, void* stream);
size_t dmd_rew_end_workspace_bytes(const dmd_rew_end* h, int rows);
int dmd_rew_end_predict(dmd_rew_end* h, int b, int t, const float* obs, const float* next_obs, const int64_t* act,
                        const float* hx_in, const float* cx_in, float* logits_rew, float* logits_end, float* hx_out,
                        float* cx_out, void* workspace, size_t workspace_bytes, void* stream);

size_t dmd_rew_end_train_workspace_bytes(const dmd_rew_end* h, int b, int t);
long long dmd_rew_end_grad_layout(const dmd_rew_end* h, long long* offsets, long long* numels, int n);
int dmd_rew_end_forward_train(dmd_rew_end* h, int b, int t, const float* obs, const float* next_obs, const int64_t* act,
                              const float* hx_in, const float* cx_in, float* logits_rew, float* logits_end, float* hx_out,
                              float* cx_out, void* workspace, size_t workspace_bytes, void* stream);
int dmd_rew_end_backward(dmd_rew_end* h, int b, int t, const float* g_logits_rew, const float* g_logits_end,
                         const float* g_hx_out, const float* g_cx_out, float* grads, long long grads_numel,
                         float* g_hx_in, float* g_cx_in, void* workspace, void* stream);
int dmd_rew_end_predict_u8(dmd_rew_end* h, int b, int t, const dmd_u8_frames* obs, const dmd_u8_frames* next_obs,
                           const int64_t* act, const float* hx_in, const float* cx_in, float* logits_rew, float* logits_end,
                           float* hx_out, float* cx_out, void* workspace, size_t workspace_bytes, void* stream);
int dmd_rew_end_forward_train_u8(dmd_rew_end* h, int b, int t, const dmd_u8_frames* obs, const dmd_u8_frames* next_obs,
                                 const int64_t* act, const float* hx_in, const float* cx_in, float* logits_rew,
                                 float* logits_end, float* hx_out, float* cx_out, void* workspace, size_t workspace_bytes,
                                 void* stream);

typedef struct dmd_optim_tensor {
  float* param;
  float* grad;
  float* exp_avg;
  float* exp_avg_sq;
  long long numel;
  double weight_decay;
} dmd_optim_tensor;
size_t dmd_grad_norm_partial_bytes(const dmd_optim_tensor* table_host, int n);
int dmd_grad_norm_clip(const dmd_optim_tensor* table_host, int n, double max_norm, int clip, float* norm_coef, void* partial,
                       size_t partial_bytes, void* stream);
int dmd_adamw_step(const dmd_optim_tensor* table_host, int n, double lr, double beta1, double beta2, double eps, double step,
                   void* stream);

#ifdef __cplusplus
}
#endif
#endif
```

Before: 6652.

## Run stride-2 downsample convs at output resolution via parity-split operand planes

Adds a parity-split prep mode that writes the input into four parity planes at half resolution. The 3x3 stride-2 conv can then run over output positions only, with tap shifts remapped across the sub-planes. The intent is to stop computing and discarding the three quarters of full-resolution positions a stride-2 conv does not need. It also adds a flag that trims tail tiles covering only padding in inference, at the cost of larger shared-memory slabs, bigger scratch slots and an extra prep path.

```diff
diff --git a/diamond_b200/_lib.py b/diamond_b200/_lib.py
--- a/diamond_b200/_lib.py
+++ b/diamond_b200/_lib.py
@@ -22,7 +22,7 @@
 class ConvDesc(C.Structure):
     _fields_ = [
         ("src0", _vp), ("src1", _vp), ("C0", _i), ("C1", _i), ("B", _i), ("H", _i), ("W", _i), ("taps", _i), ("stride", _i),
-        ("wpk", _vp), ("bias", _vp), ("Cout", _i), ("CoutPad", _i),
+        ("flags", _i), ("wpk", _vp), ("bias", _vp), ("Cout", _i), ("CoutPad", _i),
         ("residual", _vp), ("out", _vp), ("out_stats", _vp), ("out_gs", _i), ("debug", _i), ("debug_buf", _vp),
         ("precise", _i), ("wpk_layout", _i), ("src0_lo", _vp), ("src1_lo", _vp),
         ("xsrc0", _vp), ("xsrc1", _vp), ("xsrc0_lo", _vp), ("xsrc1_lo", _vp), ("xC0", _i), ("xC1", _i), ("wpk_x", _vp), ("bias_x", _vp),
diff --git a/diamond_b200/csrc/api.cu b/diamond_b200/csrc/api.cu
--- a/diamond_b200/csrc/api.cu
+++ b/diamond_b200/csrc/api.cu
@@ -126,6 +126,18 @@
   return r;
 }
 
+static int conv_ring_stages(uint32_t w_bytes, int Palloc, int subs, int kslabs) {
+  const ConvSmemLayout L0 = conv_smem_layout(w_bytes, Palloc, 0, subs);
+  const long long budget = 227ll * 1024 - (long long)L0.total;
+  int stages = budget > 0 ? (int)(budget / (long long)L0.slab_bytes) : 0;
+  if (stages > 4 * kslabs) stages = 4 * kslabs;
+  return stages > kMaxStages ? kMaxStages : stages;
+}
+static bool conv_s2_fits(int H, int W, int Cin, int CoutPad) {
+  if (H % 2 || W % 2 || (H / 2 + 1) * (W / 2 + 1) < 64) return false;
+  return conv_ring_stages(conv_weight_bytes(9, Cin, 0, CoutPad), (kTileM + W / 2 + 2) | 1, 4, Cin / 16) >= 2;
+}
+
 static int conv_fill(const dmd_conv_desc* d, ConvParams* p, size_t* smem, int* acc_cols) {
   DMD_CHECK(d->src0 && d->out && d->wpk, "conv: null src0/out/wpk");
   DMD_CHECK(d->taps == 9 || d->taps == 1, "conv: taps must be 1 or 9 (got %d)", d->taps);
@@ -135,6 +147,12 @@
   DMD_CHECK((d->C1 == 0) == (d->src1 == nullptr), "conv: src1/C1 mismatch");
   if (d->precise) DMD_CHECK(d->src0_lo && ((d->C1 == 0) == (d->src1_lo == nullptr)), "conv: precise mode needs the low operand parts");
   DMD_CHECK(d->CoutPad % 16 == 0 && d->CoutPad >= 16 && d->CoutPad <= 128 && d->Cout <= d->CoutPad && d->Cout > 0, "conv: bad Cout=%d CoutPad=%d", d->Cout, d->CoutPad);
+  DMD_CHECK((d->flags & ~(DMD_CONV_NO_PAD_TAIL | DMD_CONV_S2_PLANES)) == 0, "conv: unknown flags 0x%x", d->flags);
+  const bool s2 = (d->flags & DMD_CONV_S2_PLANES) != 0;
+  if (s2) {
+    DMD_CHECK(d->stride == 2 && d->taps == 9 && !d->precise && d->C1 == 0 && !d->wpk_x, "conv: DMD_CONV_S2_PLANES is a single-source, non-split 3x3 stride-2 conv without a fused projection");
+    DMD_CHECK(conv_s2_fits(d->H, d->W, d->C0, d->CoutPad), "conv: H=%d W=%d Cin=%d CoutPad=%d does not fit the output-resolution stride-2 launch", d->H, d->W, d->C0, d->CoutPad);
+  }
   memset(p, 0, sizeof(*p));
   {
     const uint8_t* hi[2] = {(const uint8_t*)d->src0, (const uint8_t*)d->src1};
@@ -164,17 +182,17 @@
     }
     p->nseg = n;
   }
-  p->B = d->B; p->H = d->H; p->W = d->W; p->taps = d->taps; p->stride = d->stride;
-  if (d->stride == 2) DMD_CHECK(p->H % 2 == 0 && p->W % 2 == 0, "conv: stride 2 needs even H,W");
+  if (d->stride == 2) DMD_CHECK(d->H % 2 == 0 && d->W % 2 == 0, "conv: stride 2 needs even H,W");
+  p->s2 = s2; p->B = d->B; p->H = s2 ? d->H / 2 : d->H; p->W = s2 ? d->W / 2 : d->W; p->taps = d->taps; p->stride = s2 ? 1 : d->stride;
   p->wpk = reinterpret_cast<const __half*>(d->wpk); p->bias = d->bias; p->Cout = d->Cout; p->CoutPad = d->CoutPad;
   p->resid = d->residual; p->out = d->out; p->ostats = d->out_stats; p->ogs = d->out_gs > 0 ? d->out_gs : d->Cout;
-  const Plc g = plc_geometry(d->B, d->H, d->W);
+  const Plc g = plc_geometry(p->B, p->H, p->W);
   p->PW = g.PW; p->PH = g.PH; p->Q = g.Q; p->G = g.G; p->plane_bytes = (unsigned long long)g.Qalloc * 16;
   DMD_CHECK((long long)g.Q * (g.PW > g.PH ? g.PW : g.PH) < (1ll << 32), "conv: problem too large for 32-bit position math");
   p->trs = d->wpk_layout == 1 ? 1 : 0;
   if (p->trs) DMD_CHECK(d->taps == 9 && !d->precise && 3 * d->CoutPad <= 256, "conv: row-stacked weights need a 3x3, non-split conv with CoutPad <= 80");
   const int halo = d->taps == 9 ? g.PW + 1 : 0;
-  p->P = kTileM + 2 * halo; p->Palloc = p->P | 1;
+  p->P = kTileM + (s2 ? 1 : 2) * halo; p->Palloc = p->P | 1;
   if (d->out_stats) {
     const int L4 = d->Cout / 4;
     DMD_CHECK(g.PH * g.PW >= 64, "conv: image too small for the statistics epilogue (a tile may touch at most %d images)", kStatSlots);
@@ -184,16 +202,16 @@
   }
   p->dPW.init(g.PW); p->dPH.init(g.PH);
   p->num_tiles = (g.Q + kTileM - 1) / kTileM;
+  if (d->flags & DMD_CONV_NO_PAD_TAIL) {
+    const int e = p->stride;
+    p->num_tiles = (((d->B - 1) * g.PH + p->H - e) * g.PW + p->W - e) / kTileM + 1;
+  }
   const int kslabs = p->Cin / 16 + p->xslabs;
   const uint32_t w_bytes = conv_weight_bytes(p->taps, p->Cin, p->Cextra, p->CoutPad);
-  const ConvSmemLayout L0 = conv_smem_layout(w_bytes, p->Palloc, 0);
-  const long long budget = 227ll * 1024 - (long long)L0.total;
-  int stages = budget > 0 ? (int)(budget / (long long)L0.slab_bytes) : 0;
-  if (stages > 4 * kslabs) stages = 4 * kslabs;
-  if (stages > kMaxStages) stages = kMaxStages;
+  const int stages = conv_ring_stages(w_bytes, p->Palloc, s2 ? 4 : 1, kslabs);
   DMD_CHECK(stages >= 2, "conv: shared memory too small for W=%d Cin=%d CoutPad=%d", p->W, p->Cin, p->CoutPad);
   p->stages = stages;
-  *smem = conv_smem_layout(w_bytes, p->Palloc, stages).total;
+  *smem = conv_smem_layout(w_bytes, p->Palloc, stages, s2 ? 4 : 1).total;
   *acc_cols = d->CoutPad <= 16 ? 16 : (d->CoutPad <= 32 ? 32 : (d->CoutPad <= 64 ? 64 : 128));
   return 0;
 }
@@ -259,7 +277,7 @@
   if (init_kernels()) return 1;
   const int grid = p0.num_tiles < g_num_sms ? p0.num_tiles : g_num_sms;
   ConvParams p = p0;
-  p.ktrace = kt_slot(p.taps == 9 ? "conv3x3" : "conv1x1", p.num_tiles, (p.Cin + p.Cextra) * 1000 + p.W);
+  p.ktrace = kt_slot(p.s2 ? "conv3x3s2" : (p.taps == 9 ? "conv3x3" : "conv1x1"), p.num_tiles, (p.Cin + p.Cextra) * 1000 + p.W);
   if (p.taps == 9) return launch_pdl(conv_tc_kernel<kCols, 9>, dim3(grid), dim3(kConvThreads), smem, st, p);
   return launch_pdl(conv_tc_kernel<kCols, 1>, dim3(grid), dim3(kConvThreads), smem, st, p);
 }
@@ -289,9 +307,11 @@
     DMD_CHECK(d->upsample == 0, "prep: norm + upsample unsupported");
   }
   p->B = d->B; p->Hs = d->Hs; p->Ws = d->Ws; p->ups = d->upsample;
-  DMD_CHECK(d->upsample >= 0 && d->upsample <= 2, "prep: upsample must be 0, 1 (nearest 2x) or 2 (zero insertion)");
-  DMD_CHECK(d->upsample != 2 || (d->mode == 0 && !d->silu && d->C1 == 0 && !d->dst_raw0 && !d->dst_lo0), "prep: zero insertion is a raw single-source operand");
-  p->H = d->upsample ? 2 * d->Hs : d->Hs; p->W = d->upsample ? 2 * d->Ws : d->Ws;
+  DMD_CHECK(d->upsample >= 0 && d->upsample <= 3, "prep: upsample must be 0, 1 (nearest 2x), 2 (zero insertion) or 3 (parity split)");
+  DMD_CHECK(d->upsample < 2 || (d->mode == 0 && !d->silu && d->C1 == 0 && !d->dst_raw0 && !d->dst_lo0), "prep: zero insertion and the parity split are raw single-source operands");
+  DMD_CHECK(d->upsample != 3 || (d->Hs % 2 == 0 && d->Ws % 2 == 0), "prep: the parity split needs even Hs, Ws");
+  DMD_CHECK(d->upsample != 3 || (long long)d->B * (d->Hs + 2) * (d->Ws + 2) * d->C0 < (1ll << 33), "prep: problem too large for the parity split's 32-bit thread index");
+  p->H = d->upsample == 3 ? d->Hs / 2 : (d->upsample ? 2 * d->Hs : d->Hs); p->W = d->upsample == 3 ? d->Ws / 2 : (d->upsample ? 2 * d->Ws : d->Ws);
   p->mode = d->mode; p->act = d->silu ? 1 : 0;
   p->film = d->film; p->film_stride = d->film_stride; p->film_off = d->film_off; p->film_ctot = d->C0 + d->C1;
   p->gamma = d->gamma; p->beta = d->beta; p->eps = d->eps;
@@ -312,6 +332,10 @@
 static int prep_launch(const PrepParams& p0, int nsrc, cudaStream_t st) {
   PrepParams p = p0;
   p.ktrace = kt_slot("prep", (p.Qalloc + p.pos_per_block - 1) / p.pos_per_block * nsrc, p.mode * 1000 + p.W);
+  if (p.ups == 3) {
+    const long long total = (long long)((p.Qalloc + 31) / 32) * 128 * (p.s[0].Cpad >> 3);
+    return launch_pdl(parity_split_prep_kernel, dim3((unsigned)((total + 255) / 256)), dim3(256), 0, st, p);
+  }
   if (p.ups == 2) {
     const long long total = (long long)p.Qalloc * (p.s[0].Cpad >> 3);
     return launch_pdl(zero_insert_prep_kernel, dim3((unsigned)((total + 255) / 256)), dim3(256), 0, st, p);
@@ -1135,7 +1159,8 @@
     o.a = a; o.has_b = b != nullptr; if (b) o.b = *b;
     o.upsample = upsample; o.mode = mode; o.film = film; o.gamma_idx = gamma_idx; o.beta_idx = beta_idx; o.silu = silu; o.also_raw = also_raw; o.split = split;
     o.C0 = round_up(a.C, 16); o.C1 = b ? round_up(b->C, 16) : 0;
-    o.H = upsample ? 2 * a.H : a.H; o.W = upsample ? 2 * a.W : a.W;
+    const bool doubled = upsample == 1 || upsample == 2;
+    o.H = doubled ? 2 * a.H : a.H; o.W = doubled ? 2 * a.W : a.W;
     materialize(o);
     return o;
   }
@@ -1180,6 +1205,7 @@
     d.precise = cw.precise; d.wpk_layout = cw.trs;
     if (split) { d.src0_lo = raw ? in.rl0 : in.nl0; d.src1_lo = in.C1 ? in.rl1 : nullptr; }
     d.C0 = in.C0; d.C1 = in.C1; d.B = pl->B; d.H = in.H; d.W = in.W; d.taps = cw.taps; d.stride = stride;
+    d.flags = (pl->train ? 0 : DMD_CONV_NO_PAD_TAIL) | (in.upsample == 3 ? DMD_CONV_S2_PLANES : 0);
     d.wpk = pk(cw.pk_off); d.bias = P(cw.b_idx);
     d.Cout = cw.Cout; d.CoutPad = cw.CoutPad;
     d.residual = resid ? (resid->data ? resid->data : (const float*)1) : nullptr; d.out = out.data ? out.data : (float*)1;
@@ -1192,6 +1218,16 @@
       if (conv_fill(&dp, &op.conv, &op.smem, &op.cols)) { err = 1; return; }
       pl->ops.push_back(op);
     }
+  }
+
+  size_t operand_slot_bytes(int B, int H, int W, int C) const {
+    const size_t plain = plc16_bytes(B, H, W, C), split = pl->train ? 0 : plc16_bytes(B, H / 2, W / 2, 4 * C);
+    return plain > split ? plain : split;
+  }
+
+  int down_ups(const ConvW& cw, const Tens& x) const {
+    const bool waves = plc_geometry(pl->B, x.H, x.W).Q > kPlanSms * kTileM;
+    return !pl->train && waves && !cw.precise && !cw.three_pass && conv_s2_fits(x.H, x.W, cw.Cin, cw.CoutPad) ? 3 : 0;
   }
 
   Tens resblock(const ResBlockW& rb, const Tens& x, const Tens* skip) {
@@ -1228,7 +1264,7 @@
     if (H % (1 << (L - 1)) || W % (1 << (L - 1))) return fail("rew_end: H=%d W=%d must be multiples of %d", H, W, 1 << (L - 1));
     int cmax = 16;
     for (int i = 0; i < L; ++i) cmax = c.channels[i] > cmax ? c.channels[i] : cmax;
-    const size_t slot_bytes = (plc16_bytes(B, H, W, cmax) + 255) & ~(size_t)255;
+    const size_t slot_bytes = (operand_slot_bytes(B, H, W, cmax) + 255) & ~(size_t)255;
     for (int i = 0; i < kScratchSlots; ++i) pl->scratch[i] = (uint8_t*)bump->take(slot_bytes);
     pl->scratch_next = 0;
     pl->CP_in = h->conv_in.c0_store;
@@ -1245,7 +1281,7 @@
     for (int i = 0; i <= L; ++i) {
       if (i > 0 && i < L) {
         Tens xd = tensor(c.channels[i - 1], x.H / 2, x.W / 2, true);
-        Operand ind = prep(x, nullptr, 0, 0, nullptr, 0, 0, false, false);
+        Operand ind = prep(x, nullptr, down_ups(h->downs[i], x), 0, nullptr, 0, 0, false, false);
         conv(h->downs[i], ind, false, 2, nullptr, xd, true);
         Rec rec; rec.kind = R_DOWN; rec.cw = &h->downs[i]; rec.x = x; rec.o = xd; rec.in1 = ind; record(rec);
         x = xd;
@@ -1272,7 +1308,7 @@
     if (padded && pl->train) return fail("denoiser: training at H=%d W=%d (not multiples of %d) needs the pad / crop adjoints, which are not built", H, W, div);
     int cmax = 16;
     for (int i = 0; i < L; ++i) cmax = c.channels[i] > cmax ? c.channels[i] : cmax;
-    const size_t slot_bytes = (plc16_bytes(B, Hp, Wp, cmax) + 255) & ~(size_t)255;
+    const size_t slot_bytes = (operand_slot_bytes(B, Hp, Wp, cmax) + 255) & ~(size_t)255;
     for (int i = 0; i < kScratchSlots; ++i) pl->scratch[i] = (uint8_t*)bump->take(slot_bytes);
     pl->scratch_next = 0;
     pl->CP_in = h->conv_in.c0_store;
@@ -1299,7 +1335,7 @@
       Tens xd = x;
       if (i > 0) {
         xd = tensor(c.channels[i - 1], x.H / 2, x.W / 2, true);
-        Operand in = prep(x, nullptr, 0, 0, nullptr, 0, 0, false, false);
+        Operand in = prep(x, nullptr, down_ups(h->downs[i], x), 0, nullptr, 0, 0, false, false);
         conv(h->downs[i], in, false, 2, nullptr, xd, true);
         Rec rec; rec.kind = R_DOWN; rec.cw = &h->downs[i]; rec.x = x; rec.o = xd; rec.in1 = in; record(rec);
       }
diff --git a/diamond_b200/csrc/conv_tc.cuh b/diamond_b200/csrc/conv_tc.cuh
--- a/diamond_b200/csrc/conv_tc.cuh
+++ b/diamond_b200/csrc/conv_tc.cuh
@@ -54,6 +54,7 @@
   unsigned long long plane_bytes;
   int P, Palloc;
   int num_tiles, stages;
+  int s2;
   int trs;
   FastDiv dPW, dPH;
   long long* ktrace;
@@ -66,12 +67,12 @@
 __host__ __device__ inline uint32_t conv_weight_bytes(int taps, int Cin, int Cextra, int CoutPad) {
   return (((uint32_t)taps * Cin * CoutPad * 2 + 127u) & ~127u) + (uint32_t)Cextra * CoutPad * 2;
 }
-__host__ __device__ inline ConvSmemLayout conv_smem_layout(uint32_t w_bytes, int Palloc, int stages) {
+__host__ __device__ inline ConvSmemLayout conv_smem_layout(uint32_t w_bytes, int Palloc, int stages, int subs = 1) {
   ConvSmemLayout L;
   L.bias_off = 512;
   L.w_off = L.bias_off + 128 * 4;
   L.a_off = (L.w_off + w_bytes + 127u) & ~127u;
-  L.slab_bytes = 2u * Palloc * 16;
+  L.slab_bytes = 2u * subs * Palloc * 16;
   L.total = L.a_off + (uint32_t)stages * L.slab_bytes + 16;
   return L;
 }
@@ -257,7 +258,7 @@
   uint64_t* wbar = reinterpret_cast<uint64_t*>(smem);
   uint64_t* full = wbar + 1;
   uint64_t* empty = full + kMaxStages;
-  const ConvSmemLayout L = conv_smem_layout(conv_weight_bytes(p.taps, p.Cin, p.Cextra, p.CoutPad), p.Palloc, p.stages);
+  const ConvSmemLayout L = conv_smem_layout(conv_weight_bytes(p.taps, p.Cin, p.Cextra, p.CoutPad), p.Palloc, p.stages, p.s2 ? 4 : 1);
   float* sbias = reinterpret_cast<float*>(smem + L.bias_off);
   uint8_t* sW = smem + L.w_off;
   uint8_t* sA = smem + L.a_off;
@@ -301,7 +302,18 @@
       for (int ks = 0; ks < kslabs; ++ks, ++nslab) {
         if ((nslab & 1u) == pid) {
           mbar_wait(empty + stage, phase ^ 1u);
-          if (elect_one_sync()) {
+          if (p.s2) {
+            if (elect_one_sync()) {
+              uint8_t* slab = sA + (size_t)stage * L.slab_bytes;
+              mbar_expect_tx(full + stage, 8 * chunk_bytes);
+              const uint8_t* plane = p.seg_base[seg] + (size_t)(8 * seg_ks) * p.plane_bytes + pos0;
+#pragma unroll
+              for (int s = 0; s < 4; ++s)
+#pragma unroll
+                for (int c = 0; c < 2; ++c)
+                  bulk_g2s(slab + (size_t)(2 * s + c) * p.Palloc * 16, plane + (size_t)(4 * c + s) * p.plane_bytes, chunk_bytes, full + stage);
+            }
+          } else if (elect_one_sync()) {
             uint8_t* slab = sA + (size_t)stage * L.slab_bytes;
             const bool xs = ks >= main_slabs;
             const uint32_t bytes = xs ? (uint32_t)kTileM * 16 : chunk_bytes;
@@ -333,10 +345,14 @@
     const uint32_t slab16 = L.slab_bytes >> 4;
     const uint32_t kstep16 = (2u * b_lbo) >> 4;
     const uint32_t xstep16 = (2u * x_lbo) >> 4;
+    const int par = p.s2 ? 2 * p.Palloc : 0;
+    const int tap_dy[3] = {p.s2 ? 2 * par - p.PW : -p.PW, 0, p.s2 ? 2 * par : p.PW};
+    const int tap_dx[3] = {par - 1, 0, p.s2 ? par : 1};
     uint32_t shift[kTaps], b_tap[kTaps];
 #pragma unroll
     for (int t = 0; t < kTaps; ++t) {
-      shift[t] = (uint32_t)(halo + (kTaps == 9 ? (t / 3 - 1) * p.PW + (t % 3 - 1) : 0));
+      shift[t] = (uint32_t)(halo + (kTaps == 9 ? tap_dy[t / 3] + tap_dx[t % 3] : 0));
+      asm volatile("" : "+r"(shift[t]));
       b_tap[t] = p.trs ? ((uint32_t)(t / 3) * p.Cin * 3u * p.CoutPad * 2 + (uint32_t)(t % 3) * p.CoutPad * 16) >> 4
                        : ((uint32_t)t * p.Cin * p.CoutPad * 2) >> 4;
     }
@@ -712,4 +728,32 @@
   *reinterpret_cast<uint4*>(S.dst + (size_t)j * p.plane_bytes + (size_t)pa * 16) = packed;
 }
 
-}
+__global__ void __launch_bounds__(256) parity_split_prep_kernel(const PrepParams p) {
+  pdl_launch_dependents();
+  pdl_wait();
+  if (blockIdx.x == 0 && threadIdx.x == 0) ktrace_stamp(p.ktrace);
+  const PrepSrc& S = p.s[0];
+  const int lgn = __ffs(S.Cpad >> 3) - 1;
+  const uint32_t idx = blockIdx.x * blockDim.x + threadIdx.x;
+  const int j = (int)(idx & ((1u << lgn) - 1u));
+  const uint32_t t = idx >> lgn;
+  const int par = (int)((t >> 5) & 3u);
+  const int pa = (int)(((t >> 7) << 5) | (t & 31u));
+  if (pa >= p.Qalloc) return;
+  uint4 packed = make_uint4(0u, 0u, 0u, 0u);
+  const int q = pa - p.G;
+  if (q >= 0 && q < p.Q && j * 8 < S.C) {
+    const uint32_t R = p.dPW.div((uint32_t)q);
+    const int x = q - (int)R * p.PW;
+    const int n = (int)p.dPH.div(R);
+    const int y = (int)R - n * p.PH;
+    if (x < p.W && y < p.H) {
+      const float4* gp = reinterpret_cast<const float4*>(S.src + (((size_t)n * p.Hs + 2 * y + (par >> 1)) * p.Ws + 2 * x + (par & 1)) * S.C + j * 8);
+      const float4 a = __ldg(gp), b = __ldg(gp + 1);
+      packed.x = pack_h2(a.x, a.y); packed.y = pack_h2(a.z, a.w); packed.z = pack_h2(b.x, b.y); packed.w = pack_h2(b.z, b.w);
+    }
+  }
+  *reinterpret_cast<uint4*>(S.dst + (size_t)(4 * j + par) * p.plane_bytes + (size_t)pa * 16) = packed;
+}
+
+}
diff --git a/diamond_b200/ops.py b/diamond_b200/ops.py
--- a/diamond_b200/ops.py
+++ b/diamond_b200/ops.py
@@ -57,7 +57,10 @@
     return st
 
 
-def prep_act(src0: Tensor, *, src1: Optional[Tensor] = None, upsample: bool = False, mode: int = 0, silu: bool = False,
+CONV_NO_PAD_TAIL, CONV_S2_PLANES = 1, 2
+
+
+def prep_act(src0: Tensor, *, src1: Optional[Tensor] = None, upsample: int = 0, mode: int = 0, silu: bool = False,
              stats0: Optional[Tensor] = None, stats1: Optional[Tensor] = None, gs0: int = 0, gs1: int = 0,
              film: Optional[Tensor] = None, film_off: int = 0, gamma: Optional[Tensor] = None, beta: Optional[Tensor] = None,
              eps: float = 1e-5, also_raw: bool = False, split: bool = False, raw_split: bool = False):
@@ -66,17 +69,20 @@
         raise ValueError("raw_split needs also_raw")
     lib = _lib.lib()
     b, hs, ws, c0 = src0.shape
-    h, w = (2 * hs, 2 * ws) if upsample else (hs, ws)
+    upsample = int(upsample)
+    h, w = (2 * hs, 2 * ws) if upsample in (1, 2) else (hs, ws)
     c1 = src1.shape[3] if src1 is not None else 0
 
     def buf(c):
+        if upsample == 3:
+            return torch.empty(lib.dmd_plc16_bytes(b, h // 2, w // 2, 4 * round_up(c, 16)), dtype=torch.uint8, device=src0.device)
         return torch.empty(lib.dmd_plc16_bytes(b, h, w, c), dtype=torch.uint8, device=src0.device)
 
     n0, n1 = buf(c0), (buf(c1) if c1 else None)
     r0, r1 = (buf(c0) if also_raw else None), (buf(c1) if (also_raw and c1) else None)
     d = _lib.PrepDesc()
     d.src0, d.src1, d.C0, d.C1 = src0.data_ptr(), _lib.ptr(src1), c0, c1
-    d.B, d.Hs, d.Ws, d.upsample, d.mode, d.silu = b, hs, ws, int(upsample), mode, int(silu)
+    d.B, d.Hs, d.Ws, d.upsample, d.mode, d.silu = b, hs, ws, upsample, mode, int(silu)
     d.stats0, d.stats1, d.gs0, d.gs1 = _lib.ptr(stats0), _lib.ptr(stats1), gs0, gs1
     d.film, d.film_stride, d.film_off = _lib.ptr(film), (film.shape[1] if film is not None else 0), film_off
     d.gamma, d.beta, d.eps = _lib.ptr(gamma), _lib.ptr(beta), eps
@@ -97,7 +103,7 @@
                    cout_pad: int, taps: int = 9, *, bias: Optional[Tensor] = None, stride: int = 1,
                    residual: Optional[Tensor] = None, out_gs: int = 0, out: Optional[Tensor] = None,
                    ostats: Optional[Tensor] = None, debug: int = 0, debug_buf: Optional[Tensor] = None,
-                   lo0: Optional[Tensor] = None, lo1: Optional[Tensor] = None, xproj=None, trs: bool = False):
+                   lo0: Optional[Tensor] = None, lo1: Optional[Tensor] = None, xproj=None, trs: bool = False, flags: int = 0):
     _cuda(n0, n1, wpk, bias, residual)
     ho, wo = h // stride, w // stride
     if out is None:
@@ -106,7 +112,7 @@
         ostats = torch.zeros(b, cout // out_gs, 2, device=n0.device, dtype=torch.float64)
     d = _lib.ConvDesc()
     d.src0, d.src1, d.C0, d.C1 = n0.data_ptr(), _lib.ptr(n1), c0, c1
-    d.B, d.H, d.W, d.taps, d.stride = b, h, w, taps, stride
+    d.B, d.H, d.W, d.taps, d.stride, d.flags = b, h, w, taps, stride, flags
     d.wpk, d.bias, d.Cout, d.CoutPad = wpk.data_ptr(), _lib.ptr(bias), cout, cout_pad
     d.residual, d.out, d.out_stats, d.out_gs, d.debug = _lib.ptr(residual), out.data_ptr(), _lib.ptr(ostats), out_gs, debug
     d.debug_buf = _lib.ptr(debug_buf)
diff --git a/include/diamond_b200.h b/include/diamond_b200.h
--- a/include/diamond_b200.h
+++ b/include/diamond_b200.h
@@ -52,6 +52,9 @@
 
 int dmd_prep_act(const dmd_prep_desc* d, void* stream);
 
+#define DMD_CONV_NO_PAD_TAIL 1
+#define DMD_CONV_S2_PLANES 2
+
 typedef struct dmd_conv_desc {
   const void* src0;
   const void* src1;
@@ -59,6 +62,7 @@
   int B, H, W;
   int taps;
   int stride;
+  int flags;
   const void* wpk;
   const float* bias;
   int Cout, CoutPad;
```

Result: faster. 6813, median of 6 (+2.4%).
